# CFGpp-diffusion/CFGpp

Hardware: AMD Instinct MI355X
Metric: images/sec (higher is better)
Workload: dtype fp16; 1 GPU; SD1.5 512x512 ddim_cfg++ 50 NFE lambda=0.6 batch=8/GPU; per_gpu_batch=8, global_batch=8, nfe=50, unet_batch_rows=16, weights=seeded synthetic, exact diffusers shapes, build_id=cfgpp-build:b06ef47996861b66:nogit

## Files before the change

### cfgpp_amd/_lib.py

```python
from __future__ import annotations

import ctypes as C
import os

HERE = os.path.dirname(os.path.abspath(__file__))
LIB_PATH = os.environ.get("CFGPP_LIB") or os.path.join(HERE, "libcfgpp_hip.so")


class CfgppError(RuntimeError):
    pass


class UNetConfigC(C.Structure):
    _fields_ = [
        ("in_channels", C.c_int), ("out_channels", C.c_int),
        ("num_levels", C.c_int),
        ("block_out_channels", C.c_int * 4),
        ("layers_per_block", C.c_int),
        ("level_has_attn", C.c_int * 4),
        ("transformer_depth", C.c_int * 4),
        ("num_heads", C.c_int * 4),
        ("cross_attention_dim", C.c_int),
        ("addition_embed", C.c_int),
        ("addition_time_embed_dim", C.c_int),
        ("addition_pooled_dim", C.c_int),
        ("norm_groups", C.c_int),
        ("sample_h", C.c_int), ("sample_w", C.c_int),
        ("max_rows", C.c_int),
    ]


_P, _I, _F, _L = C.c_void_p, C.c_int, C.c_float, C.c_long

PROTOTYPES = {
    "cfgpp_last_error": (C.c_char_p, []),
    "cfgpp_build_id": (C.c_char_p, []),
    "cfgpp_step_ddim": (_I, [_P, _P, _P, _P, _I, _F, _F, _F, _F, _F, _I, _I, _L, _P]),
    "cfgpp_step_ddim_h": (_I, [_P, _P, _P, _P, _F, _F, _F, _F, _F, _I, _I, _L, _P]),
    "cfgpp_step_ddim_masked": (_I, [_P, _P, _P, _P, _F, _F, _F, _F, _F, _I, _I, _P, _P, _P, _F, _F, _I, _L, _P]),
    "cfgpp_kdiff_input": (_I, [_P, _P, _F, _I, _L, _P]),
    "cfgpp_step_kdiff": (_I, [_P, _P, _P, _P, _P, C.POINTER(C.c_float), _I, _I, _I, _I, _L, _P]),
    "cfgpp_kdiff_denoise": (_I, [_P, _P, _P, _F, _F, _P, _P, _L, _P]),
    "cfgpp_lincomb": (_I, [_P, _P, _P, _P, _F, _F, _I, _L, _P]),
    "cfgpp_unet_create": (_P, [C.POINTER(UNetConfigC), _I]),
    "cfgpp_unet_destroy": (None, [_P]),
    "cfgpp_unet_load_tensor": (_I, [_P, C.c_char_p, _P, _I, C.POINTER(C.c_long), _I]),
    "cfgpp_unet_missing": (_I, [_P]),
    "cfgpp_unet_finalize": (_I, [_P]),
    "cfgpp_unet_set_context": (_I, [_P, _P, _I, _I, _P, _P, _I, _P]),
    "cfgpp_unet_image_condition": (_I, [_P, _P, _I, _P]),
    "cfgpp_unet_forward": (_I, [_P, _P, _I, _I, _F, _P, _I, _P]),
    "cfgpp_sample_graph_ddim": (_I, [_P, _P, _P, _I, _I, _P, _P, _P, _I, C.POINTER(C.c_float), _I, _F, _I, _I, _P]),
    "cfgpp_unet_profile": (_I, [_P, _P, _I, _I, _F, _P, _I, _P, C.POINTER(C.c_double), C.POINTER(C.c_double), C.POINTER(C.c_int), C.c_char_p, _L]),
    "cfgpp_unet_tuning": (_I, [_P, _I, C.POINTER(C.c_int), _I, _I]),
    "cfgpp_unet_attach_control": (_I, [_P, _P, _F]),
    "cfgpp_unet_lora": (_I, [_P, C.c_char_p, _P, _P, _I, _P]),
    "cfgpp_unet_flops": (C.c_double, [_P, _I]),
    "cfgpp_unet_device_bytes": (C.c_double, [_P]),
    "cfgpp_vae_create": (_P, [_I, _I, _I, _F, _I]),
    "cfgpp_vae_destroy": (None, [_P]),
    "cfgpp_vae_load_tensor": (_I, [_P, C.c_char_p, _P, _I, C.POINTER(C.c_long), _I]),
    "cfgpp_vae_finalize": (_I, [_P]),
    "cfgpp_vae_decode": (_I, [_P, _P, _P, _I, _P]),
    "cfgpp_vae_decode_image": (_I, [_P, _P, _P, _I, _P]),
    "cfgpp_vae_encode": (_I, [_P, _P, _P, _P, _P, _I, _P]),
    "cfgpp_vae_flops": (C.c_double, [_P, _I]),
    "cfgpp_text_create": (_P, [_I, _I, _I, _I, _I, _I, _I, _I, _I]),
    "cfgpp_text_destroy": (None, [_P]),
    "cfgpp_text_load_tensor": (_I, [_P, C.c_char_p, _P, _I, C.POINTER(C.c_long), _I]),
    "cfgpp_text_finalize": (_I, [_P]),
    "cfgpp_text_encode": (_I, [_P, C.POINTER(C.c_int), C.POINTER(C.c_int), _I, _I, _P, _P, _P]),
    "cfgpp_text_device_bytes": (C.c_double, [_P]),
    "cfgpp_vae_encode_flops": (C.c_double, [_P, _I]),
    "cfgpp_vae_device_bytes": (C.c_double, [_P]),
}

IP_ADAPTER_PROTOTYPES = {
    "cfgpp_unet_ip_load": (_I, [_P, C.c_char_p, _P, _I, C.POINTER(C.c_long), _I]),
    "cfgpp_unet_image_context": (_I, [_P, _P, _I, _I, _F, _P]),
}

LONG_PROMPT_PROTOTYPES = {
    "cfgpp_unet_set_max_tokens": (_I, [_P, _I]),
}

DEBUG_PROTOTYPES = {
    "cfgpp_op_softmax_rows": (_I, [_P, _L, _I, _P]),
    "cfgpp_op_conv_in_ex": (_I, [_P, _I, _P, _P, _P, _I, _I, _I, _I, _I, _I, _P, _P, _F, _P]),
    "cfgpp_op_groupnorm": (_I, [_P, _P, _P, _P, _P, _P, _I, _I, _I, _I, _I, _I, _F, _I, _I, _P]),
    "cfgpp_op_groupnorm_pre": (_I, [_P, _P, _P, _P, _P, _P, _P, _P, _I, _I, _I, _I, _I, _I, _F, _I, _I, _P]),
    "cfgpp_op_igemm_set_gstat": (None, [_P]),
    "cfgpp_op_igemm_gstat_written": (_I, []),
    "cfgpp_groupnorm_set_prestats": (None, [_I]),
    "cfgpp_groupnorm_prestats_enabled": (_I, []),
    "cfgpp_unet_set_share_prefix": (None, [_I]),
    "cfgpp_unet_share_prefix_enabled": (_I, []),
    "cfgpp_unet_shared_prefix_ops": (_I, [_P, _I, _I]),
    "cfgpp_op_layernorm": (_I, [_P, _P, _P, _P, _L, _I, _F, _P]),
    "cfgpp_op_attention_prepare_vt": (_I, [_P, _I, _I, _I, _P]),
    "cfgpp_op_attention": (_I, [_P, _P, _P, _P, _I, _I, _I, _I, _I, _I, _I, _P]),
    "cfgpp_op_attention_cross": (_I, [_P, _P, _P, _P, _I, _I, _I, _I, _I, _I, _I, _P]),
    "cfgpp_attention_set_cross_long": (None, [_I]),
    "cfgpp_op_attention_clear_slots": (_I, [_P, _P, _I, _I, _I, _I, _I, _P]),
    "cfgpp_op_attention_ip": (_I, [_P, _P, _P, _P, _I, _I, _I, _I, _I, _I, _F, _I, _I, _P]),
    "cfgpp_op_conv_in": (_I, [_P, _I, _P, _P, _P, _I, _I, _I, _I, _I, _I, _P]),
    "cfgpp_op_conv_in_cond": (_I, [_P, _I, _P, _I, _I, _P, _P, _P, _I, _I, _I, _I, _I, _I, _P]),
    "cfgpp_op_conv_in_add": (_I, [_P, _I, _P, _I, _I, _P, _I, _P, _P, _P, _I, _I, _I, _I, _I, _I, _P]),
    "cfgpp_op_cn_conv3x3": (_I, [_P, _I, _P, _I, _P, _P, _I, _I, _I, _I, _I, _I, _I, _P]),
    "cfgpp_op_residual_add": (_I, [C.POINTER(C.c_void_p), C.POINTER(C.c_void_p), C.POINTER(C.c_int), _I, _I, _F, _P]),
    "cfgpp_op_residual_nchw": (_I, [_P, _P, _I, _I, _I, _I, _F, _P]),
    "cfgpp_controlnet_residual": (_I, [_P, _I, _F, _P, _I, C.POINTER(C.c_int), _P]),
    "cfgpp_vae_profile": (_I, [_P, _P, _P, _I, _P, C.c_char_p, C.c_long]),
    "cfgpp_unet_read_weight": (_I, [_P, C.c_char_p, _P]),
    "cfgpp_op_vae_posterior": (_I, [_P, _P, _P, _P, _P, _P, _I, _I, _F, _P]),
    "cfgpp_op_conv_out": (_I, [_P, _P, _I, _P, _P, _I, _I, _I, _I, _I, _P]),
    "cfgpp_op_conv_out_ex": (_I, [_P, _P, _I, _P, _P, _I, _I, _I, _I, _I, _F, _F, _I, _P]),
    "cfgpp_conv_out_set_tiled": (None, [_I]),
    "cfgpp_op_sinusoid": (_I, [_P, _F, _P, _I, _I, _I, _I, _P]),
    "cfgpp_op_skinny_gemm": (_I, [_P, _I, _P, _P, _P, _I, _P, _I, _I, _I, _I, _I, _I, _P]),
    "cfgpp_op_f16_to_f32_rows": (_I, [_P, _P, _I, _I, _I, _I, _P]),
    "cfgpp_op_igemm": (_I, [_P, _P, _I, _I, _I, _I, _I, _I, _P, _I, _I, _P, _P, _I, _P, _I, _I, _P, _I, _I, _I, _P]),
    "cfgpp_op_igemm_heads": (_I, [_P, _I, _P, _I, _I, _P, _I, _P, _P, _P, _I, _I, _I, _I, _I, _I, _P]),
    "cfgpp_op_fold_upsample": (_I, [_P, _P, _I, _I, _P]),
    "cfgpp_op_upsample_conv3x3": (_I, [_P, _I, _I, _I, _P, _P, _I, _I, _P, _P, _P]),
    "cfgpp_igemm_set_upsample_phase": (None, [_I]),
    "cfgpp_igemm_last_amode": (_I, []),
    "cfgpp_igemm_last_config_ran": (_I, []),
    "cfgpp_igemm_force_config": (None, [_I]),
    "cfgpp_igemm_set_staging": (None, [_I]),
    "cfgpp_igemm_set_staged_epilogue": (None, [_I]),
    "cfgpp_igemm_set_big_tiles": (None, [_I]),
    "cfgpp_igemm_set_tail_split": (None, [_I]),
    "cfgpp_igemm_set_autotune": (None, [_I]),
    "cfgpp_igemm_set_blocked_walk": (None, [_I]),
    "cfgpp_igemm_walk_plan_probe": (None, [_I, _I, _I, _I, _I, _I, _I, C.POINTER(C.c_int)]),
    "cfgpp_igemm_set_n_major": (None, [_I]),
    "cfgpp_igemm_force_split": (None, [_I]),
    "cfgpp_igemm_set_split_tile": (None, [_I]),
    "cfgpp_igemm_set_mf16": (None, [_I]),
    "cfgpp_igemm_set_mf16_rounds": (None, [_I]),
    "cfgpp_igemm_set_mf16_heads": (None, [_I]),
    "cfgpp_igemm_set_mf16_linear": (None, [_I]),
    "cfgpp_igemm_set_big_split": (None, [_I]),
    "cfgpp_igemm_set_tune_mask": (None, [C.c_uint]),
    "cfgpp_igemm_tuner_state": (C.c_uint, []),
    "cfgpp_igemm_timeline": (None, [_P, _L, _I]),
    "cfgpp_igemm_timeline_info": (None, [C.POINTER(C.c_int)]),
    "cfgpp_groupnorm_set_mode": (None, [_I]),
    "cfgpp_layernorm_set_rows_per_wave": (None, [_I]),
    "cfgpp_attention_set_dma": (None, [_I]),
    "cfgpp_attention_set_stagger": (None, [_I]),
    "cfgpp_attention_set_cross": (None, [_I]),
    "cfgpp_attention_last_launch": (None, [C.POINTER(C.c_int)]),
    "cfgpp_groupnorm_last_launch": (None, [C.POINTER(C.c_int)]),
    "cfgpp_layernorm_last_launch": (None, [C.POINTER(C.c_int)]),
    "cfgpp_softmax_last_launch": (None, [C.POINTER(C.c_int)]),
}

_lib = None


def load():
    global _lib
    if _lib is not None:
        return _lib
    if not os.path.exists(LIB_PATH):
        raise CfgppError(
            f"{LIB_PATH} not found: build it with `python -m cfgpp_amd.build` "
            "(__graft_entry__.build()).  The HIP path has no CPU fallback.")
    import torch
    try:
        lib = C.CDLL(LIB_PATH)
    except OSError as e:
        raise CfgppError(f"cannot load {LIB_PATH}: {e}") from e
    for name, (res, args) in list(PROTOTYPES.items()) + list(IP_ADAPTER_PROTOTYPES.items()) + list(LONG_PROMPT_PROTOTYPES.items()) + list(DEBUG_PROTOTYPES.items()):
        try:
            fn = getattr(lib, name)
        except AttributeError as e:
            raise CfgppError(f"{LIB_PATH} does not export {name}") from e
        fn.restype = res
        fn.argtypes = args
    if os.environ.get("CFGPP_AUTOTUNE", "1") == "0":
        lib.cfgpp_igemm_set_autotune(0)
    _lib = lib
    return lib


def build_id() -> str:
    return load().cfgpp_build_id().decode("utf-8", "replace")


def last_error() -> str:
    return load().cfgpp_last_error().decode("utf-8", "replace")


def check(rc: int, what: str):
    if rc != 0:
        raise CfgppError(f"{what} failed (rc={rc}): {last_error()}")
```

### cfgpp_amd/csrc/cfgpp_debug.h

```cpp
#ifndef CFGPP_DEBUG_H
#define CFGPP_DEBUG_H
#ifdef __cplusplus
extern "C" {
#endif

int cfgpp_op_softmax_rows(void* s, long rows, int ncols, void* stream);
int cfgpp_op_conv_in_ex(const void* z, int z_is_half, void* out, const float* w, const float* bias,
                        int R, int zB, int Cin, int H, int W, int Cout, const float* pre_w, const float* pre_b,
                        float in_scale, void* stream);
int cfgpp_op_groupnorm(const void* src0, const void* src1, void* dst, const float* gamma, const float* beta,
                       float* stats, int N, int H, int W, int C0, int C1, int G, float eps, int silu,
                       int dst_padded, void* stream);
int cfgpp_op_groupnorm_pre(const void* src0, const void* src1, void* dst, const float* gamma, const float* beta,
                           const float* gst0, const float* gst1, float* stats, int N, int H, int W, int C0, int C1, int G,
                           float eps, int silu, int dst_padded, void* stream);
void cfgpp_op_igemm_set_gstat(void* buf);
int cfgpp_op_igemm_gstat_written(void);
void cfgpp_groupnorm_set_prestats(int on);
int cfgpp_groupnorm_prestats_enabled(void);
void cfgpp_unet_set_share_prefix(int on);
int cfgpp_unet_share_prefix_enabled(void);
int cfgpp_unet_shared_prefix_ops(cfgpp_unet* u, int rows, int z_rows);
void cfgpp_groupnorm_set_mode(int mode);
int cfgpp_op_layernorm(const void* x, void* y, const float* gamma, const float* beta, long rows, int C,
                       float eps, void* stream);
void cfgpp_layernorm_set_rows_per_wave(int rpw);
void cfgpp_groupnorm_last_launch(int* out8);
void cfgpp_layernorm_last_launch(int* out2);
void cfgpp_softmax_last_launch(int* out1);
int cfgpp_op_attention_prepare_vt(void* vt, int BH, int d, int tok_pad, void* stream);
int cfgpp_op_attention(const void* q, const void* k, const void* vt, void* o, int B, int heads, int d,
                       int nq, int nk, int q_tok_pad, int k_tok_pad, void* stream);
void cfgpp_attention_set_dma(int mode);
void cfgpp_attention_set_stagger(int sleeps);
void cfgpp_attention_set_cross(int on);
int cfgpp_op_attention_cross(const void* q, const void* k, const void* vt, void* o, int B, int heads, int d,
                             int nq, int nk, int q_tok_pad, int k_tok_pad, void* stream);
void cfgpp_attention_set_cross_long(int mode);
void cfgpp_attention_last_launch(int* out4);
int cfgpp_op_attention_clear_slots(void* k, void* vt, int BH, int d, int tok_pad, int slot0, int n, void* stream);
int cfgpp_op_attention_ip(const void* q, const void* k, const void* vt, void* o, int B, int heads, int d, int nq, int nk_text,
                          int n_img, float ip_scale, int q_tok_pad, int k_tok_pad, void* stream);
int cfgpp_op_conv_in(const void* z, int z_is_half, void* out, const float* w, const float* bias,
                     int R, int zB, int Cin, int H, int W, int Cout, void* stream);
int cfgpp_op_conv_in_cond(const void* z, int z_is_half, const void* cond, int cond_rows, int Cc, void* out, const float* w,
                          const float* bias, int R, int zB, int Cz, int H, int W, int Cout, void* stream);
int cfgpp_op_conv_in_add(const void* z, int z_is_half, const void* cond, int cond_rows, int Cc, const void* addend, int add_rows,
                         void* out, const float* w, const float* bias, int R, int zB, int Cz, int H, int W, int Cout, void* stream);
int cfgpp_op_cn_conv3x3(const void* in, int in_kind, void* out, int out_pad, const float* w, const float* bias, int R, int Ci, int Co,
                        int Hi, int Wi, int stride, int silu, void* stream);
int cfgpp_op_residual_add(void* const* dst, const void* const* src, const int* hwc, int n, int rows, float scale, void* stream);
int cfgpp_op_residual_nchw(const void* src, float* out, int rows, int H, int W, int C, float scale, void* stream);
int cfgpp_controlnet_residual(cfgpp_unet* cn, int i, float scale, float* out, int rows, int* hwc_out, void* stream);

int cfgpp_unet_read_weight(cfgpp_unet* u, const char* key, void* host_fp16_out);

int cfgpp_vae_profile(cfgpp_vae* v, const void* z, void* img, int B, void* stream, char* detail, long detail_cap);

int cfgpp_op_vae_posterior(const float* conv_out, const float* qw, const float* qb, const float* noise, float* z,
                           float* moments, int B, int HW, float scale, void* stream);
int cfgpp_op_conv_out(const void* x, void* out, int out_is_half, const void* w, const float* bias,
                      int R, int H, int W, int C, int Cout, void* stream);
int cfgpp_op_conv_out_ex(const void* x, void* out, int out_is_half, const void* w, const float* bias,
                         int R, int H, int W, int C, int Cout, float post_scale, float post_shift, int clamp01, void* stream);
void cfgpp_conv_out_set_tiled(int on);
int cfgpp_op_sinusoid(const float* vals, float scalar, float* out, int count, int dim, int out_ld, int out_off,
                      void* stream);
int cfgpp_op_skinny_gemm(const float* x, int ldx, const void* w, const float* bias, const float* addend, int add_ld,
                         float* out, int ldo, int M, int N, int K, int silu_in, int silu_out, void* stream);
int cfgpp_op_f16_to_f32_rows(const void* in, float* out, int rows, int cols, int out_ld, int out_off, void* stream);

int cfgpp_op_igemm(const void* a0, const void* a1, int C0, int C1, int taps, int amode, int H, int W,
                   const void* w, int M, int N, const float* bias, const float* temb, int temb_ld,
                   const void* resid, int rmode, int rld, void* out, int omode, int old_, int epi,
                   void* stream);
int cfgpp_op_fold_upsample(const void* w9, void* w4, int O, int I, void* stream);
int cfgpp_op_upsample_conv3x3(const void* src, int C, int Hs, int Ws, const void* w9, const void* w4, int rows, int N,
                              const float* bias, void* out, void* stream);
void cfgpp_igemm_set_upsample_phase(int on);
int cfgpp_igemm_last_amode(void);
int cfgpp_igemm_last_config_ran(void);
int cfgpp_op_igemm_heads(const void* a, int K, const void* w, int M, int N, const float* bias, int rows_per_batch,
                         void* hq, void* hk, void* hvt, int part0, int part_width, int head_dim, int heads,
                         int q_tok_pad, int tok_pad, void* stream);
void cfgpp_igemm_force_config(int cfg);
void cfgpp_igemm_set_tail_split(int on);
void cfgpp_igemm_set_mf16(int mode);
void cfgpp_igemm_set_mf16_linear(int on);
void cfgpp_igemm_set_mf16_heads(int on);
void cfgpp_igemm_set_mf16_rounds(int n);
void cfgpp_igemm_set_split_tile(int cfg);
void cfgpp_igemm_force_split(int s);
void cfgpp_igemm_set_big_split(int min_kt);
void cfgpp_igemm_set_n_major(int mode);
void cfgpp_igemm_set_blocked_walk(int on);
void cfgpp_igemm_walk_plan_probe(int M, int N, int K, int BM, int BN, int smem, int n_major, int* out5);
void cfgpp_igemm_set_tune_mask(unsigned mask);
unsigned cfgpp_igemm_tuner_state(void);
void cfgpp_igemm_set_autotune(int on);
void cfgpp_igemm_set_big_tiles(int on);
void cfgpp_igemm_set_staged_epilogue(int on);
void cfgpp_igemm_set_staging(int glds);
void cfgpp_igemm_timeline(void* buf, long cap_blocks, int target);
void cfgpp_igemm_timeline_info(int* out12);

#ifdef __cplusplus
}
#endif
#endif
```

### cfgpp_amd/csrc/common.h

```cpp
#pragma once
#include <hip/hip_runtime.h>
#include <stdint.h>

typedef _Float16 half_t;
typedef _Float16 half2_t __attribute__((ext_vector_type(2)));
typedef _Float16 half4_t __attribute__((ext_vector_type(4)));
typedef _Float16 half8_t __attribute__((ext_vector_type(8)));
typedef float f32x4 __attribute__((ext_vector_type(4)));
typedef float f32x16 __attribute__((ext_vector_type(16)));

#define CFGPP_WAVE 64

void cfgpp_set_error(const char* fmt, ...);
int cfgpp_claim_device(int device_id);
#define CFGPP_HIP_CHECK(expr)                                                         \
    do {                                                                              \
        hipError_t _e = (expr);                                                       \
        if (_e != hipSuccess) {                                                       \
            cfgpp_set_error("%s:%d: %s -> %s", __FILE__, __LINE__, #expr,             \
                            hipGetErrorString(_e));                                   \
            return -1;                                                                \
        }                                                                             \
    } while (0)
#define CFGPP_REQUIRE(cond, ...)                                                      \
    do {                                                                              \
        if (!(cond)) {                                                                \
            cfgpp_set_error(__VA_ARGS__);                                             \
            return -2;                                                                \
        }                                                                             \
    } while (0)

int step_advance_launch(const float* tab, int* idx, float* cur, hipStream_t s);
int step_ddim_dev_launch(void* z, void* z0t_out, const void* eps_uc, const void* eps_c, int eps_is_half, int z_is_half, float lam,
                         const float* cdev, int tweedie_uc, int renoise_uc, long n, hipStream_t s);

struct CnAddEntry {
    half_t* dst;
    const half_t* src;
    int H, W, C, pad_;
};
int cn_residual_add_launch(const CnAddEntry* tab, int n, long max_n8, int rows, float scale, hipStream_t s);

int fanout_rows_launch(half_t* const* p, const long* row_elems, int nseg, int h, hipStream_t s);

int lora_merge_launch(const half_t* base, half_t* dst, const float* up, const float* down, int rank, int kind, long O, long I,
                      int taps, hipStream_t s);

static inline int cdiv(long a, long b) { return (int)((a + b - 1) / b); }

struct RowMap {
    int mode;
    int H, W;
    int ld;
};

__host__ __device__ __forceinline__ int cfgpp_vt_pos(int tok) {
    return (tok & ~12) | ((tok & 4) << 1) | ((tok & 8) >> 1);
}

__device__ __forceinline__ float silu_f(float x) { return x / (1.0f + __expf(-x)); }
__device__ __forceinline__ float gelu_erf_f(float x) {
    const float ax = fabsf(x) * 0.70710678118654752440f;
    const float t = __builtin_amdgcn_rcpf(1.0f + 0.3275911f * ax);
    const float poly = t * (0.254829592f + t * (-0.284496736f + t * (1.421413741f + t * (-1.453152027f + t * 1.061405429f))));
    const float erfc_ax = poly * __builtin_amdgcn_exp2f(-ax * ax * 1.4426950408889634f);
    const float cdf = x >= 0.f ? 1.0f - 0.5f * erfc_ax : 0.5f * erfc_ax;
    return x * cdf;
}

typedef float f32x2 __attribute__((ext_vector_type(2)));
#define CFGPP_GELU_C 4.75f
#define CFGPP_GELU_POLY {4.912262559e-01f, 5.645360425e-02f, -1.591939032e-01f, 2.464362979e-01f, -1.982378513e-01f, 1.363233291e-02f, \
                         1.386516690e-01f, -1.158297956e-01f, -9.092462249e-03f, 6.090912968e-02f, -1.936562732e-02f, -1.160200126e-02f, \
                         6.012340542e-03f}
__device__ __forceinline__ f32x2 gelu_erf_pk(f32x2 x) {
    constexpr float k[13] = CFGPP_GELU_POLY;
    f32x2 a;
    a.x = fminf(fabsf(x.x), CFGPP_GELU_C); a.y = fminf(fabsf(x.y), CFGPP_GELU_C);
    const f32x2 t = __builtin_elementwise_fma(a, (f32x2){2.0f / CFGPP_GELU_C, 2.0f / CFGPP_GELU_C}, (f32x2){-1.0f, -1.0f});
    f32x2 p = {k[12], k[12]};
#pragma unroll
    for (int i = 11; i >= 0; --i) p = __builtin_elementwise_fma(p, t, (f32x2){k[i], k[i]});
    f32x2 m;
    m.x = fabsf(x.x) * p.x; m.y = fabsf(x.y) * p.y;
    return __builtin_elementwise_fma(x, (f32x2){0.5f, 0.5f}, m);
}

template <int MAXV>
__device__ __forceinline__ void ln_row_stats(const half8_t (&raw)[MAXV], int chunks, int C, float eps, int lane,
                                             float (&v)[MAXV][8], float& mean, float& rstd) {
    float sum = 0.f;
#pragma unroll
    for (int j = 0; j < MAXV; ++j) {
        const bool live = lane + j * 64 < chunks;
#pragma unroll
        for (int k = 0; k < 8; ++k) { v[j][k] = live ? (float)raw[j][k] : 0.f; sum += v[j][k]; }
    }
#pragma unroll
    for (int o = 32; o > 0; o >>= 1) sum += __shfl_xor(sum, o);
    mean = sum / (float)C;
    float sq = 0.f;
#pragma unroll
    for (int j = 0; j < MAXV; ++j) {
        const bool live = lane + j * 64 < chunks;
#pragma unroll
        for (int k = 0; k < 8; ++k) { const float d = v[j][k] - mean; sq = live ? fmaf(d, d, sq) : sq; }
    }
#pragma unroll
    for (int o = 32; o > 0; o >>= 1) sq += __shfl_xor(sq, o);
    rstd = rsqrtf(sq / (float)C + eps);
}
__device__ __forceinline__ half8_t ln_row_affine(const float (&v)[8], float mean, float rstd, const float4 (&g)[2], const float4 (&be)[2]) {
    const float gg[8] = {g[0].x, g[0].y, g[0].z, g[0].w, g[1].x, g[1].y, g[1].z, g[1].w};
    const float bb[8] = {be[0].x, be[0].y, be[0].z, be[0].w, be[1].x, be[1].y, be[1].z, be[1].w};
    half8_t o;
#pragma unroll
    for (int k = 0; k < 8; ++k) {
        float f = fmaf((v[k] - mean) * rstd, gg[k], bb[k]);
        asm volatile("" : "+v"(f));
        o[k] = (half_t)f;
    }
    return o;
}
```

### cfgpp_amd/csrc/engine_base.h

```cpp
#pragma once
#include <algorithm>
#include <cmath>
#include <cstring>
#include <deque>
#include <functional>
#include <map>
#include <string>
#include <utility>
#include <vector>

#include "../../include/cfgpp.h"
#include "../../include/cfgpp_ip_adapter.h"
#include "../../include/cfgpp_long_prompt.h"
#include "cfgpp_debug.h"
#include "igemm.h"

namespace {


struct HostParam {
    std::vector<long> shape;
    std::vector<half_t> h;
    std::vector<float> f;
    bool is_matrix = false;
    bool loaded = false;
    long numel() const { long n = 1; for (long s : shape) n *= s; return n; }
};

struct Tensor {
    half_t* p = nullptr;
    int H = 0, W = 0, C = 0;
    float* gst = nullptr;
    int* gst_ok = nullptr;
};

using Op = std::function<int(hipStream_t, int )>;

enum { SLOT_PLAIN = 0, SLOT_CONV3 = 1, SLOT_GEGLU = 2, SLOT_MEMBER = 3 };
struct WeightSlot {
    half_t* ptr = nullptr;
    int kind = SLOT_PLAIN;
    long row_off = 0;
    long O = 0, I = 0; int taps = 1;
    half_t* base = nullptr;
    long K() const { return I * taps; }
    half_t* rows() const { return ptr + row_off * K(); }
};


struct EngineBase {
    int max_rows = 1;
    int norm_groups = 32;
    std::map<std::string, HostParam> params;
    std::map<std::string, WeightSlot> slots;
    std::vector<void*> allocs;
    double dev_bytes = 0;
    double macs_per_row = 0;
    double attn_macs_per_row = 0;

    std::vector<Op> plan;
    std::vector<int> plan_kind;
    std::vector<double> plan_macs;
    std::vector<std::string> plan_desc;
    std::vector<char> plan_share;
    int rows_for(size_t i, int rows, bool shared) const {
        const int m = i < plan_share.size() ? plan_share[i] : 0;
        if (m == 0) return rows;
        return shared ? rows / 2 : (m == 1 ? rows : 0);
    }
    void tag(int kind, double macs, const std::string& desc = "") {
        plan_kind.resize(plan.size(), 3); plan_macs.resize(plan.size(), 0.0); plan_desc.resize(plan.size());
        if (!plan.empty()) { plan_kind.back() = kind; plan_macs.back() = macs; plan_desc.back() = desc; }
    }
    std::deque<int> cfg_hints;
    std::vector<int*> plan_hint;
    int tuned_rows = 0;
    bool tuned_shared = false;
    std::map<std::pair<int, bool>, std::vector<int>> tuned_by_rows;
    int* new_hint(bool in_main_plan) {
        cfg_hints.push_back(0);
        int* h = &cfg_hints.back();
        if (in_main_plan) { plan_hint.resize(plan.size() + 1, nullptr); plan_hint[plan.size()] = h; }
        return h;
    }
    int tune_plan(hipStream_t s, int rows, bool shared = false) {
        const auto key = std::make_pair(rows, shared);
        auto cached = tuned_by_rows.find(key);
        if (cached != tuned_by_rows.end() && cached->second.size() == cfg_hints.size()) {
            size_t k = 0;
            for (int& h : cfg_hints) h = cached->second[k++];
            tuned_rows = rows; tuned_shared = shared;
            return 0;
        }
        static const int cands[] = {0, 1, 4, 5, 6, 7, 8, 9, 10, 11, 12, 13, 14, 15, 16, 17, 20, 24, 25, 26, 27, 28};
        const size_t n = plan.size();
        plan_hint.resize(n, nullptr);
        hipStreamCaptureStatus cap = hipStreamCaptureStatusNone;
        if (hipStreamIsCapturing(s, &cap) != hipSuccess || cap != hipStreamCaptureStatusNone) return 0;
// ... 333 lines not shown
```

### cfgpp_amd/csrc/norm_kernels.hip

```cpp
#include <algorithm>
#include "common.h"

namespace {

struct GNArgs {
    const half_t* src0;
    const half_t* src1;
    half_t* dst;
    const float* gamma;
    const float* beta;
    float* stats;
    int nblk;
    int spb;
    int N, H, W;
    int C0, C1;
    int G;
    float eps;
    int silu;
    int pix_per_block;
    int dst_padded;
    int gs;
    const float* gst0; const float* gst1;
    int pre;
};
// ... 225 lines not shown
    }
    s_acc[tid] = acc;
    __syncthreads();
    for (int o = 128; o > 0; o >>= 1) {
        if (tid < o) { GnAcc x = s_acc[tid]; gn_acc_merge(x, s_acc[tid + o]); s_acc[tid] = x; }
        __syncthreads();
    }
    if (tid == 0) {
        const GnAcc t = s_acc[0];
        float var = t.m2 / t.n;
        var = var < 0.f ? 0.f : var;
        float* dst = a.stats + ((long)n * a.G + g) * 2;
        dst[0] = t.mean; dst[1] = rsqrtf(var + a.eps);
    }
}

__global__ void __launch_bounds__(256)
gn_apply_kernel(GNArgs a) {
    __shared__ float s_mean[64], s_rstd[64];
    const int C = a.C0 + a.C1;
    const int cpg = C / a.G;
    const int chunks = C / 8;
    const int n = blockIdx.y;
    const int HW = a.H * a.W;
    const int p0 = blockIdx.x * a.pix_per_block;
    const int p1 = min(p0 + a.pix_per_block, HW);
    if (a.pre) {
        if ((int)threadIdx.x < a.G) {
            const float2 mr = *reinterpret_cast<const float2*>(a.stats + ((long)n * a.G + threadIdx.x) * 2);
            s_mean[threadIdx.x] = mr.x; s_rstd[threadIdx.x] = mr.y;
        }
    } else {
        __shared__ float s_ps[8][64];
        const int NSL = 256 / a.G < 8 ? 256 / a.G : 8;
        const int g = threadIdx.x % a.G, sl = threadIdx.x / a.G;
        const float* st = a.stats + (long)n * a.nblk * a.G * 2;
        const float n_full = (float)(cpg * a.spb), n_last = (float)(cpg * (HW - (a.nblk - 1) * a.spb));
        const float inv_cnt = 1.0f / ((float)cpg * (float)HW);
        const float ref = st[g * 2];
        if (sl < NSL) {
            float s = 0.f;
            for (int b = sl; b < a.nblk; b += NSL) s += (b == a.nblk - 1 ? n_last : n_full) * (st[((long)b * a.G + g) * 2] - ref);
            s_ps[sl][g] = s;
        }
        __syncthreads();
        float tot = 0.f;
        for (int k = 0; k < NSL; ++k) tot += s_ps[k][g];
        const float mean = ref + tot * inv_cnt;
        __syncthreads();
        if (sl < NSL) {
            float q = 0.f;
            for (int b = sl; b < a.nblk; b += NSL) {
                const float2 mm = *reinterpret_cast<const float2*>(st + ((long)b * a.G + g) * 2);
                const float d = mm.x - mean;
                q += mm.y + (b == a.nblk - 1 ? n_last : n_full) * d * d;
            }
            s_ps[sl][g] = q;
        }
        __syncthreads();
        if ((int)threadIdx.x < a.G) {
            float m2 = 0.f;
            for (int k = 0; k < NSL; ++k) m2 += s_ps[k][g];
            s_mean[g] = mean; s_rstd[g] = rsqrtf(m2 * inv_cnt + a.eps);
        }
    }
    __syncthreads();
    const int ppi = max(1, (int)blockDim.x / chunks);
    const float invW = 1.0f / (float)a.W;
    const long pbase = (long)n * (a.H + 2) * (a.W + 2) + (a.W + 2) + 1;
    auto poff = [&](int p) -> long { return pbase + p + 2 * (int)(((float)p + 0.5f) * invW); };
    for (int cbase = 0; cbase < chunks; cbase += blockDim.x) {
        int chunk, psub;
        if (chunks <= (int)blockDim.x) { chunk = threadIdx.x % chunks; psub = threadIdx.x / chunks; }
        else { chunk = cbase + threadIdx.x; psub = 0; }
        const bool active = (chunk < chunks) && (psub < ppi);
        if (active) {
            const int c = chunk * 8;
            const half_t* src; int cs, Cs;
            if (c < a.C0) { src = a.src0; cs = c; Cs = a.C0; } else { src = a.src1; cs = c - a.C0; Cs = a.C1; }
            float sc[8], sh[8];
#pragma unroll
            for (int k = 0; k < 8; ++k) {
                const int g = (c + k) / cpg;
                const float ga = a.gamma[c + k] * s_rstd[g];
                sc[k] = ga; sh[k] = a.beta[c + k] - s_mean[g] * ga;
            }
            auto one = [&](int p, const half8_t v, long po) {
                half8_t o;
#pragma unroll
                for (int k = 0; k < 8; ++k) {
                    float f = (float)v[k] * sc[k] + sh[k];
                    if (a.silu) f = silu_f(f);
                    o[k] = (half_t)f;
                }
                const long orow = a.dst_padded ? po : ((long)n * HW + p);
                *reinterpret_cast<half8_t*>(a.dst + orow * C + c) = o;
            };
            int p = p0 + psub;
            for (; p + 3 * ppi < p1; p += 4 * ppi) {
                half8_t v[4]; long po[4];
#pragma unroll
                for (int u = 0; u < 4; ++u) { po[u] = poff(p + u * ppi); v[u] = *reinterpret_cast<const half8_t*>(src + po[u] * Cs + cs); }
#pragma unroll
                for (int u = 0; u < 4; ++u) one(p + u * ppi, v[u], po[u]);
            }
            for (; p < p1; p += ppi) {
                const long po = poff(p);
                one(p, *reinterpret_cast<const half8_t*>(src + po * Cs + cs), po);
            }
        }
        if (chunks <= (int)blockDim.x) break;
    }
}

int g_gn_mode = 0;
int g_ln_rpw = 0;
int g_gn_last[8] = {0, 0, 0, 0, 0, 0, 0, 0};
int g_ln_last[2] = {0, 0};
int g_sm_last[1] = {0};

template <int MAXCH, int NT>
void launch_gn_slab(const GNArgs& a, int wgs, hipStream_t s) {
    hipLaunchKernelGGL((gn_slab_kernel<MAXCH, NT>), dim3(wgs), dim3(NT), 0, s, a);
}

template <int MAXV, int RPW>
__global__ void __launch_bounds__(256)
layernorm_kernel(const half_t* __restrict__ x, half_t* __restrict__ y, const float* __restrict__ gamma,
                 const float* __restrict__ beta, long rows, int C, float eps) {
    const int lane = threadIdx.x & 63;
    const long row0 = ((long)blockIdx.x * 4 + (threadIdx.x >> 6)) * RPW;
    if (row0 >= rows) return;
    const int chunks = C / 8;
    half8_t raw[RPW][MAXV];
#pragma unroll
    for (int r = 0; r < RPW; ++r) {
        const long row = row0 + r < rows ? row0 + r : rows - 1;
        const half_t* xr = x + row * C;
#pragma unroll
        for (int j = 0; j < MAXV; ++j) {
            const int ch = lane + j * 64;
            raw[r][j] = *reinterpret_cast<const half8_t*>(xr + (ch < chunks ? ch : chunks - 1) * 8);
        }
    }
    float v[RPW][MAXV][8];
    float mean[RPW], rstd[RPW];
#pragma unroll
    for (int r = 0; r < RPW; ++r) ln_row_stats<MAXV>(raw[r], chunks, C, eps, lane, v[r], mean[r], rstd[r]);
    float4 g[MAXV][2], be[MAXV][2];
#pragma unroll
    for (int j = 0; j < MAXV; ++j) {
        const int ch = lane + j * 64;
        const int cc = (ch < chunks ? ch : chunks - 1) * 8;
        g[j][0] = *reinterpret_cast<const float4*>(gamma + cc); g[j][1] = *reinterpret_cast<const float4*>(gamma + cc + 4);
        be[j][0] = *reinterpret_cast<const float4*>(beta + cc); be[j][1] = *reinterpret_cast<const float4*>(beta + cc + 4);
    }
#pragma unroll
    for (int j = 0; j < MAXV; ++j) {
        const int ch = lane + j * 64;
        if (ch < chunks) {
#pragma unroll
            for (int r = 0; r < RPW; ++r)
                if (row0 + r < rows) *reinterpret_cast<half8_t*>(y + (row0 + r) * C + ch * 8) = ln_row_affine(v[r][j], mean[r], rstd[r], g[j], be[j]);
        }
    }
}

template <int MAXC>
__global__ void __launch_bounds__(256)
softmax_rows_kernel(half_t* __restrict__ s, int ncols) {
    __shared__ float red[8];
    half_t* row = s + (long)blockIdx.x * ncols;
    const int nchunks = ncols / 8;
    const int tid = threadIdx.x, lane = tid & 63, wid = tid >> 6;
    float v[MAXC][8];
    float mx = -INFINITY;
#pragma unroll
// ... 76 lines not shown
    a.gamma = gamma; a.beta = beta;
    a.N = N; a.H = H; a.W = W; a.C0 = C0; a.C1 = C1; a.G = G; a.eps = eps; a.silu = silu;
    a.dst_padded = dst_padded; a.stats = stats; a.nblk = 0; a.spb = 0; a.gs = 1; a.pix_per_block = 0;
    a.gst0 = nullptr; a.gst1 = nullptr; a.pre = 0;
    const int HW = H * W;
    const int cpg = C / G;
    if (g_gn_mode != 1 && cpg >= 8) {
        int gs = 0;
        for (int t = 1; t <= 4; t <<= 1) if (G % t == 0 && (t * cpg) % 8 == 0) { gs = t; break; }
        const int cpp = gs ? gs * cpg / 8 : 0;
        int nt = 0;
        if (cpp && cpp <= 32) {
            for (int cand : {320, 640, 960}) {
                if (cand % cpp) continue;
                const int chunks_per_thread = cdiv(HW, cand / cpp);
                if (chunks_per_thread <= 16) { nt = cand; break; }
            }
        }
        if (nt) {
            const int R = nt / cpp, cpt = cdiv(HW, R);
            const int wgs = N * (G / gs);
            const bool worth = g_gn_mode == 2 || wgs >= 48;
            if (worth) {
                a.gs = gs;
#define GN_SLAB(NT_)                                                                        \
                if (nt == NT_) {                                                            \
                    if (cpt <= 2) launch_gn_slab<2, NT_>(a, wgs, s);                        \
                    else if (cpt <= 4) launch_gn_slab<4, NT_>(a, wgs, s);                   \
                    else if (cpt <= 8) launch_gn_slab<8, NT_>(a, wgs, s);                   \
                    else launch_gn_slab<16, NT_>(a, wgs, s);                                \
                }
                GN_SLAB(320) GN_SLAB(640) GN_SLAB(960)
#undef GN_SLAB
                g_gn_last[0] = 1; g_gn_last[1] = nt; g_gn_last[2] = cpt <= 2 ? 2 : cpt <= 4 ? 4 : cpt <= 8 ? 8 : 16;
                g_gn_last[3] = gs; g_gn_last[4] = cpp;
                CFGPP_HIP_CHECK(hipGetLastError());
                return 0;
            }
        }
    }
    const int nblk_max = std::max(64, std::min(256, cdiv(768, N)));
    int ppb = 16;
    while (cdiv(HW, ppb) > nblk_max) ppb <<= 1;
    a.pix_per_block = ppb; a.spb = ppb;
    a.nblk = cdiv(HW, ppb);
    hipLaunchKernelGGL(gn_stats_kernel, dim3(a.nblk, N), dim3(256), 0, s, a);
    GNArgs b = a;
    int apb = 64;
    while (apb > 16 && (long)N * cdiv(HW, apb) < 1024) apb >>= 1;
    b.pix_per_block = apb;
    hipLaunchKernelGGL(gn_apply_kernel, dim3(cdiv(HW, apb), N), dim3(256), 0, s, b);
    g_gn_last[0] = 2; g_gn_last[5] = ppb; g_gn_last[6] = a.nblk; g_gn_last[7] = apb;
    CFGPP_HIP_CHECK(hipGetLastError());
    return 0;
}

int cfgpp_op_groupnorm_pre(const void* src0, const void* src1, void* dst, const float* gamma, const float* beta,
                           const float* gst0, const float* gst1, float* stats, int N, int H, int W, int C0, int C1, int G,
                           float eps, int silu, int dst_padded, void* stream) {
    for (int i = 0; i < 8; ++i) g_gn_last[i] = 0;
    const int C = C0 + C1;
    CFGPP_REQUIRE(G > 0 && G <= 64 && C % G == 0, "groupnorm_pre: C=%d not divisible by G=%d (G<=64)", C, G);
    CFGPP_REQUIRE(C0 % 8 == 0 && C1 % 8 == 0, "groupnorm_pre: C0=%d C1=%d must be multiples of 8", C0, C1);
    CFGPP_REQUIRE((H * W) % 32 == 0, "groupnorm_pre: H*W=%d must be a multiple of 32 (the producers' statistics blocks)", H * W);
    CFGPP_REQUIRE(src0 && dst && gamma && beta && stats && gst0 && (C1 == 0 || (src1 && gst1)), "groupnorm_pre: null pointer");
    hipStream_t s = (hipStream_t)stream;
    GNArgs a;
    a.src0 = (const half_t*)src0; a.src1 = (const half_t*)src1; a.dst = (half_t*)dst;
    a.gamma = gamma; a.beta = beta;
    a.N = N; a.H = H; a.W = W; a.C0 = C0; a.C1 = C1; a.G = G; a.eps = eps; a.silu = silu;
    a.dst_padded = dst_padded; a.stats = stats; a.nblk = 0; a.spb = 0; a.gs = 1;
    a.gst0 = gst0; a.gst1 = gst1; a.pre = 1;
    const int HW = H * W;
    hipLaunchKernelGGL(gn_finalize_kernel, dim3(G, N), dim3(256), 0, s, a);
    int apb = 64;
    while (apb > 16 && (long)N * cdiv(HW, apb) < 1024) apb >>= 1;
    a.pix_per_block = apb;
    hipLaunchKernelGGL(gn_apply_kernel, dim3(cdiv(HW, apb), N), dim3(256), 0, s, a);
    g_gn_last[0] = 3; g_gn_last[7] = apb;
    CFGPP_HIP_CHECK(hipGetLastError());
    return 0;
}

int cfgpp_op_layernorm(const void* x, void* y, const float* gamma, const float* beta, long rows, int C,
                       float eps, void* stream) {
    g_ln_last[0] = 0; g_ln_last[1] = 0;
    CFGPP_REQUIRE(C % 8 == 0 && C <= 64 * 8 * 4, "layernorm: C=%d must be a multiple of 8 and <= 2048", C);
    CFGPP_REQUIRE(x && y && gamma && beta && rows > 0, "layernorm: bad args");
    hipStream_t s = (hipStream_t)stream;
    const int need = cdiv(C / 8, 64);
    const int rpw = g_ln_rpw > 0 ? g_ln_rpw : (C <= 320 && rows >= 2L * 4096 ? 2 : 1);
#define LN_LAUNCH(MV, RP) hipLaunchKernelGGL((layernorm_kernel<MV, RP>), dim3(cdiv(rows, 4 * RP)), dim3(256), 0, s, \
                                             (const half_t*)x, (half_t*)y, gamma, beta, rows, C, eps)
#define LN_BY_RPW(MV) do { if (rpw >= 4) LN_LAUNCH(MV, 4); else if (rpw == 2) LN_LAUNCH(MV, 2); else LN_LAUNCH(MV, 1); } while (0)
    if (need <= 1) LN_BY_RPW(1);
    else if (need <= 2) LN_BY_RPW(2);
    else if (need <= 3) LN_BY_RPW(3);
    else LN_LAUNCH(4, 1);
    g_ln_last[0] = need <= 3 ? need : 4; g_ln_last[1] = need <= 3 ? (rpw >= 4 ? 4 : rpw == 2 ? 2 : 1) : 1;
#undef LN_BY_RPW
#undef LN_LAUNCH
    CFGPP_HIP_CHECK(hipGetLastError());
    return 0;
}

}
```

### cfgpp_amd/csrc/small_kernels.hip

```cpp
#include <algorithm>

#include "common.h"

namespace {

template <typename TIN>
__global__ void __launch_bounds__(256)
conv_in_kernel(const TIN* __restrict__ z, const half_t* __restrict__ cond, int Cc, int cond_rows,
               half_t* __restrict__ out, const float* __restrict__ w,
               const float* __restrict__ bias, int R, int zB, int Cz, int H, int W, int Cout,
               const float* __restrict__ pre_w, const float* __restrict__ pre_b, float in_scale,
               const half_t* __restrict__ add, int add_rows) {
    constexpr int TP = 16;
    __shared__ float patch[TP][9 * 16];
    const int r = blockIdx.y;
    const int p0 = blockIdx.x * TP;
    const int HW = H * W;
    const int zb = r % zB;
    const int cb = cond ? zb % cond_rows : 0;
    const int Cin = Cz + Cc;
    const int K = 9 * Cin;
    for (int i = threadIdx.x; i < TP * K; i += blockDim.x) {
        const int tp = i / K, k = i - tp * K;
        const int tap = k / Cin, ci = k - tap * Cin;
        const int p = p0 + tp;
        float v = 0.f;
        if (p < HW) {
            const int y = p / W + tap / 3 - 1, x = p % W + tap % 3 - 1;
            if (y >= 0 && y < H && x >= 0 && x < W) {
                if (ci >= Cz) {
                    v = (float)cond[((long)(cb * Cc + ci - Cz) * H + y) * W + x];
                } else if (pre_w) {
                    float acc = pre_b ? pre_b[ci] : 0.f;
                    for (int j = 0; j < Cz; ++j)
                        acc += pre_w[ci * Cz + j] * (float)(half_t)((float)z[((long)(zb * Cz + j) * H + y) * W + x] * in_scale);
                    v = acc;
                } else {
                    v = (float)z[((long)(zb * Cz + ci) * H + y) * W + x] * in_scale;
                }
            }
        }
        patch[tp][k] = (float)(half_t)v;
    }
    __syncthreads();
    for (int co = threadIdx.x; co < Cout; co += blockDim.x) {
        float acc[TP];
        const float b = bias ? bias[co] : 0.f;
#pragma unroll
        for (int tp = 0; tp < TP; ++tp) acc[tp] = b;
        for (int k = 0; k < K; ++k) {
            const float wv = w[(long)k * Cout + co];
#pragma unroll
            for (int tp = 0; tp < TP; ++tp) acc[tp] += wv * patch[tp][k];
        }
#pragma unroll
        for (int tp = 0; tp < TP; ++tp) {
            const int p = p0 + tp;
            if (p < HW) {
                const int y = p / W, x = p - y * W;
                half_t v = (half_t)acc[tp];
                if (add) v = (half_t)((float)v + (float)add[((long)((zb % add_rows) * (H + 2) + y + 1) * (W + 2) + x + 1) * Cout + co]);
                out[((long)(r * (H + 2) + y + 1) * (W + 2) + x + 1) * Cout + co] = v;
            }
        }
    }
}

template <int CO, typename TOUT>
__global__ void __launch_bounds__(256)
conv_out_kernel(const half_t* __restrict__ x, TOUT* __restrict__ out, const half_t* __restrict__ w,
                const float* __restrict__ bias, int R, int H, int W, int C, int cout_real,
                float post_scale, float post_shift, int clamp01) {
    const int lane = threadIdx.x & 63;
    const long pix = (long)blockIdx.x * 4 + (threadIdx.x >> 6);
    const long total = (long)R * H * W;
    if (pix >= total) return;
    const int HW = H * W;
    const int r = (int)(pix / HW), p = (int)(pix - (long)r * HW);
    const int y = p / W, xq = p - y * W;
    const int cpt = C / 8;
    float acc[CO];
#pragma unroll
    for (int o = 0; o < CO; ++o) acc[o] = 0.f;
    for (int c = lane; c < 9 * cpt; c += 64) {
        const int tap = c / cpt, cc = (c - tap * cpt) * 8;
        const int dy = tap / 3 - 1, dx = tap % 3 - 1;
        const half8_t xv = *reinterpret_cast<const half8_t*>(
            x + ((long)(r * (H + 2) + y + 1 + dy) * (W + 2) + xq + 1 + dx) * C + cc);
#pragma unroll
        for (int o = 0; o < CO; ++o) {
            const half8_t wv = *reinterpret_cast<const half8_t*>(w + ((long)o * 9 + tap) * C + cc);
#pragma unroll
            for (int k = 0; k < 8; ++k) acc[o] += (float)xv[k] * (float)wv[k];
        }
    }
#pragma unroll
    for (int o = 0; o < CO; ++o)
#pragma unroll
        for (int s = 32; s > 0; s >>= 1) acc[o] += __shfl_xor(acc[o], s);
    if (lane < cout_real) {
        float v = 0.f;
#pragma unroll
        for (int o = 0; o < CO; ++o) if (lane == o) v = acc[o];
        v += bias ? bias[lane] : 0.f;
        v = v * post_scale + post_shift;
        if (clamp01) v = fminf(fmaxf(v, 0.f), 1.f);
        out[((long)(r * cout_real + lane) * H + y) * W + xq] = (TOUT)v;
    }
}

template <int CO, typename TOUT>
__global__ void __launch_bounds__(256)
conv_out_tile_kernel(const half_t* __restrict__ x, TOUT* __restrict__ out, const half_t* __restrict__ w,
                     const float* __restrict__ bias, int R, int H, int W, int C, int cout_real,
                     float post_scale, float post_shift, int clamp01) {
    constexpr int TH = 8, TW = 32, HH = TH + 2, HW_ = TW + 2, PITCH = 144;
    __shared__ __attribute__((aligned(16))) char tile[HH * HW_ * PITCH];
    const int tid = threadIdx.x;
    const int tiles_x = (W + TW - 1) / TW, tiles_y = (H + TH - 1) / TH;
    int b = blockIdx.x;
    const int txi = b % tiles_x; b /= tiles_x;
    const int tyi = b % tiles_y; const int r = b / tiles_y;
    const int y0 = tyi * TH, x0 = txi * TW;
    const int ty = tid >> 5, tx = tid & 31;
    typedef _Float16 h2 __attribute__((ext_vector_type(2)));
    float acc[CO];
#pragma unroll
    for (int o = 0; o < CO; ++o) acc[o] = 0.f;
    const half_t* xr = x + (long)r * (H + 2) * (W + 2) * C;
    for (int cb = 0; cb < C; cb += 64) {
        __syncthreads();
        for (int i = tid; i < HH * HW_ * 8; i += 256) {
            const int px = i >> 3, ch = i & 7;
            const int hy = px / HW_, hx = px - hy * HW_;
            const int gy = y0 + hy, gx = x0 + hx;
            half8_t v = {0, 0, 0, 0, 0, 0, 0, 0};
            if (gy < H + 2 && gx < W + 2) v = *reinterpret_cast<const half8_t*>(xr + ((long)gy * (W + 2) + gx) * C + cb + ch * 8);
            *reinterpret_cast<half8_t*>(tile + px * PITCH + ch * 16) = v;
        }
        __syncthreads();
#pragma unroll
        for (int tap = 0; tap < 9; ++tap) {
            const int dy = tap / 3, dx = tap - 3 * (tap / 3);
            const char* px = tile + ((ty + dy) * HW_ + tx + dx) * PITCH;
#pragma unroll
            for (int ch = 0; ch < 8; ++ch) {
                const half8_t xv = *reinterpret_cast<const half8_t*>(px + ch * 16);
#pragma unroll
                for (int o = 0; o < CO; ++o) {
                    const half8_t wv = *reinterpret_cast<const half8_t*>(w + ((long)o * 9 + tap) * C + cb + ch * 8);
#pragma unroll
                    for (int k = 0; k < 4; ++k)
                        acc[o] = __builtin_amdgcn_fdot2((h2){xv[2 * k], xv[2 * k + 1]}, (h2){wv[2 * k], wv[2 * k + 1]}, acc[o], false);
                }
            }
        }
    }
    const int y = y0 + ty, xq = x0 + tx;
    if (y < H && xq < W) {
#pragma unroll
        for (int o = 0; o < CO; ++o) {
            if (o < cout_real) {
                float v = acc[o] + (bias ? bias[o] : 0.f);
                v = v * post_scale + post_shift;
                if (clamp01) v = fminf(fmaxf(v, 0.f), 1.f);
                out[((long)(r * cout_real + o) * H + y) * W + xq] = (TOUT)v;
            }
        }
    }
}

__global__ void sinusoid_kernel(const float* __restrict__ vals, float scalar, float* __restrict__ out,
                                int count, int dim, int out_ld, int out_off) {
    const int i = blockIdx.x;
    const int half_dim = dim / 2;
    const float v = vals ? vals[i] : scalar;
    for (int j = threadIdx.x; j < half_dim; j += blockDim.x) {
        const float e = expf(-9.210340371976184f * (float)j / (float)half_dim);
        const float arg = v * e;
        out[(long)i * out_ld + out_off + j] = (float)(half_t)cosf(arg);
        out[(long)i * out_ld + out_off + half_dim + j] = (float)(half_t)sinf(arg);
    }
}

template <int MB, int NB>
__global__ void __launch_bounds__(256)
skinny_gemm_kernel(const float* __restrict__ x, int ldx, const half_t* __restrict__ w, const float* __restrict__ bias,
                   const float* __restrict__ addend, int add_ld, float* __restrict__ out, int ldo,
                   int M, int N, int K, int silu_in, int silu_out) {
    const int lane = threadIdx.x & 63, wid = threadIdx.x >> 6;
    const int n0 = (blockIdx.x * 4 + wid) * NB;
    const int m0 = blockIdx.y * MB;
    if (n0 >= N) return;
    float acc[MB][NB];
#pragma unroll
    for (int i = 0; i < MB; ++i)
#pragma unroll
        for (int j = 0; j < NB; ++j) acc[i][j] = 0.f;
    for (int kc = lane * 8; kc < K; kc += 64 * 8) {
        float xv[MB][8];
#pragma unroll
        for (int i = 0; i < MB; ++i) {
            const int m = min(m0 + i, M - 1);
            const float4 a = *reinterpret_cast<const float4*>(x + (long)m * ldx + kc);
            const float4 b = *reinterpret_cast<const float4*>(x + (long)m * ldx + kc + 4);
            xv[i][0] = a.x; xv[i][1] = a.y; xv[i][2] = a.z; xv[i][3] = a.w;
            xv[i][4] = b.x; xv[i][5] = b.y; xv[i][6] = b.z; xv[i][7] = b.w;
            if (silu_in) {
#pragma unroll
                for (int k = 0; k < 8; ++k) xv[i][k] = silu_f(xv[i][k]);
            }
        }
#pragma unroll
        for (int j = 0; j < NB; ++j) {
            const int n = min(n0 + j, N - 1);
            const half8_t wv = *reinterpret_cast<const half8_t*>(w + (long)n * K + kc);
#pragma unroll
            for (int i = 0; i < MB; ++i)
#pragma unroll
                for (int k = 0; k < 8; ++k) acc[i][j] += xv[i][k] * (float)wv[k];
        }
    }
#pragma unroll
    for (int i = 0; i < MB; ++i)
#pragma unroll
        for (int j = 0; j < NB; ++j)
#pragma unroll
            for (int s = 32; s > 0; s >>= 1) acc[i][j] += __shfl_xor(acc[i][j], s);
    if (lane == 0) {
#pragma unroll
        for (int i = 0; i < MB; ++i) {
            const int m = m0 + i;
            if (m >= M) continue;
#pragma unroll
            for (int j = 0; j < NB; ++j) {
                const int n = n0 + j;
                if (n >= N) continue;
                float v = acc[i][j] + (bias ? bias[n] : 0.f);
                if (addend) v += addend[(long)m * add_ld + n];
                if (silu_out) v = silu_f(v);
                out[(long)m * ldo + n] = v;
            }
        }
    }
}

__global__ void f16_to_f32_rows_kernel(const half_t* __restrict__ in, float* __restrict__ out, int rows, int cols,
                                       int out_ld, int out_off) {
    const long n = (long)rows * cols;
    for (long i = (long)blockIdx.x * blockDim.x + threadIdx.x; i < n; i += (long)gridDim.x * blockDim.x) {
        const int r = (int)(i / cols), c = (int)(i - (long)r * cols);
        out[(long)r * out_ld + out_off + c] = (float)in[i];
    }
}

struct FanoutArgs {
    uint4* p[3];
    long n16[3];
};

__global__ void __launch_bounds__(256)
fanout_rows_kernel(FanoutArgs a) {
    const long n = a.n16[blockIdx.y];
    const uint4* __restrict__ src = a.p[blockIdx.y];
    uint4* __restrict__ dst = a.p[blockIdx.y] + n;
    const long T = (long)gridDim.x * 256;
    long i = (long)blockIdx.x * 256 + threadIdx.x;
    for (; i + 3 * T < n; i += 4 * T) {
        const uint4 v0 = src[i], v1 = src[i + T], v2 = src[i + 2 * T], v3 = src[i + 3 * T];
        dst[i] = v0; dst[i + T] = v1; dst[i + 2 * T] = v2; dst[i + 3 * T] = v3;
    }
    for (; i < n; i += T) dst[i] = src[i];
}

}

int fanout_rows_launch(half_t* const* p, const long* row_elems, int nseg, int h, hipStream_t s) {
    CFGPP_REQUIRE(p && row_elems && nseg > 0 && nseg <= 3 && h > 0, "fanout_rows: bad args");
    FanoutArgs a{};
    long most = 0;
    for (int k = 0; k < nseg; ++k) {
        CFGPP_REQUIRE(p[k] && row_elems[k] > 0 && row_elems[k] % 8 == 0 && ((uintptr_t)p[k] & 15) == 0, "fanout_rows: segment %d is not made of 16-byte units", k);
        a.p[k] = reinterpret_cast<uint4*>(p[k]);
        a.n16[k] = (long)h * (row_elems[k] / 8);
        most = std::max(most, a.n16[k]);
    }
    dim3 grid((unsigned)std::min<long>(cdiv(most, 256 * 4), 2048), (unsigned)nseg);
    hipLaunchKernelGGL(fanout_rows_kernel, grid, dim3(256), 0, s, a);
    CFGPP_HIP_CHECK(hipGetLastError());
    return 0;
}


__global__ void __launch_bounds__(256)
vae_posterior_kernel(const float* __restrict__ co, const float* __restrict__ qw, const float* __restrict__ qb,
                     const float* __restrict__ noise, float* __restrict__ z, float* __restrict__ moments,
                     int B, int HW, float scale) {
    const long i = (long)blockIdx.x * blockDim.x + threadIdx.x;
    if (i >= (long)B * HW) return;
    const int b = (int)(i / HW), p = (int)(i - (long)b * HW);
    float x[8], m[8];
#pragma unroll
    for (int j = 0; j < 8; ++j) x[j] = (float)(half_t)co[((long)b * 8 + j) * HW + p];
#pragma unroll
    for (int o = 0; o < 8; ++o) {
        float acc = qb[o];
#pragma unroll
        for (int j = 0; j < 8; ++j) acc += qw[o * 8 + j] * x[j];
        m[o] = (float)(half_t)acc;
    }
#pragma unroll
    for (int c = 0; c < 4; ++c) {
        const float lv = fminf(fmaxf(m[4 + c], -30.f), 20.f);
        const float n = noise ? noise[((long)b * 4 + c) * HW + p] : 0.f;
        z[((long)b * 4 + c) * HW + p] = (m[c] + __expf(0.5f * lv) * n) * scale;
        if (moments) { moments[((long)b * 8 + c) * HW + p] = m[c]; moments[((long)b * 8 + 4 + c) * HW + p] = lv; }
    }
}

extern "C" {

int cfgpp_op_vae_posterior(const float* conv_out, const float* qw, const float* qb, const float* noise, float* z,
                           float* moments, int B, int HW, float scale, void* stream) {
    CFGPP_REQUIRE(conv_out && qw && qb && z && B > 0 && HW > 0, "vae_posterior: bad args");
    hipLaunchKernelGGL(vae_posterior_kernel, dim3(cdiv((long)B * HW, 256)), dim3(256), 0, (hipStream_t)stream, conv_out, qw, qb, noise, z, moments, B, HW, scale);
    CFGPP_HIP_CHECK(hipGetLastError());
    return 0;
}

int cfgpp_op_conv_in_add(const void* z, int z_is_half, const void* cond, int cond_rows, int Cc, const void* addend, int add_rows,
                         void* out, const float* w, const float* bias, int R, int zB, int Cz, int H, int W, int Cout, void* stream);

int cfgpp_op_conv_in_cond(const void* z, int z_is_half, const void* cond, int cond_rows, int Cc, void* out, const float* w,
                          const float* bias, int R, int zB, int Cz, int H, int W, int Cout, void* stream) {
    return cfgpp_op_conv_in_add(z, z_is_half, cond, cond_rows, Cc, nullptr, 1, out, w, bias, R, zB, Cz, H, W, Cout, stream);
}

int cfgpp_op_conv_in_add(const void* z, int z_is_half, const void* cond, int cond_rows, int Cc, const void* addend, int add_rows,
                         void* out, const float* w, const float* bias, int R, int zB, int Cz, int H, int W, int Cout, void* stream) {
    CFGPP_REQUIRE(Cz >= 1 && Cz <= 8, "conv_in: Cin=%d (<= 8)", Cz);
    CFGPP_REQUIRE(!addend || add_rows > 0, "conv_in: addend with add_rows=%d", add_rows);
    const half_t* add = (const half_t*)addend;
    if (!add) add_rows = 1;
    CFGPP_REQUIRE(!cond || (Cc >= 1 && Cz + Cc <= 16 && cond_rows > 0), "conv_in: condition of %d channels x %d rows on %d latent channels (Cin <= 16)",
                  Cc, cond_rows, Cz);
    CFGPP_REQUIRE(z && out && w && R > 0 && zB > 0, "conv_in: bad args");
    if (!cond) { Cc = 0; cond_rows = 1; }
    dim3 grid(cdiv((long)H * W, 16), R);
    hipStream_t s = (hipStream_t)stream;
    if (z_is_half)
        hipLaunchKernelGGL(conv_in_kernel<half_t>, grid, dim3(256), 0, s, (const half_t*)z, (const half_t*)cond, Cc, cond_rows, (half_t*)out, w, bias,
                           R, zB, Cz, H, W, Cout, (const float*)nullptr, (const float*)nullptr, 1.0f, add, add_rows);
    else
        hipLaunchKernelGGL(conv_in_kernel<float>, grid, dim3(256), 0, s, (const float*)z, (const half_t*)cond, Cc, cond_rows, (half_t*)out, w, bias,
                           R, zB, Cz, H, W, Cout, (const float*)nullptr, (const float*)nullptr, 1.0f, add, add_rows);
    CFGPP_HIP_CHECK(hipGetLastError());
    return 0;
}

int cfgpp_op_conv_in_ex(const void* z, int z_is_half, void* out, const float* w, const float* bias,
                        int R, int zB, int Cin, int H, int W, int Cout, const float* pre_w, const float* pre_b,
                        float in_scale, void* stream) {
    CFGPP_REQUIRE(Cin >= 1 && Cin <= 8, "conv_in: Cin=%d (<= 8)", Cin);
    CFGPP_REQUIRE(z && out && w && R > 0 && zB > 0, "conv_in: bad args");
    dim3 grid(cdiv((long)H * W, 16), R);
    hipStream_t s = (hipStream_t)stream;
    if (z_is_half)
        hipLaunchKernelGGL(conv_in_kernel<half_t>, grid, dim3(256), 0, s, (const half_t*)z, (const half_t*)nullptr, 0, 1, (half_t*)out, w, bias,
                           R, zB, Cin, H, W, Cout, pre_w, pre_b, in_scale, (const half_t*)nullptr, 1);
    else
        hipLaunchKernelGGL(conv_in_kernel<float>, grid, dim3(256), 0, s, (const float*)z, (const half_t*)nullptr, 0, 1, (half_t*)out, w, bias,
                           R, zB, Cin, H, W, Cout, pre_w, pre_b, in_scale, (const half_t*)nullptr, 1);
    CFGPP_HIP_CHECK(hipGetLastError());
    return 0;
}

int cfgpp_op_conv_in(const void* z, int z_is_half, void* out, const float* w, const float* bias,
                     int R, int zB, int Cin, int H, int W, int Cout, void* stream) {
    return cfgpp_op_conv_in_ex(z, z_is_half, out, w, bias, R, zB, Cin, H, W, Cout, nullptr, nullptr, 1.0f, stream);
}

int cfgpp_op_conv_out_ex(const void* x, void* out, int out_is_half, const void* w, const float* bias,
                         int R, int H, int W, int C, int Cout, float post_scale, float post_shift, int clamp01, void* stream);
static int g_conv_out_tiled = 1;
void cfgpp_conv_out_set_tiled(int on) { g_conv_out_tiled = on ? 1 : 0; }

int cfgpp_op_conv_out(const void* x, void* out, int out_is_half, const void* w, const float* bias,
                      int R, int H, int W, int C, int Cout, void* stream) {
    return cfgpp_op_conv_out_ex(x, out, out_is_half, w, bias, R, H, W, C, Cout, 1.0f, 0.0f, 0, stream);
}

int cfgpp_op_conv_out_ex(const void* x, void* out, int out_is_half, const void* w, const float* bias,
                         int R, int H, int W, int C, int Cout, float post_scale, float post_shift, int clamp01, void* stream) {
    CFGPP_REQUIRE(Cout >= 1 && Cout <= 8 && C % 8 == 0, "conv_out: Cout=%d C=%d", Cout, C);
    CFGPP_REQUIRE(x && out && w, "conv_out: null pointer");
    const long total = (long)R * H * W;
    dim3 grid(cdiv(total, 4));
    hipStream_t s = (hipStream_t)stream;
    if (Cout <= 4 && C % 64 == 0 && (long)H * W >= 128 * 128 && g_conv_out_tiled) {
        dim3 tg((unsigned)((long)R * cdiv(H, 8) * cdiv(W, 32)));
        if (out_is_half)
            hipLaunchKernelGGL((conv_out_tile_kernel<4, half_t>), tg, dim3(256), 0, s, (const half_t*)x, (half_t*)out, (const half_t*)w, bias, R, H, W, C, Cout, post_scale, post_shift, clamp01);
        else if (Cout <= 3)
            hipLaunchKernelGGL((conv_out_tile_kernel<3, float>), tg, dim3(256), 0, s, (const half_t*)x, (float*)out, (const half_t*)w, bias, R, H, W, C, Cout, post_scale, post_shift, clamp01);
        else
            hipLaunchKernelGGL((conv_out_tile_kernel<4, float>), tg, dim3(256), 0, s, (const half_t*)x, (float*)out, (const half_t*)w, bias, R, H, W, C, Cout, post_scale, post_shift, clamp01);
        CFGPP_HIP_CHECK(hipGetLastError());
        return 0;
    }
    if (Cout > 4) {
        CFGPP_REQUIRE(!out_is_half, "conv_out: 8-channel output is fp32 only");
        hipLaunchKernelGGL((conv_out_kernel<8, float>), grid, dim3(256), 0, s, (const half_t*)x, (float*)out, (const half_t*)w, bias, R, H, W, C, Cout, post_scale, post_shift, clamp01);
    } else if (out_is_half)
        hipLaunchKernelGGL((conv_out_kernel<4, half_t>), grid, dim3(256), 0, s, (const half_t*)x, (half_t*)out, (const half_t*)w, bias, R, H, W, C, Cout, post_scale, post_shift, clamp01);
    else
        hipLaunchKernelGGL((conv_out_kernel<4, float>), grid, dim3(256), 0, s, (const half_t*)x, (float*)out, (const half_t*)w, bias, R, H, W, C, Cout, post_scale, post_shift, clamp01);
    CFGPP_HIP_CHECK(hipGetLastError());
    return 0;
}

int cfgpp_op_sinusoid(const float* vals, float scalar, float* out, int count, int dim, int out_ld, int out_off,
                      void* stream) {
    CFGPP_REQUIRE(out && count > 0 && dim % 2 == 0, "sinusoid: bad args");
    hipLaunchKernelGGL(sinusoid_kernel, dim3(count), dim3(128), 0, (hipStream_t)stream, vals, scalar, out, count, dim, out_ld, out_off);
    CFGPP_HIP_CHECK(hipGetLastError());
    return 0;
}

int cfgpp_op_skinny_gemm(const float* x, int ldx, const void* w, const float* bias, const float* addend, int add_ld,
                         float* out, int ldo, int M, int N, int K, int silu_in, int silu_out, void* stream) {
    CFGPP_REQUIRE(x && w && out && M > 0 && N > 0 && K % 8 == 0, "skinny_gemm: bad args (K=%d)", K);
    hipStream_t s = (hipStream_t)stream;
    if (M == 1) {
        dim3 grid(cdiv(N, 4 * 2), 1);
        hipLaunchKernelGGL((skinny_gemm_kernel<1, 2>), grid, dim3(256), 0, s, x, ldx, (const half_t*)w, bias, addend, add_ld, out, ldo, M, N, K, silu_in, silu_out);
    } else {
        dim3 grid(cdiv(N, 4 * 2), cdiv(M, 4));
        hipLaunchKernelGGL((skinny_gemm_kernel<4, 2>), grid, dim3(256), 0, s, x, ldx, (const half_t*)w, bias, addend, add_ld, out, ldo, M, N, K, silu_in, silu_out);
    }
    CFGPP_HIP_CHECK(hipGetLastError());
    return 0;
}

int cfgpp_op_f16_to_f32_rows(const void* in, float* out, int rows, int cols, int out_ld, int out_off, void* stream) {
    hipLaunchKernelGGL(f16_to_f32_rows_kernel, dim3(cdiv((long)rows * cols, 256) > 1024 ? 1024 : cdiv((long)rows * cols, 256)),
                       dim3(256), 0, (hipStream_t)stream, (const half_t*)in, out, rows, cols, out_ld, out_off);
    CFGPP_HIP_CHECK(hipGetLastError());
    return 0;
}

}
```

### cfgpp_amd/csrc/unet.hip

```cpp
#include "engine_base.h"

struct cfgpp_unet : EngineBase {
    cfgpp_unet_config cfg;
    int device = 0;
    bool finalized = false;

    std::vector<Op> ctx_plan;
    const void* in_z = nullptr; int in_z_half = 0; int in_z_rows = 0; float in_t = 0.f; void* out_eps = nullptr;
    const float* in_t_dev = nullptr;
    half_t* d_cond = nullptr; int cond_rows = 0;
    float* d_step_tab = nullptr; int step_tab_cap = 0; float* d_step_cur = nullptr; int* d_step_idx = nullptr;
    hipStream_t cap_stream = nullptr;
    struct GraphKey { const void* z; void* z0t; void* eps; const void* euc; const void* ec; int z_half, z_rows, rows, tw, rn; float lam; long n; int tuned_serial; int cond_rows;
                      int ip_active = 0, ip_n_img = 0; unsigned ip_scale_bits = 0;
                      int ctx_tokens = 77; };
    struct Graph { GraphKey key; hipGraph_t graph; hipGraphExec_t exec; };
    std::vector<Graph> graphs;
    int tuned_serial = 0;
    int prefix_ops = 0;
    double prefix_macs_per_row = 0;
    int ran_shared = -1;
    bool shares(int rows, int z_rows) const;
    bool enter_call(int rows, int z_rows) {
        const bool sh = shares(rows, z_rows);
        if (ran_shared != (int)sh) { if (ran_shared >= 0) ++tuned_serial; ran_shared = (int)sh; }
        return sh;
    }
    static void destroy(Graph& g) { if (g.exec) hipGraphExecDestroy(g.exec); if (g.graph) hipGraphDestroy(g.graph); g.exec = nullptr; g.graph = nullptr; }
    void drop_graphs() { for (auto& g : graphs) destroy(g); graphs.clear(); }
    ~cfgpp_unet() { drop_graphs(); if (cap_stream) hipStreamDestroy(cap_stream); for (auto& a : ip_allocs) hipFree(a.first); }
    const half_t* ctx_ehs = nullptr; int ctx_rows = 0; int ctx_tokens = 77;
    int max_tokens = 77;
    const half_t* ctx_text = nullptr; const float* ctx_tids = nullptr; int ctx_cond_rows = 0;
    bool ctx_set = false;

    float* d_sin_t = nullptr; float* d_emb_h = nullptr; float* d_emb_t = nullptr; float* d_emb = nullptr;
    float* d_temb_all = nullptr; int temb_total = 0;
    float* d_add_in = nullptr; float* d_add_h = nullptr; float* d_aug = nullptr;

    half_t *tok_x = nullptr, *tok_ln = nullptr, *tok_attn = nullptr, *tok_ff = nullptr;
    half_t *hq[4] = {nullptr, nullptr, nullptr, nullptr}, *hk[4] = {nullptr, nullptr, nullptr, nullptr},
           *hvt[4] = {nullptr, nullptr, nullptr, nullptr};

    bool control = false;
    std::vector<int> embed_ch;
    std::vector<Op> img_plan;
    const void* img_in = nullptr; int img_in_half = 0;
    half_t* d_img_emb = nullptr; int img_rows = 0;
    std::vector<Tensor> ctrl_res;
    std::vector<Tensor> ctrl_dst;
    cfgpp_unet* ctrl = nullptr; float ctrl_scale = 0.f;
    CnAddEntry* d_ctrl_tab = nullptr; long ctrl_max_n8 = 0;

    static constexpr int IP_SLOT = 96, IP_MAX = 32;
    struct IpBlock {
        std::string name;
        int C, nheads, d, dp, tok; half_t* ck; half_t* cvt;
        size_t plan_idx;
        half_t* wkv = nullptr;
        bool has_k = false, has_v = false;
    };
    std::vector<IpBlock> ip_blocks;
    int ip_ck_pad = 0;
    half_t* ip_wproj = nullptr; float* ip_bproj = nullptr; float* ip_ng = nullptr; float* ip_nb = nullptr;
    long ip_proj_rows = 0, ip_bias_rows = 0; int ip_embed = 0;
    half_t* ip_proj_out = nullptr; half_t* ip_tok = nullptr; long ip_tok_cap = 0;
    std::vector<std::pair<void*, size_t>> ip_allocs;
    bool ip_active = false; int ip_n_img = 0; float ip_scale = 0.f;
    const void* ip_src = nullptr; int ip_rows = 0;
    void* ip_malloc(size_t bytes) {
        void* p = nullptr;
        if (hipMalloc(&p, bytes) != hipSuccess) return nullptr;
        ip_allocs.push_back(std::make_pair(p, bytes)); dev_bytes += (double)bytes;
        return p;
    }
    void ip_free(void* p) {
        for (size_t i = 0; i < ip_allocs.size(); ++i)
            if (ip_allocs[i].first == p) { hipFree(p); dev_bytes -= (double)ip_allocs[i].second; ip_allocs.erase(ip_allocs.begin() + i); return; }
    }
    double ip_macs_per_key = 0;
    void ip_set_active(bool on, int n_img, float scale) {
        ip_active = on; ip_n_img = on ? n_img : 0; ip_scale = on ? scale : 0.f;
        for (const IpBlock& b : ip_blocks) {
            const double per_key = 2.0 * (double)b.nheads * b.tok * b.d;
            const std::string desc = "cross_attn heads=" + std::to_string(b.nheads) + " N=" + std::to_string(b.tok) + " d=" + std::to_string(b.d);
            plan_macs[b.plan_idx] = per_key * (ctx_tokens + ip_n_img);
            plan_desc[b.plan_idx] = on ? desc + " ip=" + std::to_string(n_img) : ctx_tokens != 77 ? desc + " keys=" + std::to_string(ctx_tokens) : desc;
        }
    }
    void retag_cross() { if (plan_macs.size() == plan.size()) ip_set_active(ip_active, ip_n_img, ip_scale); }
    void ip_drop() {
        if (plan_macs.size() == plan.size()) ip_set_active(false, 0, 0.f);
        while (!ip_allocs.empty()) ip_free(ip_allocs.back().first);
        for (IpBlock& b : ip_blocks) { b.wkv = nullptr; b.has_k = b.has_v = false; }
        ip_wproj = nullptr; ip_bproj = nullptr; ip_ng = nullptr; ip_nb = nullptr; ip_proj_out = nullptr; ip_tok = nullptr;
        ip_proj_rows = ip_bias_rows = 0; ip_embed = 0; ip_tok_cap = 0; ip_src = nullptr; ip_rows = 0;
    }
};

static int g_share_prefix = 1;
bool cfgpp_unet::shares(int rows, int z_rows) const { return g_share_prefix && prefix_ops > 0 && rows == 2 * z_rows; }

namespace {

void build_param_table(cfgpp_unet* u) {
    const cfgpp_unet_config& c = u->cfg;
    const int L = c.num_levels;
    const long c0 = c.block_out_channels[0], temb = 4 * c0;
    expect_conv(u, "conv_in", c0, c.in_channels, 3);
    expect_linear(u, "time_embedding.linear_1", temb, c0);
    expect_linear(u, "time_embedding.linear_2", temb, temb);
    if (c.addition_embed) {
        const long in = (long)c.addition_time_embed_dim * 6 + c.addition_pooled_dim;
        expect_linear(u, "add_embedding.linear_1", temb, in);
        expect_linear(u, "add_embedding.linear_2", temb, temb);
    }
    long ch = c0;
    for (int i = 0; i < L; ++i) {
        const long co = c.block_out_channels[i];
        const std::string p = "down_blocks." + std::to_string(i);
        for (int j = 0; j < c.layers_per_block; ++j) {
// ... 222 lines not shown
    const cfgpp_unet_config& c = u->cfg;
    const int L = c.num_levels, R = c.max_rows;
    const int c0 = c.block_out_channels[0], temb_dim = 4 * c0;
    Builder B{u};
    Plan P{u, &B, &u->plan};
    Plan PC{u, &B, &u->ctx_plan};

    long max_tok_c = 0, max_ff = 0;
    {
        int H = c.sample_h, W = c.sample_w;
        for (int i = 0; i < L; ++i) {
            const long C = c.block_out_channels[i];
            if (c.level_has_attn[i] || i == L - 1) {
                const long tok = (long)H * W;
                const int d = (int)(C / c.num_heads[i]), dp = round_up(d, 32);
                max_tok_c = std::max(max_tok_c, tok * C);
                max_ff = std::max(max_ff, tok * 4 * C);
                u->hq[i] = (half_t*)u->dmalloc((size_t)R * c.num_heads[i] * round_up((int)tok, 128) * dp * 2);
                u->hk[i] = (half_t*)u->dmalloc((size_t)R * c.num_heads[i] * round_up((int)tok, 128) * dp * 2);
                u->hvt[i] = (half_t*)u->dmalloc((size_t)R * c.num_heads[i] * dp * round_up((int)tok, 64) * 2);
                CFGPP_REQUIRE(u->hq[i] && u->hk[i] && u->hvt[i], "finalize: hipMalloc failed");
                if (cfgpp_op_attention_prepare_vt(u->hvt[i], R * c.num_heads[i], d, round_up((int)tok, 64), nullptr)) return -1;
            }
            if (i != L - 1) { H /= 2; W /= 2; }
        }
    }
    u->tok_x = (half_t*)u->dmalloc((size_t)R * max_tok_c * 2);
    u->tok_ln = (half_t*)u->dmalloc((size_t)R * max_tok_c * 2);
    u->tok_attn = (half_t*)u->dmalloc((size_t)R * max_tok_c * 2);
    u->tok_ff = (half_t*)u->dmalloc((size_t)R * max_ff * 2);
    u->d_gn_stats = (float*)u->dmalloc((size_t)R * (1024 * 64 * 2 + 64 * 2) * sizeof(float));
    u->d_sin_t = (float*)u->dmalloc((size_t)c0 * sizeof(float));
    u->d_emb_h = (float*)u->dmalloc((size_t)temb_dim * sizeof(float));
    u->d_emb_t = (float*)u->dmalloc((size_t)temb_dim * sizeof(float));
    u->d_emb = (float*)u->dmalloc((size_t)R * temb_dim * sizeof(float));
    CFGPP_REQUIRE(u->tok_x && u->tok_ln && u->tok_attn && u->tok_ff, "finalize: hipMalloc failed");

    std::vector<std::string> res_names;
    {
        for (int i = 0; i < L; ++i)
            for (int j = 0; j < c.layers_per_block; ++j) res_names.push_back("down_blocks." + std::to_string(i) + ".resnets." + std::to_string(j));
        res_names.push_back("mid_block.resnets.0"); res_names.push_back("mid_block.resnets.1");
        for (int i = 0; i < L && !u->control; ++i)
            for (int j = 0; j < c.layers_per_block + 1; ++j) res_names.push_back("up_blocks." + std::to_string(i) + ".resnets." + std::to_string(j));
    }
    std::map<std::string, int> temb_off;
    half_t* w_temb_all = nullptr; float* b_temb_all = nullptr;
    {
        std::vector<half_t> wa; std::vector<float> ba; int off = 0;
        for (auto& rn : res_names) {
            HostParam* pw = B.get(rn + ".time_emb_proj.weight"); HostParam* pb = B.get(rn + ".time_emb_proj.bias");
            CFGPP_REQUIRE(pw && pb, "finalize: %s", B.err.c_str());
            temb_off[rn] = off; off += (int)pw->shape[0];
            wa.insert(wa.end(), pw->h.begin(), pw->h.end()); ba.insert(ba.end(), pb->f.begin(), pb->f.end());
            B.drop(rn + ".time_emb_proj.weight"); B.drop(rn + ".time_emb_proj.bias");
        }
        u->temb_total = off;
        w_temb_all = B.upload(wa); b_temb_all = B.upload(ba);
        for (auto& rn : res_names) B.slot(rn + ".time_emb_proj.weight", w_temb_all, SLOT_MEMBER, temb_off[rn]);
        u->d_temb_all = (float*)u->dmalloc((size_t)R * off * sizeof(float));
    }
    const bool per_row_temb = c.addition_embed != 0;
    const int temb_ld = per_row_temb ? u->temb_total : 0;

    {
        half_t* w1 = B.linear("time_embedding.linear_1.weight"); float* b1 = B.f32("time_embedding.linear_1.bias");
        half_t* w2 = B.linear("time_embedding.linear_2.weight"); float* b2 = B.f32("time_embedding.linear_2.bias");
        cfgpp_unet* uu = u;
        u->plan.push_back([=](hipStream_t s, int) { return cfgpp_op_sinusoid(uu->in_t_dev, uu->in_t, uu->d_sin_t, 1, c0, c0, 0, s); });
        u->plan.push_back([=](hipStream_t s, int) { return cfgpp_op_skinny_gemm(uu->d_sin_t, c0, w1, b1, nullptr, 0, uu->d_emb_h, temb_dim, 1, temb_dim, c0, 0, 1, s); });
        if (per_row_temb) {
            u->plan.push_back([=](hipStream_t s, int rows) {
                const int add_ld = uu->ctx_cond_rows == 1 ? 0 : temb_dim;
                return cfgpp_op_skinny_gemm(uu->d_emb_h, 0, w2, b2, uu->d_aug, add_ld, uu->d_emb, temb_dim, rows, temb_dim, temb_dim, 0, 0, s);
            });
            u->plan.push_back([=](hipStream_t s, int rows) {
                return cfgpp_op_skinny_gemm(uu->d_emb, temb_dim, w_temb_all, b_temb_all, nullptr, 0, uu->d_temb_all, uu->temb_total, rows, uu->temb_total, temb_dim, 1, 0, s);
            });
        } else {
            u->plan.push_back([=](hipStream_t s, int) { return cfgpp_op_skinny_gemm(uu->d_emb_h, temb_dim, w2, b2, nullptr, 0, uu->d_emb_t, temb_dim, 1, temb_dim, temb_dim, 0, 0, s); });
            u->plan.push_back([=](hipStream_t s, int) {
                return cfgpp_op_skinny_gemm(uu->d_emb_t, temb_dim, w_temb_all, b_temb_all, nullptr, 0, uu->d_temb_all, uu->temb_total, 1, uu->temb_total, temb_dim, 1, 0, s);
            });
        }
        if (c.addition_embed) {
            const int tdim = c.addition_time_embed_dim, pooled = c.addition_pooled_dim, in = 6 * tdim + pooled;
            half_t* aw1 = B.linear("add_embedding.linear_1.weight"); float* ab1 = B.f32("add_embedding.linear_1.bias");
            half_t* aw2 = B.linear("add_embedding.linear_2.weight"); float* ab2 = B.f32("add_embedding.linear_2.bias");
            u->d_add_in = (float*)u->dmalloc((size_t)R * in * sizeof(float));
            u->d_add_h = (float*)u->dmalloc((size_t)R * temb_dim * sizeof(float));
            u->d_aug = (float*)u->dmalloc((size_t)R * temb_dim * sizeof(float));
            u->ctx_plan.push_back([=](hipStream_t s, int) { return cfgpp_op_f16_to_f32_rows(uu->ctx_text, uu->d_add_in, uu->ctx_cond_rows, pooled, in, 0, s); });
            u->ctx_plan.push_back([=](hipStream_t s, int) {
                for (int r = 0; r < uu->ctx_cond_rows; ++r) {
                    int e = cfgpp_op_sinusoid(uu->ctx_tids + (long)r * 6, 0.f, uu->d_add_in + (long)r * in + pooled, 6, tdim, tdim, 0, s);
                    if (e) return e;
                }
                return 0;
            });
            u->ctx_plan.push_back([=](hipStream_t s, int) { return cfgpp_op_skinny_gemm(uu->d_add_in, in, aw1, ab1, nullptr, 0, uu->d_add_h, temb_dim, uu->ctx_cond_rows, temb_dim, in, 0, 1, s); });
            u->ctx_plan.push_back([=](hipStream_t s, int) { return cfgpp_op_skinny_gemm(uu->d_add_h, temb_dim, aw2, ab2, nullptr, 0, uu->d_aug, temb_dim, uu->ctx_cond_rows, temb_dim, temb_dim, 0, 0, s); });
        }
    }

    auto load_res = [&](const std::string& p, int cin, int cout) {
        ResW w{}; w.cin = cin; w.cout = cout;
        w.n1g = B.f32(p + ".norm1.weight"); w.n1b = B.f32(p + ".norm1.bias");
        w.w1 = B.conv3(p + ".conv1.weight"); w.b1 = B.f32(p + ".conv1.bias");
        w.n2g = B.f32(p + ".norm2.weight"); w.n2b = B.f32(p + ".norm2.bias");
        w.w2 = B.conv3(p + ".conv2.weight"); w.b2 = B.f32(p + ".conv2.bias");
        if (cin != cout) { w.wsc = B.linear(p + ".conv_shortcut.weight"); w.bsc = B.f32(p + ".conv_shortcut.bias"); }
        w.temb_off = temb_off[p];
        return w;
    };
    auto resblock = [&](const std::string& p, const Tensor& x0, const Tensor* x1, int cout) {
        const int cin = x0.C + (x1 ? x1->C : 0);
        ResW w = load_res(p, cin, cout);
        Tensor g1 = u->acq(x0.H, x0.W, cin);
        P.groupnorm(x0, x1, g1.p, true, w.n1g, w.n1b, 1e-5f, true);
        Tensor h1 = u->acq(x0.H, x0.W, cout);
        P.conv3x3(g1, h1, w.w1, w.b1, 1, u->d_temb_all + w.temb_off, temb_ld, nullptr);
        u->rel(g1);
        Tensor g2 = u->acq(x0.H, x0.W, cout);
        P.groupnorm(h1, nullptr, g2.p, true, w.n2g, w.n2b, 1e-5f, true);
        u->rel(h1);
        Tensor out = u->acq(x0.H, x0.W, cout);
        if (cin != cout) {
            Tensor sc = u->acq(x0.H, x0.W, cout);
            P.conv1x1(x0, x1, sc, w.wsc, w.bsc);
            P.conv3x3(g2, out, w.w2, w.b2, 1, nullptr, 0, &sc);
            u->rel(sc);
        } else {
            P.conv3x3(g2, out, w.w2, w.b2, 1, nullptr, 0, &x0);
        }
        u->rel(g2);
        return out;
    };
    int cross_block_counter = 0;
    long prefix_from = -1;
    auto transformer = [&](const std::string& p, const Tensor& x, int depth, int nheads, int lvl) {
        half_t* const HQ = u->hq[lvl]; half_t* const HK = u->hk[lvl]; half_t* const HVT = u->hvt[lvl];
        const int C = x.C, tok = x.H * x.W, d = C / nheads, dp = round_up(d, 32);
        const int q_pad = round_up(tok, 128), k_pad = round_up(tok, 64);
        const int ck_pad = std::max(128, round_up(u->max_tokens, 64));
        float* ng = B.f32(p + ".norm.weight"); float* nb = B.f32(p + ".norm.bias");
        half_t* wpi = B.linear(p + ".proj_in.weight"); float* bpi = B.f32(p + ".proj_in.bias");
        half_t* wpo = B.linear(p + ".proj_out.weight"); float* bpo = B.f32(p + ".proj_out.bias");
        P.groupnorm(x, nullptr, u->tok_ln, false, ng, nb, 1e-6f, false);
        P.linear(u->tok_ln, C, u->tok_x, C, wpi, bpi, nullptr, tok);
        for (int k = 0; k < depth; ++k) {
            const std::string b = p + ".transformer_blocks." + std::to_string(k);
            float* l1g = B.f32(b + ".norm1.weight"); float* l1b = B.f32(b + ".norm1.bias");
            float* l2g = B.f32(b + ".norm2.weight"); float* l2b = B.f32(b + ".norm2.bias");
            float* l3g = B.f32(b + ".norm3.weight"); float* l3b = B.f32(b + ".norm3.bias");
            half_t* wqkv = B.concat({b + ".attn1.to_q.weight", b + ".attn1.to_k.weight", b + ".attn1.to_v.weight"});
            half_t* wq2 = B.linear(b + ".attn2.to_q.weight");
            half_t* wff1 = nullptr; float* bff1 = nullptr;
            B.geglu(b + ".ff.net.0.proj", C, &wff1, &bff1);
            half_t* wo1 = B.linear(b + ".attn1.to_out.0.weight"); float* bo1 = B.f32(b + ".attn1.to_out.0.bias");
            half_t* wkv2 = B.concat({b + ".attn2.to_k.weight", b + ".attn2.to_v.weight"});
            half_t* wo2 = B.linear(b + ".attn2.to_out.0.weight"); float* bo2 = B.f32(b + ".attn2.to_out.0.bias");
            half_t* wff2 = B.linear(b + ".ff.net.2.weight"); float* bff2 = B.f32(b + ".ff.net.2.bias");
            half_t* ck = (half_t*)u->dmalloc((size_t)R * nheads * ck_pad * dp * 2);
            half_t* cvt = (half_t*)u->dmalloc((size_t)R * nheads * dp * ck_pad * 2);
            if (!ck || !cvt || cfgpp_op_attention_prepare_vt(cvt, R * nheads, d, ck_pad, nullptr)) { B.ok = false; B.err = "cross-attention K/V^T allocation failed"; }
            {
// ... 89 lines not shown
            });
        }
    }
    std::vector<Tensor> skips; skips.push_back(x);
    for (int i = 0; i < L; ++i) {
        const int co = c.block_out_channels[i];
        const std::string p = "down_blocks." + std::to_string(i);
        for (int j = 0; j < c.layers_per_block; ++j) {
            if (i == 0 && j == 0 && !per_row_temb && c.level_has_attn[0]) prefix_from = (long)u->plan.size();
            Tensor y = resblock(p + ".resnets." + std::to_string(j), x, nullptr, co);
            if (c.level_has_attn[i]) {
                Tensor z = transformer(p + ".attentions." + std::to_string(j), y, c.transformer_depth[i], c.num_heads[i], i);
                u->rel(y); y = z;
            }
            x = y; skips.push_back(x);
        }
        if (i != L - 1) {
            half_t* wd = B.conv3(p + ".downsamplers.0.conv.weight"); float* bd = B.f32(p + ".downsamplers.0.conv.bias");
            H /= 2; W /= 2;
            Tensor y = u->acq(H, W, co);
            P.conv3x3(x, y, wd, bd, 2, nullptr, 0, nullptr);
            x = y; skips.push_back(x);
        }
    }
    {
        const int cm = c.block_out_channels[L - 1];
        Tensor y = resblock("mid_block.resnets.0", x, nullptr, cm);
        Tensor z = transformer("mid_block.attentions.0", y, c.transformer_depth[L - 1], c.num_heads[L - 1], L - 1);
        u->rel(y);
        Tensor w = resblock("mid_block.resnets.1", z, nullptr, cm);
        u->rel(z);
        x = w;
    }
    if (u->control) {
        int e = controlnet_tail(u, B, P, skips, x);
        if (e) return e;
        skips.clear();
        CFGPP_REQUIRE(B.ok, "finalize: %s", B.err.c_str());
        CFGPP_HIP_CHECK(hipDeviceSynchronize());
        u->plan_kind.resize(u->plan.size(), 3); u->plan_macs.resize(u->plan.size(), 0.0); u->plan_desc.resize(u->plan.size());
        u->plan_share.resize(u->plan.size(), 0);
        u->finalized = true;
        return 0;
    }
    {
        u->ctrl_dst = skips; u->ctrl_dst.push_back(x);
        u->d_ctrl_tab = (CnAddEntry*)u->dmalloc(u->ctrl_dst.size() * sizeof(CnAddEntry));
        CFGPP_REQUIRE(u->d_ctrl_tab, "finalize: hipMalloc failed");
        for (const Tensor& t : u->ctrl_dst) u->ctrl_max_n8 = std::max(u->ctrl_max_n8, (long)R * t.H * t.W * (t.C / 8));
        cfgpp_unet* uu = u;
        const int n = (int)u->ctrl_dst.size();
        u->plan.push_back([uu, n](hipStream_t s, int rows) {
            if (!uu->ctrl || uu->ctrl_scale == 0.f) return 0;
            for (const Tensor& t : uu->ctrl_dst) if (t.gst_ok) *t.gst_ok = 0;
            return cn_residual_add_launch(uu->d_ctrl_tab, n, uu->ctrl_max_n8, rows, uu->ctrl_scale, s);
        });
        u->tag(3, 0.0, "controlnet residual add");
    }
    for (int i = 0; i < L; ++i) {
        const int lvl = L - 1 - i;
        const int co = c.block_out_channels[lvl];
        const std::string p = "up_blocks." + std::to_string(i);
        for (int j = 0; j < c.layers_per_block + 1; ++j) {
            Tensor skip = skips.back(); skips.pop_back();
            Tensor y = resblock(p + ".resnets." + std::to_string(j), x, &skip, co);
            u->rel(x); u->rel(skip);
            if (c.level_has_attn[lvl]) {
                Tensor z = transformer(p + ".attentions." + std::to_string(j), y, c.transformer_depth[lvl], c.num_heads[lvl], lvl);
                u->rel(y); y = z;
            }
            x = y;
        }
        if (i != L - 1) {
            half_t* wu = B.conv3(p + ".upsamplers.0.conv.weight"); float* bu = B.f32(p + ".upsamplers.0.conv.bias");
            H *= 2; W *= 2;
            Tensor y = u->acq(H, W, co);
            P.conv3x3(x, y, wu, bu, 3, nullptr, 0, nullptr);
            u->rel(x); x = y;
        }
    }
    {
        float* g = B.f32("conv_norm_out.weight"); float* b = B.f32("conv_norm_out.bias");
        Tensor gn = u->acq(H, W, c0);
        P.groupnorm(x, nullptr, gn.p, true, g, b, 1e-5f, true);
        HostParam* pw = B.get("conv_out.weight"); float* bo = B.f32("conv_out.bias");
        CFGPP_REQUIRE(pw, "finalize: %s", B.err.c_str());
        const int Co = c.out_channels;
        CFGPP_REQUIRE(Co <= 4, "finalize: out_channels %d > 4 unsupported", Co);
        std::vector<half_t> r((size_t)Co * 9 * c0);
        for (int o = 0; o < Co; ++o) for (int i = 0; i < c0; ++i) for (int t = 0; t < 9; ++t)
            r[((size_t)o * 9 + t) * c0 + i] = pw->h[((size_t)o * c0 + i) * 9 + t];
        half_t* dw = B.upload(r);
        cfgpp_unet* uu = u; half_t* gp = gn.p; const int HH = H, WW = W;
        u->macs_per_row += (double)H * W * Co * 9.0 * c0 + (double)c.sample_h * c.sample_w * c0 * 9.0 * c.in_channels;
        u->plan.push_back([=](hipStream_t s, int rows) { return cfgpp_op_conv_out(gp, uu->out_eps, 1, dw, bo, rows, HH, WW, c0, Co, s); });
    }
    CFGPP_REQUIRE(B.ok, "finalize: %s", B.err.c_str());
    CFGPP_REQUIRE(skips.empty(), "finalize: internal error, %d skips left", (int)skips.size());
    CFGPP_HIP_CHECK(hipDeviceSynchronize());
    u->plan_kind.resize(u->plan.size(), 3); u->plan_macs.resize(u->plan.size(), 0.0); u->plan_desc.resize(u->plan.size());
    u->plan_share.resize(u->plan.size(), 0);
    u->finalized = true;
    return 0;
}

int cfgpp_unet_set_context(cfgpp_unet* u, const void* ehs, int rows, int tokens, const void* text_embeds,
                           const void* time_ids, int cond_rows, void* stream) {
    CFGPP_REQUIRE(u && u->finalized, "set_context: context not finalized");
    CFGPP_REQUIRE(ehs && rows > 0 && rows <= u->cfg.max_rows, "set_context: rows=%d (max %d)", rows, u->cfg.max_rows);
    CFGPP_REQUIRE(tokens >= 77 && tokens % 77 == 0 && tokens <= u->max_tokens,
                  "set_context: tokens=%d (a multiple of 77 up to max_tokens=%d, which cfgpp_unet_set_max_tokens raises before finalize)", tokens,
                  u->max_tokens);
    if (u->cfg.addition_embed) {
        CFGPP_REQUIRE(text_embeds && time_ids, "set_context: SDXL needs text_embeds and time_ids");
        CFGPP_REQUIRE(cond_rows == rows || cond_rows == 1, "set_context: cond_rows=%d must be rows (%d) or 1", cond_rows, rows);
    }
    u->ctx_ehs = (const half_t*)ehs; u->ctx_rows = rows; u->ctx_tokens = tokens;
    u->ctx_text = (const half_t*)text_embeds; u->ctx_tids = (const float*)time_ids; u->ctx_cond_rows = cond_rows;
    for (auto& op : u->ctx_plan) { int e = op((hipStream_t)stream, rows); if (e) return e; }
    u->ctx_set = true;
    u->retag_cross();
    return 0;
}

int cfgpp_unet_set_max_tokens(cfgpp_unet* u, int max_tokens) {
    CFGPP_REQUIRE(u, "set_max_tokens: null engine");
    CFGPP_REQUIRE(!u->finalized, "set_max_tokens: max_tokens=%d after cfgpp_unet_finalize (the cross-attention buffers are sized there)", max_tokens);
    CFGPP_REQUIRE(max_tokens == 77 || max_tokens == 154 || max_tokens == 231 || max_tokens == 308,
                  "set_max_tokens: max_tokens=%d (77, 154, 231 or 308)", max_tokens);
    u->max_tokens = max_tokens;
    return 0;
}

int cfgpp_unet_image_condition(cfgpp_unet* u, const void* cond, int cond_rows, void* stream) {
    CFGPP_REQUIRE(u && u->finalized, "image_condition: engine not finalized");
    if (u->control) {
        CFGPP_REQUIRE(cond && cond_rows > 0 && cond_rows <= u->cfg.max_rows, "image_condition: ControlNet image_rows=%d (1 .. %d)", cond_rows,
                      u->cfg.max_rows);
        u->img_in = cond; u->img_in_half = 1;
        for (auto& op : u->img_plan) { int e = op((hipStream_t)stream, cond_rows); if (e) return e; }
        u->img_in = nullptr;
        u->img_rows = cond_rows;
        return 0;
    }
    CFGPP_REQUIRE(u->cfg.in_channels > u->cfg.out_channels && u->d_cond,
                  "image_condition: this UNet takes %d input channels for %d latent channels - no image condition (not an inpaint UNet)",
                  u->cfg.in_channels, u->cfg.out_channels);
    CFGPP_REQUIRE(cond && cond_rows > 0 && cond_rows <= u->cfg.max_rows, "image_condition: cond_rows=%d (1 .. %d)", cond_rows, u->cfg.max_rows);
    const size_t bytes = (size_t)cond_rows * (u->cfg.in_channels - u->cfg.out_channels) * u->cfg.sample_h * u->cfg.sample_w * sizeof(half_t);
    CFGPP_HIP_CHECK(hipMemcpyAsync(u->d_cond, cond, bytes, hipMemcpyDeviceToDevice, (hipStream_t)stream));
    u->cond_rows = cond_rows;
    return 0;
}

static int ip_fail(const char* key, const char* why) { cfgpp_set_error("ip_load: %s: %s", key, why); return -2; }

int cfgpp_unet_ip_load(cfgpp_unet* u, const char* key, const void* host, int dtype, const long* shape, int ndim) {
    CFGPP_REQUIRE(u && u->finalized, "ip_load: the engine is not finalized (the adapter attaches to the uploaded UNet)");
    CFGPP_REQUIRE(!u->control, "ip_load: a ControlNet takes no image tokens (diffusers passes it the text context only)");
    CFGPP_REQUIRE(!key || u->max_tokens == 77, "ip_load: IP-Adapter on an engine with max_tokens=%d (the image slots sit at key 96 of a 128-slot "
                  "buffer: max_tokens must be 77)", u->max_tokens);
    CFGPP_HIP_CHECK(hipSetDevice(u->device));
    if (!key) {
        CFGPP_HIP_CHECK(hipDeviceSynchronize());
        u->ip_drop();
        for (const auto& b : u->ip_blocks)
            if (cfgpp_op_attention_clear_slots(b.ck, b.cvt, u->max_rows * b.nheads, b.d, u->ip_ck_pad, cfgpp_unet::IP_SLOT, cfgpp_unet::IP_MAX, nullptr)) return -1;
        return 0;
    }
    CFGPP_REQUIRE(host && shape && (dtype == 0 || dtype == 1), "ip_load: %s: null tensor or dtype %d (0 fp32, 1 fp16)", key, dtype);
    const std::string k = key;
    const long cross = u->cfg.cross_attention_dim;
    long n = 1; for (int i = 0; i < ndim; ++i) n *= shape[i];
    auto to_half = [&](std::vector<half_t>& h) {
        h.resize(n);
        if (dtype == 0) { const float* s = (const float*)host; for (long i = 0; i < n; ++i) h[i] = (half_t)s[i]; }
        else std::memcpy(h.data(), host, n * sizeof(half_t));
    };
// ... 117 lines not shown
            a.a0 = u->ip_tok; a.C0 = cross; a.amode = 0; a.w = b.wkv; a.N = 2 * b.C; a.K = cross; a.epi = EPI_HEADS;
            a.hq = nullptr; a.hk = b.ck + (size_t)cfgpp_unet::IP_SLOT * b.dp; a.hvt = b.cvt + cfgpp_unet::IP_SLOT;
            a.part0 = 1; a.part_width = b.C; a.head_dim = b.d; a.head_dim_pad = b.dp; a.heads = b.nheads;
            a.tok_pad = u->ip_ck_pad; a.q_tok_pad = u->ip_ck_pad; a.rows_per_batch = n_img; a.M = rows * n_img;
            if (int e = igemm_launch(a, s)) return e;
        }
        u->ip_src = image_embeds; u->ip_rows = rows;
    }
    u->ip_set_active(true, n_img, scale);
    return 0;
}

int cfgpp_unet_attach_control(cfgpp_unet* u, cfgpp_unet* cn, float scale) {
    CFGPP_REQUIRE(u && u->finalized, "attach_control: UNet not finalized");
    CFGPP_REQUIRE(!u->control, "attach_control: the target is itself a ControlNet");
    if (!cn) { u->ctrl = nullptr; u->ctrl_scale = 0.f; return 0; }
    CFGPP_REQUIRE(cn->finalized && cn->control, "attach_control: not a finalized ControlNet (cfgpp_unet_create with out_channels = 0, then finalize)");
    const cfgpp_unet_config &a = u->cfg, &b = cn->cfg;
    CFGPP_REQUIRE(a.num_levels == b.num_levels && a.layers_per_block == b.layers_per_block, "attach_control: levels %d x %d vs the UNet's %d x %d",
                  b.num_levels, b.layers_per_block, a.num_levels, a.layers_per_block);
    for (int i = 0; i < a.num_levels; ++i)
        CFGPP_REQUIRE(a.block_out_channels[i] == b.block_out_channels[i], "attach_control: channels of level %d: %d vs the UNet's %d", i,
                      b.block_out_channels[i], a.block_out_channels[i]);
    CFGPP_REQUIRE(a.sample_h == b.sample_h && a.sample_w == b.sample_w, "attach_control: latent %d x %d vs the UNet's %d x %d", b.sample_h,
                  b.sample_w, a.sample_h, a.sample_w);
    CFGPP_REQUIRE(a.max_rows == b.max_rows, "attach_control: max_rows %d vs the UNet's %d", b.max_rows, a.max_rows);
    CFGPP_REQUIRE(b.in_channels == a.out_channels, "attach_control: the ControlNet takes %d latent channels, the UNet %d", b.in_channels,
                  a.out_channels);
    CFGPP_REQUIRE(cn->ctrl_res.size() == u->ctrl_dst.size(), "attach_control: %d residuals for %d skip connections + mid block",
                  (int)cn->ctrl_res.size(), (int)u->ctrl_dst.size());
    std::vector<CnAddEntry> tab(u->ctrl_dst.size());
    for (size_t i = 0; i < tab.size(); ++i) {
        const Tensor &d = u->ctrl_dst[i], &r = cn->ctrl_res[i];
        CFGPP_REQUIRE(d.H == r.H && d.W == r.W && d.C == r.C, "attach_control: residual %d is %d x %d x %d, the UNet tensor %d x %d x %d", (int)i,
                      r.H, r.W, r.C, d.H, d.W, d.C);
        tab[i] = CnAddEntry{d.p, r.p, d.H, d.W, d.C, 0};
    }
    CFGPP_HIP_CHECK(hipSetDevice(u->device));
    CFGPP_HIP_CHECK(hipDeviceSynchronize());
    CFGPP_HIP_CHECK(hipMemcpy(u->d_ctrl_tab, tab.data(), tab.size() * sizeof(CnAddEntry), hipMemcpyHostToDevice));
    u->ctrl = cn; u->ctrl_scale = scale;
    return 0;
}

int cfgpp_controlnet_residual(cfgpp_unet* cn, int i, float scale, float* out, int rows, int* hwc_out, void* stream) {
    CFGPP_REQUIRE(cn && cn->finalized && cn->control, "controlnet_residual: not a finalized ControlNet");
    const int n = (int)cn->ctrl_res.size();
    if (!out && !hwc_out) return n;
    CFGPP_REQUIRE(i >= 0 && i < n, "controlnet_residual: index %d (0 .. %d)", i, n - 1);
    const Tensor& r = cn->ctrl_res[i];
    if (hwc_out) { hwc_out[0] = r.H; hwc_out[1] = r.W; hwc_out[2] = r.C; }
    if (!out) return n;
    CFGPP_REQUIRE(rows > 0 && rows <= cn->cfg.max_rows, "controlnet_residual: rows=%d", rows);
    int e = cfgpp_op_residual_nchw(r.p, out, rows, r.H, r.W, r.C, scale, stream);
    return e ? e : n;
}

int cfgpp_unet_forward(cfgpp_unet* u, const void* z, int z_is_half, int z_rows, float t, void* eps_out, int rows,
                       void* stream) {
    CFGPP_REQUIRE(u && u->finalized, "forward: context not finalized");
    CFGPP_REQUIRE(u->ctx_set, "forward: set_context has not been called");
    CFGPP_REQUIRE(z && eps_out && z_rows > 0 && rows > 0 && rows <= u->cfg.max_rows, "forward: bad args (rows=%d max=%d)", rows, u->cfg.max_rows);
    CFGPP_REQUIRE(rows == u->ctx_rows, "forward: rows=%d but context was set for %d rows", rows, u->ctx_rows);
    CFGPP_REQUIRE(u->control || u->cfg.in_channels == u->cfg.out_channels || (u->cond_rows > 0 && (u->cond_rows == 1 || u->cond_rows == z_rows)),
                  "forward: inpaint UNet (%d input channels) needs cfgpp_unet_image_condition with 1 or z_rows=%d rows first (has %d)",
                  u->cfg.in_channels, z_rows, u->cond_rows);
    CFGPP_REQUIRE(!u->control || u->img_rows > 0, "forward: ControlNet without a control image (call cfgpp_unet_image_condition first)");
    CFGPP_REQUIRE(!u->ip_active || u->ip_rows == rows, "forward: the image context (IP-Adapter) was set for %d rows, the forward runs %d: call "
                  "cfgpp_unet_image_context after cfgpp_unet_set_context", u->ip_rows, rows);
    if (u->ctrl && u->ctrl_scale != 0.f) {
        cfgpp_unet* cn = u->ctrl;
        CFGPP_REQUIRE(cn->img_rows > 0, "forward: a ControlNet is attached but has no control image (cfgpp_unet_image_condition)");
        CFGPP_REQUIRE(cn->ctx_set && cn->ctx_rows == rows, "forward: the attached ControlNet's context is set for %d rows, the forward runs %d",
                      cn->ctx_set ? cn->ctx_rows : 0, rows);
        int e = cfgpp_unet_forward(cn, z, z_is_half, z_rows, t, eps_out, rows, stream);
        if (e) return e;
    }
    u->in_z = z; u->in_z_half = z_is_half; u->in_z_rows = z_rows; u->in_t = t; u->in_t_dev = nullptr; u->out_eps = eps_out;
    const bool shared = u->enter_call(rows, z_rows);
    if ((u->tuned_rows != rows || u->tuned_shared != shared) && igemm_autotune_enabled()) {
        int e = u->tune_plan((hipStream_t)stream, rows, shared); if (e) return e;
        ++u->tuned_serial;
    }
    for (size_t i = 0; i < u->plan.size(); ++i) { int e = u->plan[i]((hipStream_t)stream, u->rows_for(i, rows, shared)); if (e) return e; }
    return 0;
}

int cfgpp_sample_graph_ddim(cfgpp_unet* u, void* z, void* z0t, int z_is_half, int z_rows, void* eps, const void* eps_uc,
                            const void* eps_c, int rows, const float* host_steps, int n_steps, float lam, int tweedie_uc,
                            int renoise_uc, void* stream) {
    CFGPP_REQUIRE(u && u->finalized && u->ctx_set, "sample_graph: context not ready");
    CFGPP_REQUIRE(z && z0t && eps && eps_uc && eps_c && host_steps && n_steps > 0 && z_rows > 0, "sample_graph: bad args");
    CFGPP_REQUIRE(rows == u->ctx_rows && rows <= u->cfg.max_rows, "sample_graph: rows=%d but context was set for %d rows", rows, u->ctx_rows);
    CFGPP_REQUIRE(!u->ctrl && !u->control, "sample_graph: a ControlNet is attached (a controlled step is not captured): detach it "
                                            "(cfgpp_unet_attach_control(u, NULL, 0)) or run the eager loop");
    hipStream_t s = (hipStream_t)stream;
    CFGPP_REQUIRE(u->cfg.in_channels == u->cfg.out_channels || (u->cond_rows > 0 && (u->cond_rows == 1 || u->cond_rows == z_rows)),
                  "sample_graph: inpaint UNet (%d input channels) needs cfgpp_unet_image_condition with 1 or z_rows=%d rows first (has %d)",
                  u->cfg.in_channels, z_rows, u->cond_rows);
    const long n = (long)z_rows * u->cfg.out_channels * u->cfg.sample_h * u->cfg.sample_w;
    if (!u->d_step_cur) {
        u->d_step_cur = (float*)u->dmalloc(8 * sizeof(float));
        u->d_step_idx = (int*)u->dmalloc(sizeof(int));
        CFGPP_REQUIRE(u->d_step_cur && u->d_step_idx, "sample_graph: out of device memory");
        CFGPP_HIP_CHECK(hipStreamCreateWithFlags(&u->cap_stream, hipStreamNonBlocking));
    }
    if (n_steps > u->step_tab_cap) {
        u->drop_graphs();
        const int cap = n_steps < 64 ? 64 : n_steps;
        u->d_step_tab = (float*)u->dmalloc((size_t)cap * 8 * sizeof(float));
        CFGPP_REQUIRE(u->d_step_tab, "sample_graph: out of device memory");
        u->step_tab_cap = cap;
    }
    u->enter_call(rows, z_rows);
    CFGPP_REQUIRE(!u->ip_active || u->ip_rows == rows, "sample_graph: the image context (IP-Adapter) was set for %d rows, the loop runs %d", u->ip_rows, rows);
    cfgpp_unet::GraphKey want{z, z0t, eps, eps_uc, eps_c, z_is_half, z_rows, rows, tweedie_uc, renoise_uc, lam, n, 0, u->cond_rows};
    want.ip_active = u->ip_active ? 1 : 0; want.ip_n_img = u->ip_n_img; std::memcpy(&want.ip_scale_bits, &u->ip_scale, sizeof(float));
    want.ctx_tokens = u->ctx_tokens;
    auto same = [&](const cfgpp_unet::GraphKey& k) {
        return k.z == want.z && k.z0t == want.z0t && k.eps == want.eps && k.euc == want.euc && k.ec == want.ec && k.z_half == want.z_half &&
               k.z_rows == want.z_rows && k.rows == want.rows && k.tw == want.tw && k.rn == want.rn && k.lam == want.lam && k.n == want.n &&
               k.tuned_serial == u->tuned_serial && k.cond_rows == want.cond_rows && k.ip_active == want.ip_active &&
               k.ip_n_img == want.ip_n_img && k.ip_scale_bits == want.ip_scale_bits && k.ctx_tokens == want.ctx_tokens;
    };
    int hit = -1;
    for (size_t i = 0; i < u->graphs.size(); ++i) if (same(u->graphs[i].key)) hit = (int)i;
    if (hit < 0) {
        int e = cfgpp_unet_forward(u, z, z_is_half, z_rows, host_steps[0], eps, rows, stream);
        if (e) return e;
        CFGPP_HIP_CHECK(hipStreamSynchronize(s));
        for (size_t i = 0; i < u->graphs.size();)
            if (u->graphs[i].key.tuned_serial != u->tuned_serial) { cfgpp_unet::destroy(u->graphs[i]); u->graphs.erase(u->graphs.begin() + i); } else ++i;
        cfgpp_unet::Graph g{want, nullptr, nullptr};
        g.key.tuned_serial = u->tuned_serial;
        u->in_t_dev = u->d_step_cur;
        hipError_t he = hipStreamBeginCapture(u->cap_stream, hipStreamCaptureModeRelaxed);
        int rc = 0;
        if (he == hipSuccess) {
            rc = step_advance_launch(u->d_step_tab, u->d_step_idx, u->d_step_cur, u->cap_stream);
            const bool shared = u->shares(rows, z_rows);
            for (size_t i = 0; i < u->plan.size() && rc == 0; ++i) rc = u->plan[i](u->cap_stream, u->rows_for(i, rows, shared));
            if (rc == 0) rc = step_ddim_dev_launch(z, z0t, eps_uc, eps_c, 1, z_is_half, lam, u->d_step_cur + 1, tweedie_uc, renoise_uc, n, u->cap_stream);
            he = hipStreamEndCapture(u->cap_stream, &g.graph);
        }
        u->in_t_dev = nullptr;
        if (he != hipSuccess || rc != 0 || !g.graph) {
            cfgpp_unet::destroy(g);
            if (rc == 0) cfgpp_set_error("sample_graph: stream capture failed: %s", hipGetErrorString(he));
            return rc ? rc : -1;
        }
        he = hipGraphInstantiate(&g.exec, g.graph, nullptr, nullptr, 0);
        if (he != hipSuccess) { cfgpp_unet::destroy(g); cfgpp_set_error("sample_graph: hipGraphInstantiate: %s", hipGetErrorString(he)); return -1; }
        if (u->graphs.size() >= 4) { cfgpp_unet::destroy(u->graphs.front()); u->graphs.erase(u->graphs.begin()); }
        u->graphs.push_back(g);
        hit = (int)u->graphs.size() - 1;
    }
    if (hit != (int)u->graphs.size() - 1) std::swap(u->graphs[hit], u->graphs.back());
    hipGraphExec_t exec = u->graphs.back().exec;
    std::vector<float> tab((size_t)n_steps * 8, 0.f);
    for (int i = 0; i < n_steps; ++i) for (int k = 0; k < 5; ++k) tab[(size_t)i * 8 + k] = host_steps[(size_t)i * 5 + k];
    CFGPP_HIP_CHECK(hipMemcpyAsync(u->d_step_tab, tab.data(), tab.size() * sizeof(float), hipMemcpyHostToDevice, s));
    CFGPP_HIP_CHECK(hipStreamSynchronize(s));
    CFGPP_HIP_CHECK(hipMemsetAsync(u->d_step_idx, 0, sizeof(int), s));
    for (int i = 0; i < n_steps; ++i) CFGPP_HIP_CHECK(hipGraphLaunch(exec, s));
    return 0;
}

// ... 11 lines not shown
    std::vector<hipEvent_t> ev(n + 1);
    for (auto& e : ev) CFGPP_HIP_CHECK(hipEventCreate(&e));
    CFGPP_HIP_CHECK(hipEventRecord(ev[0], s));
    int rc = 0;
    for (size_t i = 0; i < n && rc == 0; ++i) { rc = u->plan[i](s, op_rows[i]); if (rc == 0 && hipEventRecord(ev[i + 1], s) != hipSuccess) rc = -1; }
    if (rc == 0 && hipStreamSynchronize(s) != hipSuccess) rc = -1;
    for (int k = 0; k < 4; ++k) { out_ms[k] = 0; out_flops[k] = 0; out_launches[k] = 0; }
    if (rc == 0) {
        for (size_t i = 0; i < n; ++i) {
            if (op_rows[i] == 0) continue;
            float ms = 0.f; hipEventElapsedTime(&ms, ev[i], ev[i + 1]);
            const int k = u->plan_kind[i];
            out_ms[k] += ms; out_flops[k] += 2.0 * u->plan_macs[i] * op_rows[i]; out_launches[k] += 1;
        }
        if (detail && detail_cap > 0) {
            std::string txt;
            for (size_t i = 0; i < n; ++i) {
                if (op_rows[i] == 0) continue;
                float ms = 0.f; hipEventElapsedTime(&ms, ev[i], ev[i + 1]);
                char line[256];
                const std::string desc = u->plan_desc[i] + (op_rows[i] != rows ? " rows=" + std::to_string(op_rows[i]) : std::string());
                snprintf(line, sizeof(line), "%zu\t%d\t%s\t%.1f\t%.3f\n", i, u->plan_kind[i], desc.c_str(), ms * 1e3,
                         2.0 * u->plan_macs[i] * op_rows[i] * 1e-9);
                txt += line;
            }
            const long ncopy = std::min<long>((long)txt.size(), detail_cap - 1);
            std::memcpy(detail, txt.data(), ncopy); detail[ncopy] = 0;
        }
    }
    for (auto& e : ev) hipEventDestroy(e);
    return rc;
}

int cfgpp_unet_tuning(cfgpp_unet* u, int rows, int* hints, int cap, int set) {
    CFGPP_REQUIRE(u && u->finalized && hints && rows > 0, "unet_tuning: bad args");
    const int n = (int)u->cfg_hints.size();
    CFGPP_REQUIRE(cap >= n, "unet_tuning: buffer of %d for %d launches", cap, n);
    if (set) {
        for (int sh = 0; sh < 2; ++sh) u->tuned_by_rows[std::make_pair(rows, sh != 0)] = std::vector<int>(hints, hints + n);
        if (u->tuned_rows == rows) u->tuned_rows = 0;
        ++u->tuned_serial;
        return n;
    }
    auto it = u->tuned_by_rows.find(std::make_pair(rows, u->ran_shared == 1));
    if (it == u->tuned_by_rows.end()) { cfgpp_set_error("unet_tuning: batch %d has not been tuned", rows); return -3; }
    std::copy(it->second.begin(), it->second.end(), hints);
    return n;
}

double cfgpp_unet_flops(cfgpp_unet* u, int rows) {
    if (!u || !u->finalized) return 0.0;
    const double once = u->ran_shared == 1 ? u->prefix_macs_per_row * (rows / 2) : 0.0;
    const double ip = u->ip_active ? u->ip_macs_per_key * u->ip_n_img : 0.0;
    const double text = u->ip_macs_per_key * (u->ctx_tokens - 77);
    return 2.0 * ((u->macs_per_row + u->attn_macs_per_row + text + ip) * rows - once);
}

void cfgpp_unet_set_share_prefix(int on) { g_share_prefix = on ? 1 : 0; }
int cfgpp_unet_share_prefix_enabled(void) { return g_share_prefix; }
int cfgpp_unet_shared_prefix_ops(cfgpp_unet* u, int rows, int z_rows) {
    if (!u || !u->finalized) return 0;
    return u->shares(rows, z_rows) ? u->prefix_ops : 0;
}
double cfgpp_unet_device_bytes(cfgpp_unet* u) { return u ? u->dev_bytes : 0.0; }

static WeightSlot* lora_slot(cfgpp_unet* u, const char* key, const char* who) {
    if (!u || !key) { cfgpp_set_error("%s: null argument", who); return nullptr; }
    if (!u->finalized) { cfgpp_set_error("%s: %s: the engine is not finalized (weights are merged into the uploaded, repacked matrices)", who, key); return nullptr; }
    const std::string k = key;
    if (k == "conv_in.weight" || k == "conv_out.weight") {
        cfgpp_set_error("%s: %s runs on the fp32 small-kernel path and takes no adapter", who, key); return nullptr;
    }
    auto it = u->params.find(k);
    if (it == u->params.end()) { cfgpp_set_error("%s: unknown key %s", who, key); return nullptr; }
    if (!it->second.is_matrix) { cfgpp_set_error("%s: %s is a 1-D parameter (bias / norm): adapters apply to matrices", who, key); return nullptr; }
    auto sl = u->slots.find(k);
    if (sl == u->slots.end()) { cfgpp_set_error("%s: %s is not held as an fp16 matrix (fp32 direct-convolution path)", who, key); return nullptr; }
    return &sl->second;
}

int cfgpp_unet_lora(cfgpp_unet* u, const char* key, const float* up, const float* down, int rank, void* stream) {
    WeightSlot* w = lora_slot(u, key, "lora");
    if (!w) return -2;
    CFGPP_REQUIRE(rank >= 0, "lora: %s: rank %d", key, rank);
    CFGPP_REQUIRE(rank == 0 || (up && down), "lora: %s: rank %d with a null up / down matrix", key, rank);
    CFGPP_HIP_CHECK(hipSetDevice(u->device));
    hipStream_t s = (hipStream_t)stream;
    const size_t bytes = (size_t)w->O * w->K() * sizeof(half_t);
    if (rank == 0) {
        if (w->base) {
            CFGPP_HIP_CHECK(hipMemcpyAsync(w->rows(), w->base, bytes, hipMemcpyDeviceToDevice, s));
            return u->refold(w->rows(), s);
        }
        return 0;
    }
    if (!w->base) {
        half_t* b = (half_t*)u->dmalloc(bytes, false);
        CFGPP_REQUIRE(b, "lora: %s: out of device memory for the saved base (%zu bytes)", key, bytes);
        CFGPP_HIP_CHECK(hipMemcpyAsync(b, w->rows(), bytes, hipMemcpyDeviceToDevice, s));
        w->base = b;
    }
    const int kind = w->kind == SLOT_MEMBER ? SLOT_PLAIN : w->kind;
    int e = lora_merge_launch(w->base, w->rows(), up, down, rank, kind, w->O, w->I, w->taps, s);
    if (e) { const std::string m = cfgpp_last_error(); cfgpp_set_error("lora: %s: %s", key, m.c_str()); return e; }
    return u->refold(w->rows(), s);
}

int cfgpp_unet_read_weight(cfgpp_unet* u, const char* key, void* host_fp16_out) {
    WeightSlot* w = lora_slot(u, key, "read_weight");
    if (!w) return -2;
    CFGPP_REQUIRE(host_fp16_out, "read_weight: %s: null output", key);
    const long O = w->O, Kc = w->K(), I = w->I; const int taps = w->taps;
    std::vector<half_t> r((size_t)O * Kc);
    CFGPP_HIP_CHECK(hipSetDevice(u->device));
    CFGPP_HIP_CHECK(hipDeviceSynchronize());
    CFGPP_HIP_CHECK(hipMemcpy(r.data(), w->rows(), r.size() * sizeof(half_t), hipMemcpyDeviceToHost));
    half_t* out = (half_t*)host_fp16_out;
    for (long p = 0; p < O; ++p) {
        long o = p;
        if (w->kind == SLOT_GEGLU) { const long q = p & 63; o = (p >> 6) * 32 + (q & 31) + (q >= 32 ? O / 2 : 0); }
        const half_t* src = &r[(size_t)p * Kc];
        half_t* dst = out + (size_t)o * Kc;
        if (w->kind == SLOT_CONV3) {
            for (long i = 0; i < I; ++i) for (int t = 0; t < taps; ++t) dst[i * taps + t] = src[((i >> 6) * taps + t) * 64 + (i & 63)];
        } else {
            std::memcpy(dst, src, Kc * sizeof(half_t));
        }
    }
    return 0;
}

static float* g_op_gstat = nullptr;
static int g_op_gstat_flag = 0;
void cfgpp_op_igemm_set_gstat(void* buf) { g_op_gstat = (float*)buf; }
int cfgpp_op_igemm_gstat_written() { return g_op_gstat_flag; }

int cfgpp_op_igemm(const void* a0, const void* a1, int C0, int C1, int taps, int amode, int H, int W,
                   const void* w, int M, int N, const float* bias, const float* temb, int temb_ld,
                   const void* resid, int rmode, int rld, void* out, int omode, int old_, int epi, void* stream) {
    IGemmArgs a = base_args();
    a.a0 = (const half_t*)a0; a.a1 = (const half_t*)a1; a.C0 = C0; a.C1 = C1; a.taps = taps; a.amode = amode; a.H = H; a.W = W;
    a.w = (const half_t*)w; a.M = M; a.N = N; a.K = taps * (C0 + C1); a.bias = bias; a.temb = temb; a.temb_ld = temb_ld;
    a.rows_per_batch = H * W; a.resid = (const half_t*)resid; a.rmode = rmode; a.rld = rld;
    a.out = (half_t*)out; a.omode = omode; a.old = old_; a.epi = epi;
    a.gstat = g_op_gstat; a.stat_flag = &g_op_gstat_flag; g_op_gstat_flag = 0;
    return igemm_launch(a, (hipStream_t)stream);
}

int cfgpp_op_fold_upsample(const void* w9, void* w4, int O, int I, void* stream) {
    return igemm_fold_upsample_launch((const half_t*)w9, (half_t*)w4, O, I, (hipStream_t)stream);
}

int cfgpp_op_upsample_conv3x3(const void* src, int C, int Hs, int Ws, const void* w9, const void* w4, int rows, int N,
                              const float* bias, void* out, void* stream) {
    IGemmArgs a = base_args();
    const bool ph = w4 != nullptr && upsample_phase_form(Hs, Ws, N);
    a.a0 = (const half_t*)src; a.C0 = C; a.taps = ph ? 4 : 9; a.amode = ph ? 4 : 3; a.H = 2 * Hs; a.W = 2 * Ws;
    a.w = (const half_t*)(ph ? w4 : w9); a.M = rows * a.H * a.W; a.N = N; a.K = a.taps * C; a.bias = bias;
    a.rows_per_batch = a.H * a.W; a.out = (half_t*)out; a.omode = 1; a.old = N; a.epi = EPI_STORE;
    a.gstat = g_op_gstat; a.stat_flag = &g_op_gstat_flag; g_op_gstat_flag = 0;
    return igemm_launch(a, (hipStream_t)stream);
}

int cfgpp_op_igemm_heads(const void* a_, int K, const void* w, int M, int N, const float* bias, int rows_per_batch,
                         void* hq, void* hk, void* hvt, int part0, int part_width, int head_dim, int heads,
                         int q_tok_pad, int tok_pad, void* stream) {
// ... 10 lines not shown
```

### cfgpp_amd/csrc/vae.hip

```cpp
#include "engine_base.h"

extern "C" int cfgpp_op_softmax_rows(void* s, long rows, int ncols, void* stream);
extern "C" int cfgpp_op_vae_posterior(const float* conv_out, const float* qw, const float* qb, const float* noise, float* z,
                                      float* moments, int B, int HW, float scale, void* stream);
extern "C" int cfgpp_op_conv_in_ex(const void* z, int z_is_half, void* out, const float* w, const float* bias,
                                   int R, int zB, int Cin, int H, int W, int Cout, const float* pre_w, const float* pre_b,
                                   float in_scale, void* stream);

struct cfgpp_vae : EngineBase {
    int h = 0, w = 0, device = 0;
    float scaling = 1.f;
    bool finalized = false, has_encoder = false;
    int ch[4] = {128, 256, 512, 512};
    const void* in_z = nullptr; void* out_img = nullptr;
    std::vector<Op> enc_plan;
    const void* in_img = nullptr; const float* in_noise = nullptr; float* out_z = nullptr; float* out_moments = nullptr;
    float* enc_co = nullptr;
    float post_scale = 1.0f, post_shift = 0.0f; int post_clamp = 0;
    double dec_macs = 0, enc_macs = 0;
    half_t *tok_a = nullptr, *tok_o = nullptr, *hq = nullptr, *hk = nullptr, *hvt = nullptr, *smat = nullptr;
};

namespace {

// ... 153 lines not shown
        float* bqkv = B.upload(bb);
        half_t* wo = B.linear(ap + ".to_out.0.weight"); float* bo = B.f32(ap + ".to_out.0.bias");
        P.groupnorm(y, nullptr, v->tok_a, false, ng, nb, 1e-6f, false);
        {
            IGemmArgs a = base_args(v);
            a.a0 = v->tok_a; a.C0 = C; a.amode = 0; a.w = wqkv; a.N = 3 * C; a.K = C; a.bias = bqkv; a.epi = EPI_HEADS;
            a.rows_per_batch = T; a.hq = v->hq; a.hk = v->hk; a.hvt = v->hvt; a.part0 = 0; a.part_width = C;
            a.head_dim = C; a.head_dim_pad = C; a.heads = 1; a.tok_pad = T; a.q_tok_pad = T;
            a.vt_linear = 1;
            v->macs_per_row += (double)T * 3 * C * C;
            P.ops->push_back([a, T](hipStream_t s, int rows) mutable { IGemmArgs b = a; b.M = rows * T; return igemm_launch(b, s); });
            if (tagged) v->tag(0, (double)T * 3 * C * C, "vae qkv");
        }
        {
            cfgpp_vae* vv = v; const float scale = 1.0f / sqrtf((float)C);
            P.ops->push_back([=](hipStream_t s, int rows) {
                for (int b = 0; b < rows; ++b) {
                    IGemmArgs a = base_args(vv);
                    a.a0 = vv->hq + (size_t)b * T * C; a.C0 = C; a.amode = 0; a.w = vv->hk + (size_t)b * T * C; a.M = T; a.N = T; a.K = C;
                    a.out = vv->smat + (size_t)b * T * T; a.omode = 0; a.old = T; a.epi = EPI_STORE; a.out_scale = scale; a.rows_per_batch = T;
                    int e = igemm_launch(a, s); if (e) return e;
                }
                return 0;
            });
            if (tagged) v->tag(1, (double)T * T * C, "vae attn QK^T");
            P.ops->push_back([=](hipStream_t s, int rows) { return cfgpp_op_softmax_rows(vv->smat, (long)rows * T, T, s); });
            if (tagged) v->tag(2, 0.0, "vae softmax");
            P.ops->push_back([=](hipStream_t s, int rows) {
                for (int b = 0; b < rows; ++b) {
                    IGemmArgs a = base_args(vv);
                    a.a0 = vv->smat + (size_t)b * T * T; a.C0 = T; a.amode = 0; a.w = vv->hvt + (size_t)b * C * T; a.M = T; a.N = C; a.K = T;
                    a.out = vv->tok_o + (size_t)b * T * C; a.omode = 0; a.old = C; a.epi = EPI_STORE; a.rows_per_batch = T;
                    int e = igemm_launch(a, s); if (e) return e;
                }
                return 0;
            });
            if (tagged) v->tag(1, (double)T * T * C, "vae attn PV");
            v->attn_macs_per_row += 2.0 * T * (double)T * C;
        }
        Tensor z2 = v->acq(y.H, y.W, C);
        P.linear_to_padded(v->tok_o, C, z2, wo, bo, y);
        v->rel(y);
        Tensor out = resblock(P, pfx + ".resnets.1", z2, C);
        v->rel(z2);
        return out;
    };

    Tensor x = v->acq(H, W, C);
    {
        HostParam* pw = B.get("decoder.conv_in.weight"); HostParam* pb = B.get("decoder.conv_in.bias");
        HostParam* qw = B.get("post_quant_conv.weight"); HostParam* qb = B.get("post_quant_conv.bias");
        CFGPP_REQUIRE(pw && pb && qw && qb, "vae_finalize: %s", B.err.c_str());
        std::vector<float> r((size_t)36 * C);
        for (int o = 0; o < C; ++o) for (int i = 0; i < 4; ++i) for (int t = 0; t < 9; ++t)
            r[(size_t)(t * 4 + i) * C + o] = pw->f[((size_t)o * 4 + i) * 9 + t];
        float* dw = B.upload(r); float* db = B.upload(pb->f);
        float* dqw = B.upload(qw->f); float* dqb = B.upload(qb->f);
        cfgpp_vae* vv = v; half_t* xp = x.p; const int HH = H, WW = W; const float inv = 1.0f / v->scaling;
        v->plan.push_back([=](hipStream_t s, int rows) {
            return cfgpp_op_conv_in_ex(vv->in_z, 0, xp, dw, db, rows, rows, 4, HH, WW, C, dqw, dqb, inv, s);
        });
        v->tag(3, 0.0, "vae conv_in");
        v->macs_per_row += (double)H * W * C * 36.0;
    }
    x = mid_block(PD, "decoder.mid_block", x);
    for (int i = 0; i < 4; ++i) {
        const int co = v->ch[3 - i];
        const std::string p = "decoder.up_blocks." + std::to_string(i);
        for (int j = 0; j < 3; ++j) {
            Tensor y = resblock(PD, p + ".resnets." + std::to_string(j), x, co);
            v->rel(x); x = y;
        }
        if (i != 3) {
            half_t* wu = B.conv3(p + ".upsamplers.0.conv.weight"); float* bu = B.f32(p + ".upsamplers.0.conv.bias");
            H *= 2; W *= 2;
            Tensor y = v->acq(H, W, co);
            PD.conv3x3(x, y, wu, bu, 3, nullptr, 0, nullptr);
            v->rel(x); x = y;
        }
    }
    {
        float* g = B.f32("decoder.conv_norm_out.weight"); float* b = B.f32("decoder.conv_norm_out.bias");
        Tensor gn = v->acq(H, W, x.C);
        PD.groupnorm(x, nullptr, gn.p, true, g, b, 1e-6f, true);
        HostParam* pw = B.get("decoder.conv_out.weight"); float* bo = B.f32("decoder.conv_out.bias");
        CFGPP_REQUIRE(pw, "vae_finalize: %s", B.err.c_str());
        const int Cc = x.C;
        std::vector<half_t> r((size_t)4 * 9 * Cc, (half_t)0.f);
        for (int o = 0; o < 3; ++o) for (int i = 0; i < Cc; ++i) for (int t = 0; t < 9; ++t)
            r[((size_t)o * 9 + t) * Cc + i] = pw->h[((size_t)o * Cc + i) * 9 + t];
        half_t* dw = B.upload(r);
        cfgpp_vae* vv = v; half_t* gp = gn.p; const int HH = H, WW = W;
        v->macs_per_row += (double)H * W * 3 * 9.0 * Cc;
        v->plan.push_back([=](hipStream_t s, int rows) {
            return cfgpp_op_conv_out_ex(gp, vv->out_img, 0, dw, bo, rows, HH, WW, Cc, 3, vv->post_scale, vv->post_shift, vv->post_clamp, s);
        });
        v->tag(3, 0.0, "vae conv_out");
        v->rel(gn); v->rel(x);
    }
    v->dec_macs = v->macs_per_row + v->attn_macs_per_row;

    if (v->has_encoder) {
        int EH = 8 * v->h, EW = 8 * v->w;
        const int c0 = v->ch[0];
        Tensor e = v->acq(EH, EW, c0);
        {
            HostParam* pw = B.get("encoder.conv_in.weight"); HostParam* pb = B.get("encoder.conv_in.bias");
            CFGPP_REQUIRE(pw && pb, "vae_finalize: %s", B.err.c_str());
            std::vector<float> r((size_t)27 * c0);
            for (int o = 0; o < c0; ++o) for (int i = 0; i < 3; ++i) for (int t = 0; t < 9; ++t)
                r[(size_t)(t * 3 + i) * c0 + o] = pw->f[((size_t)o * 3 + i) * 9 + t];
            float* dw = B.upload(r); float* db = B.upload(pb->f);
            cfgpp_vae* vv = v; half_t* ep = e.p; const int HH = EH, WW = EW;
            v->enc_plan.push_back([=](hipStream_t s, int rows) {
                return cfgpp_op_conv_in_ex(vv->in_img, 0, ep, dw, db, rows, rows, 3, HH, WW, c0, nullptr, nullptr, 1.0f, s);
            });
            v->macs_per_row += (double)EH * EW * c0 * 27.0;
        }
        for (int i = 0; i < 4; ++i) {
            const int co = v->ch[i];
            const std::string p = "encoder.down_blocks." + std::to_string(i);
            for (int j = 0; j < 2; ++j) {
                Tensor y = resblock(PE, p + ".resnets." + std::to_string(j), e, co);
                v->rel(e); e = y;
            }
            if (i != 3) {
                half_t* wd = B.conv3(p + ".downsamplers.0.conv.weight"); float* bd = B.f32(p + ".downsamplers.0.conv.bias");
                EH /= 2; EW /= 2;
                Tensor y = v->acq(EH, EW, co);
                PE.conv3x3(e, y, wd, bd, 2, nullptr, 0, nullptr, 1);
                v->rel(e); e = y;
            }
        }
        e = mid_block(PE, "encoder.mid_block", e);
        {
            float* g = B.f32("encoder.conv_norm_out.weight"); float* b = B.f32("encoder.conv_norm_out.bias");
            Tensor gn = v->acq(EH, EW, C);
            PE.groupnorm(e, nullptr, gn.p, true, g, b, 1e-6f, true);
            HostParam* pw = B.get("encoder.conv_out.weight"); float* bo = B.f32("encoder.conv_out.bias");
            HostParam* qw = B.get("quant_conv.weight"); HostParam* qb = B.get("quant_conv.bias");
            CFGPP_REQUIRE(pw && qw && qb, "vae_finalize: %s", B.err.c_str());
            std::vector<half_t> r((size_t)8 * 9 * C);
            for (int o = 0; o < 8; ++o) for (int i = 0; i < C; ++i) for (int t = 0; t < 9; ++t)
                r[((size_t)o * 9 + t) * C + i] = pw->h[((size_t)o * C + i) * 9 + t];
            half_t* dw = B.upload(r);
            std::vector<float> qwr(qw->f);
            for (auto& f : qwr) f = (float)(half_t)f;
            float* dqw = B.upload(qwr); float* dqb = B.upload(qb->f);
            v->enc_co = (float*)v->dmalloc((size_t)R * 8 * T * sizeof(float));
            CFGPP_REQUIRE(v->enc_co, "vae_finalize: hipMalloc failed");
            cfgpp_vae* vv = v; half_t* gp = gn.p; const int HH = EH, WW = EW; const float sc = v->scaling;
            v->macs_per_row += (double)T * 8 * 9.0 * C;
            v->enc_plan.push_back([=](hipStream_t s, int rows) { return cfgpp_op_conv_out(gp, vv->enc_co, 0, dw, bo, rows, HH, WW, C, 8, s); });
            v->enc_plan.push_back([=](hipStream_t s, int rows) {
                return cfgpp_op_vae_posterior(vv->enc_co, dqw, dqb, vv->in_noise, vv->out_z, vv->out_moments, rows, T, sc, s);
            });
            v->rel(gn); v->rel(e);
        }
        v->enc_macs = v->macs_per_row + v->attn_macs_per_row - v->dec_macs;
    }
    CFGPP_REQUIRE(B.ok, "vae_finalize: %s", B.err.c_str());
    CFGPP_HIP_CHECK(hipDeviceSynchronize());
    v->plan_kind.resize(v->plan.size(), 3); v->plan_macs.resize(v->plan.size(), 0.0); v->plan_desc.resize(v->plan.size());
    v->finalized = true;
    return 0;
}

static int vae_decode_impl(cfgpp_vae* v, const void* z, void* img, int B, void* stream);

int cfgpp_vae_decode(cfgpp_vae* v, const void* z, void* img, int B, void* stream) {
    if (v) { v->post_scale = 1.0f; v->post_shift = 0.0f; v->post_clamp = 0; }
    return vae_decode_impl(v, z, img, B, stream);
}

int cfgpp_vae_decode_image(cfgpp_vae* v, const void* z, void* img, int B, void* stream) {
    if (v) { v->post_scale = 0.5f; v->post_shift = 0.5f; v->post_clamp = 1; }
    return vae_decode_impl(v, z, img, B, stream);
}

static int vae_decode_impl(cfgpp_vae* v, const void* z, void* img, int B, void* stream) {
// ... 49 lines not shown
```

### cfgpp_amd/engine.py

```python
from __future__ import annotations

import ctypes as C
from typing import Dict, Iterable, Optional, Tuple

import torch

from . import _lib
from ._lib import CfgppError, UNetConfigC, check
from .unet_config import UNetConfig


def _require_cuda(t: torch.Tensor, name: str):
    if not t.is_cuda:
        raise CfgppError(f"{name} must live on the GPU (got {t.device}); the HIP path has no CPU fallback")
    if not t.is_contiguous():
        raise CfgppError(f"{name} must be contiguous")


def _stream_ptr(t: Optional[torch.Tensor] = None) -> int:
    if t is not None and t.is_cuda:
        return torch.cuda.current_stream(t.device).cuda_stream
    return torch.cuda.current_stream().cuda_stream


# ... 149 lines not shown
        if h:
            try:
                torch.cuda.synchronize()
            except Exception:
                pass
            self.lib.cfgpp_unet_destroy(h)
            self._h = None

    def load_tensor(self, key: str, t: torch.Tensor):
        t = t.detach().cpu().contiguous()
        if t.dtype == torch.float16:
            dt = 1
        else:
            t = t.to(torch.float32)
            dt = 0
        shape = (C.c_long * t.dim())(*t.shape)
        check(self.lib.cfgpp_unet_load_tensor(self._h, key.encode(), t.data_ptr(), dt, shape, t.dim()),
              f"cfgpp_unet_load_tensor({key})")

    def load_state_dict(self, items: Iterable[Tuple[str, torch.Tensor]]):
        if isinstance(items, dict):
            items = items.items()
        for k, v in items:
            self.load_tensor(k, v)
        return self

    def set_max_tokens(self, max_tokens: int):
        check(self.lib.cfgpp_unet_set_max_tokens(self._h, int(max_tokens)), "cfgpp_unet_set_max_tokens")
        self.max_tokens = int(max_tokens)
        return self

    def finalize(self):
        check(self.lib.cfgpp_unet_finalize(self._h), "cfgpp_unet_finalize")
        self.finalized = True
        return self

    def set_context(self, ehs: torch.Tensor, text_embeds: Optional[torch.Tensor] = None,
                    time_ids: Optional[torch.Tensor] = None):
        dev = torch.device("cuda", self.device)
        ehs = ehs.to(device=dev, dtype=torch.float16).contiguous()
        rows, tokens = int(ehs.shape[0]), int(ehs.shape[1])
        te = ti = None
        cond_rows = 0
        if self.cfg.addition_embed:
            if text_embeds is None or time_ids is None:
                raise CfgppError("set_context: SDXL needs text_embeds and time_ids")
            te = text_embeds.to(device=dev, dtype=torch.float16).contiguous()
            ti = time_ids.to(device=dev, dtype=torch.float32).contiguous()
            cond_rows = int(te.shape[0])
            if int(ti.shape[0]) != cond_rows:
                raise CfgppError("set_context: text_embeds / time_ids row mismatch")
        self._keep["ctx"] = (ehs, te, ti)
        self.rows = rows
        check(self.lib.cfgpp_unet_set_context(self._h, ehs.data_ptr(), rows, tokens, _ptr(te), _ptr(ti), cond_rows,
                                              _stream_ptr(ehs)), "cfgpp_unet_set_context")

    def image_condition(self, cond: torch.Tensor):
        if self.cond_channels <= 0:
            raise CfgppError(f"image_condition: {self.cfg.name} takes no image condition (in_channels == out_channels)")
        dev = torch.device("cuda", self.device)
        cond = cond.to(device=dev, dtype=torch.float16).contiguous()
        if cond.dim() != 4 or tuple(cond.shape[1:]) != (self.cond_channels, self.H, self.W):
            raise CfgppError(f"image_condition: cond shape {tuple(cond.shape)} != [*, {self.cond_channels}, {self.H}, {self.W}]")
        check(self.lib.cfgpp_unet_image_condition(self._h, cond.data_ptr(), int(cond.shape[0]), _stream_ptr(cond)),
              "cfgpp_unet_image_condition")
        self._keep["cond"] = cond

    def forward(self, z: torch.Tensor, t: float, eps_out: Optional[torch.Tensor] = None) -> torch.Tensor:
        _require_cuda(z, "z")
        if z.dtype not in (torch.float16, torch.float32):
            raise CfgppError("forward: z must be fp16 or fp32")
        zr = int(z.shape[0])
        if tuple(z.shape[1:]) != (self.latent_channels, self.H, self.W):
            raise CfgppError(f"forward: z shape {tuple(z.shape)} != [*, {self.latent_channels}, {self.H}, {self.W}]")
        rows = self.rows
        if rows % zr != 0:
            raise CfgppError(f"forward: rows={rows} is not a multiple of z rows={zr}")
        if eps_out is None:
            eps_out = torch.empty((rows, self.cfg.out_channels, self.H, self.W), dtype=torch.float16, device=z.device)
        check(self.lib.cfgpp_unet_forward(self._h, z.data_ptr(), 1 if z.dtype == torch.float16 else 0, zr, float(t),
                                          eps_out.data_ptr(), rows, _stream_ptr(z)), "cfgpp_unet_forward")
        return eps_out

    def _matrix_shape(self, key: str):
        from .unet_config import param_shapes
        shapes = getattr(self, "_shapes", None)
        if shapes is None:
            shapes = self._shapes = dict(param_shapes(self.cfg))
        return shapes.get(key)

    def lora(self, key: str, up: Optional[torch.Tensor], down: Optional[torch.Tensor]):
        dev = torch.device("cuda", self.device)
        stream = torch.cuda.current_stream(dev).cuda_stream
        if up is None or int(up.shape[1]) == 0:
            check(self.lib.cfgpp_unet_lora(self._h, key.encode(), None, None, 0, stream), f"cfgpp_unet_lora({key})")
            return
        shape = self._matrix_shape(key)
        if shape is not None and len(shape) in (2, 4):
            O, K = int(shape[0]), 1
            for d in shape[1:]:
                K *= int(d)
            if up.dim() != 2 or down.dim() != 2 or int(up.shape[0]) != O or int(down.shape[1]) != K or int(up.shape[1]) != int(down.shape[0]):
                raise CfgppError(f"lora({key}): up {tuple(up.shape)} / down {tuple(down.shape)} do not fit the weight {tuple(shape)} "
                                 f"(up [{O}, rank], down [rank, {K}])")
        up = up.to(device=dev, dtype=torch.float32).contiguous()
        down = down.to(device=dev, dtype=torch.float32).contiguous()
        check(self.lib.cfgpp_unet_lora(self._h, key.encode(), up.data_ptr(), down.data_ptr(), int(up.shape[1]), stream),
              f"cfgpp_unet_lora({key})")

    def read_weight(self, key: str) -> torch.Tensor:
        shape = self._matrix_shape(key)
        if shape is None:
            raise CfgppError(f"read_weight: unknown key {key}")
        out = torch.empty(tuple(shape), dtype=torch.float16)
        check(self.lib.cfgpp_unet_read_weight(self._h, key.encode(), out.data_ptr()), f"cfgpp_unet_read_weight({key})")
        return out

    def ip_load(self, key: Optional[str], t: Optional[torch.Tensor] = None):
        if key is None:
            check(self.lib.cfgpp_unet_ip_load(self._h, None, None, 0, None, 0), "cfgpp_unet_ip_load(NULL)")
            self._keep.pop("ip_embeds", None)
            return
        t = t.detach().cpu().contiguous()
        if t.dtype == torch.float16:
            dt = 1
        else:
            t = t.to(torch.float32)
            dt = 0
        shape = (C.c_long * t.dim())(*t.shape)
        check(self.lib.cfgpp_unet_ip_load(self._h, key.encode(), t.data_ptr(), dt, shape, t.dim()), f"cfgpp_unet_ip_load({key})")

    def set_image_context(self, image_embeds: Optional[torch.Tensor], scale: float = 1.0):
        dev = torch.device("cuda", self.device)
        stream = torch.cuda.current_stream(dev).cuda_stream
        if image_embeds is None or float(scale) == 0.0:
            check(self.lib.cfgpp_unet_image_context(self._h, None, 0, 0, 0.0, stream), "cfgpp_unet_image_context")
            return
        e = image_embeds.to(device=dev, dtype=torch.float16).contiguous()
        if e.dim() != 2:
            raise CfgppError(f"set_image_context: image_embeds shape {tuple(e.shape)}, expected [rows, embed_dim]")
        old = self._keep.get("ip_embeds")
        if old is not None and old.shape == e.shape and bool(torch.equal(old, e)):
            e = old
        else:
            e = e.clone()
        check(self.lib.cfgpp_unet_image_context(self._h, e.data_ptr(), int(e.shape[0]), int(e.shape[1]), float(scale), stream),
              "cfgpp_unet_image_context")
        self._keep["ip_embeds"] = e

    def attach_control(self, cn, scale: float):
        check(self.lib.cfgpp_unet_attach_control(self._h, None if cn is None else cn._h, float(scale)), "cfgpp_unet_attach_control")
        self._keep["control"] = cn

    def sample_graph_ddim(self, z: torch.Tensor, z0t: torch.Tensor, eps: torch.Tensor, eps_uc: torch.Tensor, eps_c: torch.Tensor,
                          steps, lam: float, tweedie_uc: bool, renoise_uc: bool):
        for n, t in (("z", z), ("z0t", z0t), ("eps", eps)):
            _require_cuda(t, n)
        if z.dtype != z0t.dtype or z.dtype not in (torch.float16, torch.float32) or eps.dtype != torch.float16:
            raise CfgppError("sample_graph_ddim: z / z0t must both be fp32 or both fp16, eps fp16")
        if tuple(z.shape[1:]) != (self.latent_channels, self.H, self.W) or z.shape != z0t.shape:
            raise CfgppError(f"sample_graph_ddim: z shape {tuple(z.shape)}")
        if int(eps.shape[0]) != self.rows or self.rows % int(z.shape[0]) != 0:
            raise CfgppError(f"sample_graph_ddim: eps rows {int(eps.shape[0])} / z rows {int(z.shape[0])} vs context rows {self.rows}")
        flat = [float(v) for st in steps for v in st]
        if len(flat) != 5 * len(steps) or not steps:
            raise CfgppError("sample_graph_ddim: steps must be a non-empty list of (t, c1, c2, c3, c4)")
# ... 51 lines not shown
```

### cfgpp_amd/hip_engine.py

```python
from __future__ import annotations

import os
from typing import Optional, Tuple

import torch

from . import engine as E
from . import _lib
from ._lib import CfgppError
from .tune_cache import PinCache, build_id
from .unet_config import CONFIGS, UNetConfig
from .weights import load_safetensors_iter, synth_state_dict_iter


class HipEngine:

    def __init__(self, cfg: UNetConfig, max_batch: int = 1, latent_hw: Optional[Tuple[int, int]] = None,
                 device=None, weights="synthetic", weight_seed: int = 0, max_tokens: int = 77):
        if isinstance(cfg, str):
            cfg = CONFIGS[cfg]
        if not torch.cuda.is_available():
            raise CfgppError("HipEngine needs a ROCm GPU; the HIP path has no CPU fallback")
        dev = torch.device(device if device is not None else "cuda")
        if dev.type != "cuda":
# ... 37 lines not shown
            raise CfgppError(f"batch {B} exceeds engine max_batch {self.max_batch}")
        if uc.shape[0] != B:
            uc = uc.expand(B, -1, -1)
        if c.shape[0] != B:
            c = c.expand(B, -1, -1)
        if int(uc.shape[1]) != int(c.shape[1]):
            raise CfgppError(f"set_context: uc has {int(uc.shape[1])} tokens, c {int(c.shape[1])}: pad the shorter prompt with chunks of the "
                             "empty prompt (cfgpp_amd.prompt)")
        ehs = torch.cat([uc, c], dim=0)
        self.unet.set_context(ehs, text_embeds, time_ids)
        self._ctx = (ehs, text_embeds, time_ids)
        if self._control is not None:
            self._control[0].set_context(ehs, text_embeds, time_ids)
        self._pins.load(2 * B)
        self.B = B
        if self._eps is None or int(self._eps.shape[0]) != 2 * B:
            self._eps = torch.empty((2 * B, self.cfg.out_channels, self.H, self.W), dtype=torch.float16, device=self.device)

    def image_condition(self, cond: torch.Tensor):
        self.unet.image_condition(cond)

    def set_control(self, cn, image: torch.Tensor, scale: float = 1.0):
        cn.set_image(image)
        if self._ctx is not None:
            cn.set_context(*self._ctx)
        self.unet.attach_control(cn, float(scale))
        self._control = (cn, float(scale))

    def clear_control(self):
        if self._control is not None:
            self.unet.attach_control(None, 0.0)
        self._control = None

    def build_controlnet(self, spec, seed: int = 0):
        from .controlnet import build_controlnet
        return build_controlnet(spec, self.cfg, 2 * self.max_batch, (self.H, self.W), self.device.index, seed, max_tokens=self.max_tokens)

    @property
    def control(self):
        return self._control

    def set_ip_adapter(self, spec):
        from .ip_adapter import resolve
        if spec is not None and self.max_tokens != 77:
            raise CfgppError(f"ip_adapter=...: IP-Adapter on an engine with max_tokens={self.max_tokens} (max_prompt_chunks > 1) is not "
                             "supported: the image tokens' key slots sit at key 96 of a 128-slot buffer")
        parsed = resolve(spec, self.cfg)
        if self._ip is not None:
            self.unet.ip_load(None)
        self._ip = None
        if parsed is not None:
            for k, v in parsed.items():
                self.unet.ip_load(k, v)
            self._ip = parsed
        return self

    @property
    def ip_adapter(self):
        return self._ip

    def set_image_embeds(self, embeds: Optional[torch.Tensor], negative: Optional[torch.Tensor] = None, scale: float = 1.0):
        if embeds is None or float(scale) == 0.0:
            self.unet.set_image_context(None)
            return
        if self.ip_adapter is None:
            raise CfgppError("ip_adapter_image_embeds given but no IP-Adapter is loaded (get_solver(..., ip_adapter=...) / set_ip_adapter)")
        from .ip_adapter import assemble_embeds
        if int(embeds.shape[-1]) != self.ip_adapter.embed_dim:
            raise CfgppError(f"ip_adapter_image_embeds: embed_dim {int(embeds.shape[-1])}, the adapter takes {self.ip_adapter.embed_dim}")
        self.unet.set_image_context(assemble_embeds(embeds, negative, self.B), float(scale))

    def set_lora(self, adapters, ignore_text_encoder: bool = False):
        self._lora.set(adapters, ignore_text_encoder=ignore_text_encoder)
        return self

    @property
    def lora_epoch(self) -> int:
        return self._lora.epoch

    @property
    def lora_adapters(self):
        return list(self._lora.adapters)

    def predict(self, z: torch.Tensor, t: float):
        eps = self.unet.forward(z, float(t), self._eps)
        self._pins.save(self.unet.rows)
        if self.check_finite:
            self._finite_or_raise(t)
        return eps[: self.B], eps[self.B:]

    @property
    def graph_enabled(self) -> bool:
        return os.environ.get("CFGPP_GRAPH", "0") not in ("", "0") and self._control is None

    def ddim_loop_graph(self, zt: torch.Tensor, steps, lam: float, tweedie_uc: bool, renoise_uc: bool, single: str = ""):
        key = (int(zt.shape[0]), zt.dtype)
        if self._g_buf is None or self._g_buf[0] != key:
            self._g_buf = (key, torch.empty_like(zt), torch.empty_like(zt))
        _, gz, gz0 = self._g_buf
        gz.copy_(zt)
        eps = self._eps
        euc, ec = eps[: self.B], eps[self.B:]
        if single == "uc":
            ec = euc
        elif single == "c":
            euc = ec
        self.unet.sample_graph_ddim(gz, gz0, eps, euc, ec, steps, lam, tweedie_uc, renoise_uc)
        self._pins.save(self.unet.rows)
        if self.check_finite:
            self._finite_or_raise(steps[-1][0])
        return gz0.clone(), gz.clone()

    def export_tuning(self):
        return self.unet.export_tuning(self.unet.rows)

    def import_tuning(self, hints, batch: int):
        self.unet.import_tuning(hints, 2 * int(batch))
        self._pins.mark_imported(2 * int(batch))

    def device_bytes(self) -> float:
        return self.unet.device_bytes()

    step_ddim = staticmethod(E.step_ddim)
    step_ddim_masked = staticmethod(E.step_ddim_masked)
    kdiff_input = staticmethod(E.kdiff_input)
    step_kdiff = staticmethod(E.step_kdiff)
    kdiff_denoise = staticmethod(E.kdiff_denoise)
    lincomb = staticmethod(E.lincomb)

    def randn_like(self, x):
        return torch.randn_like(x)

    def flops_per_forward(self, rows: int) -> float:
        return self.unet.flops(rows)
```

### cfgpp_amd/latent_diffusion.py

```python
from __future__ import annotations

import contextlib
import functools
import os
import sys
from typing import Any, Callable, Dict, List, Optional

import torch

from . import coeffs as K
from ._lib import CfgppError
from .conditioning import SyntheticTextEncoder, as_list
from .registry import Registry
from .schedule import SchedulerTables, get_ancestral_step, get_sigmas_karras
from .unet_config import SD15, UNetConfig

__SOLVER__ = Registry("Solver")
register_solver = __SOLVER__.register
get_solver = __SOLVER__.create


class _SchedulerView:

    def __init__(self, tables: SchedulerTables):
# ... 160 lines not shown
    def _ensure_image_context(self, ctx_changed: bool, uc, c):
        job, eng = self._ip_job, self.engine
        if not hasattr(eng, "set_image_embeds"):
            return
        key = None if job is None else (job[3], uc is None, c is None)
        if not ctx_changed and self._ip_key == key:
            return
        if job is None:
            eng.set_image_embeds(None)
        else:
            emb, neg, scale = job[:3]
            if uc is None:
                neg = emb
            elif c is None:
                emb = torch.zeros_like(emb) if neg is None else neg
                neg = emb
            eng.set_image_embeds(emb, neg, scale)
        self._ip_key = key

    def _lora_epoch(self) -> int:
        return int(getattr(self.engine, "lora_epoch", 0))

    @contextlib.contextmanager
    def _control(self, image, scale):
        eng = self.engine
        if image is None:
            if getattr(eng, "control", None) is not None:
                eng.clear_control()
            yield
            return
        if self.controlnet is None:
            raise ValueError("control_image given, but the solver has no ControlNet: get_solver(..., controlnet=\"synthetic\" | path | state_dict)")
        if not torch.is_tensor(image) or image.dim() != 4 or int(image.shape[1]) != 3:
            raise ValueError(f"control_image must be a [1 or B, 3, 8h, 8w] tensor in [0, 1], got {getattr(image, 'shape', type(image))}")
        eng.set_control(self.controlnet, image, float(scale))
        try:
            yield
        finally:
            eng.clear_control()

    @torch.no_grad()
    def get_text_embed(self, null_prompt, prompt):
        if self.max_prompt_chunks > 1:
            uc, c = self._long_text_embed(self.text_encoder, [as_list(null_prompt), as_list(prompt)])[0]
            return uc.to(self.work_device), c.to(self.work_device)
        uc, _ = self.text_encoder(as_list(null_prompt))
        c, _ = self.text_encoder(as_list(prompt))
        return uc.to(self.work_device), c.to(self.work_device)

    @staticmethod
    def _refuse_long_context_when_sharded(tokens: int):
        if int(tokens) > 77:
            import torch.distributed as dist
            if dist.is_available() and dist.is_initialized() and dist.get_world_size() > 1:
                raise ValueError(f"a text context of {int(tokens)} tokens ({int(tokens) // 77} prompt chunks) in a sharded run (world size > 1) is "
                                 "not supported: the packed broadcast of the conditioning has the shapes of one 77-token chunk")

    def _long_text_embed(self, encoder, groups, n_chunks=None, clip_skip=None):
        from . import prompt as P
        K = self.max_prompt_chunks
        j = max([P.chunks_needed(encoder, g, K) for g in groups] + [int(n_chunks or 1)])
        self._refuse_long_context_when_sharded(77 * j)
        enc = [P.encode_prompts(encoder, g, K, n_chunks=j, clip_skip=clip_skip) for g in groups]
        return [e[0] for e in enc], [e[1] for e in enc], j

    def _get_vae(self):
        if self.vae is None:
            if self.work_device.type != "cuda":
                raise CfgppError("decode/encode need the HIP VAE (ROCm GPU); on CPU pass vae=<object with decode/encode>")
            from .vae import HipVAE
            self.vae = HipVAE(self.cfg.vae_scale, self.latent_hw, max_batch=self.max_batch, device=self.work_device,
                              **self._vae_kwargs)
        return self.vae

    def encode(self, x):
        return self._get_vae().encode(x.to(self.work_device)).to(self.dtype)

    def decode(self, zt):
        return self._get_vae().decode(zt.to(self.work_device))

    def predict_noise(self, zt: torch.Tensor, t, uc: Optional[torch.Tensor], c: Optional[torch.Tensor]):
        return self._predict(zt, t, uc, c)

    def _predict(self, zt, t, uc, c, added=None):
        self._ensure_context(uc, c, added)
        noise_uc, noise_c = self.engine.predict(zt, float(t))
        if uc is None:
            return noise_c, noise_c
        if c is None:
            return noise_uc, noise_uc
        return noise_uc, noise_c

    def _ensure_context(self, uc, c, added=None):
        if uc is None and c is None:
            raise ValueError("predict_noise needs at least one of uc / c")
        a = c if uc is None else uc
        b = uc if c is None else c
        extra, extra_key = self._added_context(added)
        key = (a.data_ptr(), b.data_ptr(), tuple(a.shape), tuple(b.shape), a._version, b._version, self._lora_epoch(), *extra_key)
        changed = getattr(self, "_ctx_key", None) != key
        if changed:
            self._refuse_long_context_when_sharded(max(int(a.shape[1]), int(b.shape[1])))
            self._set_context(a, b, *extra)
            self._ctx_key = key
            self._ctx_keep = (a, b, *extra)
        self._ensure_image_context(changed, uc, c)

    def _added_context(self, added):
        return (), ()

    def _ddim_step_coeffs(self, t, inversion: bool, wrap: bool):
        sqrt4 = self.tables.ddim_sqrt_coeffs(t, wrap=wrap, inversion=inversion)
        final = not wrap and int(t) - self.tables.skip < 0
        return sqrt4, (("tw" if inversion else "rn") if final else None)

    def _graph_loop(self, zt, ts, uc, c, lam, tweedie_uc, renoise_uc, inversion, wrap):
        if not getattr(self.engine, "graph_enabled", False):
            return None
        z_half = zt.dtype == torch.float16
        steps = []
        for t in ts:
            sqrt4, dev_a = self._ddim_step_coeffs(t, inversion, wrap)
            co = K.ddim_coeffs_pinned(sqrt4, eps_half=True, semantics=self.scalar_semantics, z_half=z_half, device_alpha=dev_a)
            steps.append((float(t), *[float(v) for v in co]))
        single = "c" if uc is None else ("uc" if c is None else "")
        return self.engine.ddim_loop_graph(zt, steps, lam, tweedie_uc, renoise_uc, single)

    def _set_context(self, uc, c):
        self.engine.set_context(uc, c)

    def initialize_latent(self, method: str = "random", src_img: Optional[torch.Tensor] = None, **kwargs):
        if method == "ddim":
            z = self.inversion(self.encode(src_img.to(self.dtype)), kwargs.get("uc"), kwargs.get("c"),
                               cfg_guidance=kwargs.get("cfg_guidance", 0.0))
        elif method == "npi":
            z = self.inversion(self.encode(src_img.to(self.dtype)), kwargs.get("c"), kwargs.get("c"), cfg_guidance=1.0)
        elif method in ("random", "random_kdiffusion"):
            size = tuple(kwargs.get("latent_dim", (1, self.cfg.out_channels) + self.latent_hw))
            z = self._randn(size, kwargs.get("seeds"))
            if method == "random_kdiffusion":
                sigmas = kwargs.get("sigmas", [14.6146])
                z = z * (sigmas[0] ** 2 + 1) ** 0.5
            z = z.to(self.work_device)
        else:
            raise NotImplementedError
        return z

    @staticmethod
    def _randn(size, seeds=None) -> torch.Tensor:
        if seeds is None:
            return torch.randn(size)
        if len(seeds) != size[0]:
            raise ValueError(f"{len(seeds)} seeds for a batch of {size[0]}")
        out = []
        for s in seeds:
            g = torch.Generator().manual_seed(int(s))
            out.append(torch.randn((1,) + tuple(size[1:]), generator=g))
        return torch.cat(out, dim=0)

    def timestep(self, sigma):
        return self.tables.timestep(sigma)

    def to_d(self, x, sigma, denoised):
        return (x - denoised) / sigma.item()

    get_ancestral_step = staticmethod(get_ancestral_step)

    def calculate_input(self, x, sigma):
        return x / (sigma ** 2 + 1) ** 0.5

    def calculate_denoised(self, x, model_pred, sigma):
        return x - model_pred * sigma

    def _ddim_update(self, zt, z0t, noise_uc, noise_c, lam, sqrt4, tweedie_uc, renoise_uc, device_alpha=None, last=False):
        co = K.ddim_coeffs_pinned(sqrt4, eps_half=(noise_uc.dtype == torch.float16), semantics=self.scalar_semantics,
                                  z_half=(zt.dtype == torch.float16), device_alpha=device_alpha)
        self.engine.step_ddim(zt, z0t, noise_uc, noise_c, lam, co, tweedie_uc, renoise_uc)

    def _own_latent(self, z):
        dt = torch.float16 if z.dtype == torch.float16 else torch.float32
        return z.detach().to(device=self.work_device, dtype=dt, copy=True).contiguous()

    def _run_callback(self, callback_fn, step, t, z0t, zt):
        kw = callback_fn(step, t, {"z0t": z0t.detach(), "zt": zt.detach(), "decode": self.decode})
        if kw["z0t"] is not z0t:
            z0t.copy_(kw["z0t"])
        if kw["zt"] is not zt:
            zt.copy_(kw["zt"])

    def _ddim_loop(self, zt, uc, c, lam, tweedie_uc: bool, renoise_uc: bool, *, inversion=False, wrap=False, added=None, ts=None,
                   callback_fn=None, desc="SD", update=None):
        zt = self._own_latent(zt)
        if ts is None:
            ts = self.scheduler.timesteps.flip(0) if inversion else self.scheduler.timesteps
        ts = ts.int() if wrap else ts
        self._ensure_context(uc, c, added)
        if callback_fn is None:
            done = self._graph_loop(zt, ts, uc, c, lam, tweedie_uc, renoise_uc, inversion, wrap)
            if done is not None:
                return done
        update = update or self._ddim_update
        z0t = torch.empty_like(zt)
        n = len(ts)
        for step, t in enumerate(_progress(ts, desc)):
            sqrt4, dev_a = self._ddim_step_coeffs(t, inversion, wrap)
            noise_uc, noise_c = self._predict(zt, t, uc, c, added)
            update(zt, z0t, noise_uc, noise_c, lam, sqrt4, tweedie_uc, renoise_uc, dev_a, last=(step == n - 1))
            if callback_fn is not None:
                self._run_callback(callback_fn, step, t, z0t, zt)
        return z0t, zt

    inversion_cfgpp = False

    @torch.no_grad()
    def inversion(self, z0, uc, c, cfg_guidance: float = 1.0):
        return self._ddim_loop(z0, uc, c, cfg_guidance, self.inversion_cfgpp, False, inversion=True, desc="DDIM Inversion")[1]

    def _result(self, return_latents, latents, z):
        return latents if return_latents else self._finish(z)

    def _finish(self, z):
        if os.environ.get("CFGPP_TRACE"):
            torch.cuda.synchronize() if z.is_cuda else None
            print("[cfgpp] sampling loop done, decoding", file=sys.stderr, flush=True)
        vae = self._get_vae()
        if hasattr(vae, "decode_image"):
            img = vae.decode_image(z.to(self.work_device))
        else:
            img = (self.decode(z) / 2 + 0.5).clamp(0, 1)
        return img.detach().cpu()

    def _embeds(self, prompt, kwargs, n_cond=1):
        pe = kwargs.get("prompt_embeds")
        if pe is not None:
            return tuple(e.to(self.work_device, torch.float16) for e in pe)
        if self.max_prompt_chunks > 1:
            hs = self._long_text_embed(self.text_encoder, [as_list(prompt[k]) for k in range(1 + n_cond)])[0]
            return tuple(h.to(self.work_device) for h in hs)
        out = []
        uc = None
        for k in range(n_cond):
            uc, c = self.get_text_embed(null_prompt=prompt[0], prompt=prompt[1 + k])
            out.append(c)
        return (uc, *out)

    def _batch_of(self, c, kwargs):
        return int(c.shape[0])

    def _kdiff_start(self, size, sigmas, seeds):
        return self.initialize_latent(method="random_kdiffusion", latent_dim=size, sigmas=sigmas, seeds=seeds).to(torch.float16).contiguous()

    def _kdiff_loop(self, x, sigmas, uc, c, cfg_guidance, variant: int, solver: str, callback_fn=None, *, added=None, n_steps=None,
                    alphas=None, xl_form=False, t_of_sigma=None, desc="SD"):
        xc, den, old = torch.empty_like(x), torch.empty_like(x), torch.empty_like(x)
        t_of_sigma = t_of_sigma or self.timestep
        have_old = False
        for i in _progress(range(len(self.scheduler.timesteps) if n_steps is None else n_steps), desc):
            sigma = sigmas[i]
            new_t = t_of_sigma(sigma)
            if alphas is None:
                self.engine.kdiff_input(x, xc, K.kdiff_input_scale_sd(sigma, self.scalar_semantics), 0)
            else:
                self.engine.kdiff_input(x, xc, float(alphas[i].clone().sqrt()), 1)
            noise_uc, noise_c = self._predict(xc, new_t, uc, c, added)
            first = (solver == "euler") or (not have_old)
            coef, euler = K.kdiff_coeffs(cfg_guidance, sigmas, i, first, xl_form=xl_form, semantics=self.scalar_semantics)
            self.engine.step_kdiff(x, den, old, noise_uc, noise_c, coef, variant, xl_form, euler, solver != "euler")
            have_old = True
            if callback_fn is not None:
                self._run_callback(callback_fn, i, new_t, den, x)
        return den, x

    def _ancestral_loop(self, uc, c, cfg_guidance, cfgpp: bool, two_stage: bool, callback_fn=None, seeds=None):
        B = self._batch_of(c, None)
        lam = cfg_guidance
        sigmas = self.tables.karras_sigmas()
        x = self._kdiff_start((B, self.cfg.out_channels) + self.latent_hw, sigmas, seeds)
        xc, den, uden = torch.empty_like(x), torch.empty_like(x), torch.empty_like(x)
        x2, den2, uden2 = torch.empty_like(x), torch.empty_like(x), torch.empty_like(x)
        variant = 1 if cfgpp else 0
        sem = self.scalar_semantics
        t_fn = lambda sg: sg.log().neg()
        sigma_fn = lambda tt: tt.neg().exp()
        first = lambda sc: K._first(K._s(sc), True, sem)
        n = len(self.scheduler.timesteps)
        for i in _progress(range(n), "SD"):
            sigma = sigmas[i]
            new_t = self.timestep(sigma)
            sigma_down, sigma_up = get_ancestral_step(sigmas[i], sigmas[i + 1])
            self.engine.kdiff_input(x, xc, K.kdiff_input_scale_sd(sigma, self.scalar_semantics), 0)
            noise_uc, noise_c = self.predict_noise(xc, new_t, uc, c)
            if (not two_stage) or float(sigma_down) == 0.0:
                coef = [float(lam), float(sigma), 0.0, K.divisor(sigma.item(), sem), float(sigma_down), 0.0, 0.0, 1.0, 0.0]
                self.engine.step_kdiff(x, den, None, noise_uc, noise_c, coef, variant, False, True, False)
            else:
                self.engine.kdiff_denoise(x, noise_uc, noise_c, lam, float(sigma), den, uden)
                t, t_next = t_fn(sigmas[i]), t_fn(K._s(sigma_down))
                r = 1 / 2
                h = t_next - t
                s_mid = t + r * h
                self.engine.lincomb(x2, x, uden if cfgpp else den, None, first(sigma_fn(s_mid) / sigma_fn(t)),
                                    first((-h * r).expm1()), 0)
                sigma_s = sigma_fn(s_mid)
                t_2 = self.timestep(sigma_s)
                self.engine.kdiff_input(x2, xc, K.kdiff_input_scale_sd(sigma_s, self.scalar_semantics), 0)
                nuc2, nc2 = self.predict_noise(xc, t_2, uc, c)
                self.engine.kdiff_denoise(x2, nuc2, nc2, lam, float(sigma_s), den2, uden2)
                ratio_n = first(sigma_fn(t_next) / sigma_fn(t))
                if cfgpp:
                    self.engine.lincomb(x, x, den2, uden2, ratio_n, first(torch.exp(-h)), 1)
                else:
                    self.engine.lincomb(x, x, den2, None, ratio_n, first((-h).expm1()), 0)
            if sigmas[i + 1] > 0:
                self.engine.lincomb(x, x, self.engine.randn_like(x), None, float(sigma_up), 0.0, 2)
            if callback_fn is not None:
                self._run_callback(callback_fn, i, new_t, den, x)
        return den, x


def _sd_prompts(prompt):
    return prompt


@register_solver("ddim")
class BaseDDIM(StableDiffusion):
    cfgpp = False

    @torch.no_grad()
    @controlled
    def sample(self, cfg_guidance=7.5, prompt=["", ""], callback_fn=None, **kwargs):
        uc, c = self._embeds(prompt, kwargs)
        B = int(c.shape[0])
        zt = kwargs.get("latents")
        if zt is None:
            zt = self.initialize_latent(latent_dim=(B, self.cfg.out_channels) + self.latent_hw, seeds=kwargs.get("seeds"))
        z0t, zt = self._ddim_loop(zt.to(self.work_device), uc, c, cfg_guidance, False, self.cfgpp, callback_fn=callback_fn)
        return self._result(kwargs.get("return_latents"), (z0t, zt), z0t)


@register_solver("euler")
# ... 104 lines not shown
```

Baseline: 9.146 images/sec.

## Precompute time embeddings per schedule and fuse final groupnorm into conv_out

```diff
diff --git a/cfgpp_amd/_lib.py b/cfgpp_amd/_lib.py
--- a/cfgpp_amd/_lib.py
+++ b/cfgpp_amd/_lib.py
@@ -84,6 +84,10 @@
     "cfgpp_unet_set_max_tokens": (_I, [_P, _I]),
 }
 
+TIMESTEP_PROTOTYPES = {
+    "cfgpp_unet_set_timesteps": (_I, [_P, C.POINTER(C.c_float), _I, _P]),
+}
+
 DEBUG_PROTOTYPES = {
     "cfgpp_op_softmax_rows": (_I, [_P, _L, _I, _P]),
     "cfgpp_op_conv_in_ex": (_I, [_P, _I, _P, _P, _P, _I, _I, _I, _I, _I, _I, _P, _P, _F, _P]),
@@ -116,8 +120,16 @@
     "cfgpp_op_conv_out": (_I, [_P, _P, _I, _P, _P, _I, _I, _I, _I, _I, _P]),
     "cfgpp_op_conv_out_ex": (_I, [_P, _P, _I, _P, _P, _I, _I, _I, _I, _I, _F, _F, _I, _P]),
     "cfgpp_conv_out_set_tiled": (None, [_I]),
+    "cfgpp_conv_in_set_tiled": (None, [_I]),
+    "cfgpp_op_gn_conv_out_stats": (_I, [_P, _P, _P, _I, _P, _P, _I, _I, _P, _P, _I, _I, _I, _I, _I, _F, _F, _I, _P]),
+    "cfgpp_op_gn_conv_out": (_I, [_P, _P, _I, _P, _P, _I, _P, _P, _P, _I, _F, _I, _P, _P, _I, _I, _I, _I, _I, _F, _F, _I, _P]),
+    "cfgpp_tail_set_fused": (None, [_I]),
+    "cfgpp_tail_last_fused": (_I, []),
+    "cfgpp_op_groupnorm_finalize": (_I, [_P, _P, _I, _I, _I, _I, _I, _F, _P]),
+    "cfgpp_op_groupnorm_apply": (_I, [_P, _P, _P, _P, _P, _I, _I, _I, _I, _I, _I, _P]),
     "cfgpp_op_sinusoid": (_I, [_P, _F, _P, _I, _I, _I, _I, _P]),
     "cfgpp_op_skinny_gemm": (_I, [_P, _I, _P, _P, _P, _I, _P, _I, _I, _I, _I, _I, _I, _P]),
+    "cfgpp_op_skinny_gemm_m1": (_I, [_P, _I, _P, _P, _P, _I, _P, _I, _I, _I, _I, _I, _I, _P]),
     "cfgpp_op_f16_to_f32_rows": (_I, [_P, _P, _I, _I, _I, _I, _P]),
     "cfgpp_op_igemm": (_I, [_P, _P, _I, _I, _I, _I, _I, _I, _P, _I, _I, _P, _P, _I, _P, _I, _I, _P, _I, _I, _I, _P]),
     "cfgpp_op_igemm_heads": (_I, [_P, _I, _P, _I, _I, _P, _I, _P, _P, _P, _I, _I, _I, _I, _I, _I, _P]),
@@ -173,7 +185,7 @@
         lib = C.CDLL(LIB_PATH)
     except OSError as e:
         raise CfgppError(f"cannot load {LIB_PATH}: {e}") from e
-    for name, (res, args) in list(PROTOTYPES.items()) + list(IP_ADAPTER_PROTOTYPES.items()) + list(LONG_PROMPT_PROTOTYPES.items()) + list(DEBUG_PROTOTYPES.items()):
+    for name, (res, args) in list(PROTOTYPES.items()) + list(IP_ADAPTER_PROTOTYPES.items()) + list(LONG_PROMPT_PROTOTYPES.items()) + list(TIMESTEP_PROTOTYPES.items()) + list(DEBUG_PROTOTYPES.items()):
         try:
             fn = getattr(lib, name)
         except AttributeError as e:
diff --git a/cfgpp_amd/csrc/cfgpp_debug.h b/cfgpp_amd/csrc/cfgpp_debug.h
--- a/cfgpp_amd/csrc/cfgpp_debug.h
+++ b/cfgpp_amd/csrc/cfgpp_debug.h
@@ -64,10 +64,25 @@
 int cfgpp_op_conv_out_ex(const void* x, void* out, int out_is_half, const void* w, const float* bias,
                          int R, int H, int W, int C, int Cout, float post_scale, float post_shift, int clamp01, void* stream);
 void cfgpp_conv_out_set_tiled(int on);
+void cfgpp_conv_in_set_tiled(int on);
+int cfgpp_op_gn_conv_out_stats(const void* x, const float* stats, void* out, int out_is_half, const float* gamma, const float* beta,
+                               int G, int silu, const void* w, const float* bias, int R, int H, int W, int C, int Cout,
+                               float post_scale, float post_shift, int clamp01, void* stream);
+int cfgpp_op_gn_conv_out(const void* x, const float* gst, int gst_valid, void* scratch, void* out, int out_is_half,
+                         const float* gamma, const float* beta, float* stats, int G, float eps, int silu, const void* w,
+                         const float* bias, int R, int H, int W, int C, int Cout, float post_scale, float post_shift, int clamp01,
+                         void* stream);
+void cfgpp_tail_set_fused(int on);
+int cfgpp_tail_last_fused(void);
+int cfgpp_op_groupnorm_finalize(const float* gst, float* stats, int N, int H, int W, int C, int G, float eps, void* stream);
+int cfgpp_op_groupnorm_apply(const void* src, void* dst, const float* gamma, const float* beta, const float* stats, int N, int H, int W,
+                             int C, int G, int silu, void* stream);
 int cfgpp_op_sinusoid(const float* vals, float scalar, float* out, int count, int dim, int out_ld, int out_off,
                       void* stream);
 int cfgpp_op_skinny_gemm(const float* x, int ldx, const void* w, const float* bias, const float* addend, int add_ld,
                          float* out, int ldo, int M, int N, int K, int silu_in, int silu_out, void* stream);
+int cfgpp_op_skinny_gemm_m1(const float* x, int ldx, const void* w, const float* bias, const float* addend, int add_ld,
+                            float* out, int ldo, int M, int N, int K, int silu_in, int silu_out, void* stream);
 int cfgpp_op_f16_to_f32_rows(const void* in, float* out, int rows, int cols, int out_ld, int out_off, void* stream);
 
 int cfgpp_op_igemm(const void* a0, const void* a1, int C0, int C1, int taps, int amode, int H, int W,
diff --git a/cfgpp_amd/csrc/common.h b/cfgpp_amd/csrc/common.h
--- a/cfgpp_amd/csrc/common.h
+++ b/cfgpp_amd/csrc/common.h
@@ -59,6 +59,15 @@
 }
 
 __device__ __forceinline__ float silu_f(float x) { return x / (1.0f + __expf(-x)); }
+__device__ __forceinline__ void gn_scale_shift(float gamma, float beta, float mean, float rstd, float& sc, float& sh) {
+    const float ga = gamma * rstd;
+    sc = ga; sh = beta - mean * ga;
+}
+__device__ __forceinline__ half_t gn_value(half_t x, float sc, float sh, int silu) {
+    float f = (float)x * sc + sh;
+    if (silu) f = silu_f(f);
+    return (half_t)f;
+}
 __device__ __forceinline__ float gelu_erf_f(float x) {
     const float ax = fabsf(x) * 0.70710678118654752440f;
     const float t = __builtin_amdgcn_rcpf(1.0f + 0.3275911f * ax);
diff --git a/cfgpp_amd/csrc/engine_base.h b/cfgpp_amd/csrc/engine_base.h
--- a/cfgpp_amd/csrc/engine_base.h
+++ b/cfgpp_amd/csrc/engine_base.h
@@ -12,8 +12,10 @@
 #include "../../include/cfgpp.h"
 #include "../../include/cfgpp_ip_adapter.h"
 #include "../../include/cfgpp_long_prompt.h"
+#include "../../include/cfgpp_timesteps.h"
 #include "cfgpp_debug.h"
 #include "igemm.h"
+#include "head_tail_host.h"
 
 namespace {
 
diff --git a/cfgpp_amd/csrc/head_tail_host.h b/cfgpp_amd/csrc/head_tail_host.h
--- /dev/null
+++ b/cfgpp_amd/csrc/head_tail_host.h
@@ -0,0 +1,32 @@
+#pragma once
+#include <cstring>
+#include <vector>
+
+inline bool cfgpp_tail_fused(bool have_stats, int H, int W, int C, int Cout, int G) {
+    if (!have_stats) return false;
+    if (H <= 0 || W <= 0 || C <= 0 || G <= 0) return false;
+    if ((long)H * W < 1024 || ((long)H * W) % 32 != 0) return false;
+    if (C % 64 != 0 || Cout < 1 || Cout > 4) return false;
+    return G <= 64 && C % G == 0;
+}
+
+struct CfgppTimestepTable {
+    static constexpr int MAX_N = 1024;
+    std::vector<float> ts;
+    bool set(const float* v, int n) {
+        clear();
+        if (!v || n <= 0 || n > MAX_N) return false;
+        ts.assign(v, v + n);
+        return true;
+    }
+    void clear() { ts.clear(); }
+    int size() const { return (int)ts.size(); }
+    int find(float t) const {
+        for (size_t i = 0; i < ts.size(); ++i) if (ts[i] == t) return (int)i;
+        return -1;
+    }
+};
+inline bool cfgpp_key_feeds_time_embedding(const char* key) {
+    if (!key) return true;
+    return std::strstr(key, "time_embedding.") != nullptr || std::strstr(key, ".time_emb_proj.") != nullptr;
+}
diff --git a/cfgpp_amd/csrc/norm_kernels.hip b/cfgpp_amd/csrc/norm_kernels.hip
--- a/cfgpp_amd/csrc/norm_kernels.hip
+++ b/cfgpp_amd/csrc/norm_kernels.hip
@@ -331,17 +331,12 @@
 #pragma unroll
             for (int k = 0; k < 8; ++k) {
                 const int g = (c + k) / cpg;
-                const float ga = a.gamma[c + k] * s_rstd[g];
-                sc[k] = ga; sh[k] = a.beta[c + k] - s_mean[g] * ga;
+                gn_scale_shift(a.gamma[c + k], a.beta[c + k], s_mean[g], s_rstd[g], sc[k], sh[k]);
             }
             auto one = [&](int p, const half8_t v, long po) {
                 half8_t o;
 #pragma unroll
-                for (int k = 0; k < 8; ++k) {
-                    float f = (float)v[k] * sc[k] + sh[k];
-                    if (a.silu) f = silu_f(f);
-                    o[k] = (half_t)f;
-                }
+                for (int k = 0; k < 8; ++k) o[k] = gn_value(v[k], sc[k], sh[k], a.silu);
                 const long orow = a.dst_padded ? po : ((long)n * HW + p);
                 *reinterpret_cast<half8_t*>(a.dst + orow * C + c) = o;
             };
@@ -584,6 +579,32 @@
     return 0;
 }
 
+int cfgpp_op_groupnorm_finalize(const float* gst, float* stats, int N, int H, int W, int C, int G, float eps, void* stream) {
+    CFGPP_REQUIRE(G > 0 && G <= 64 && C % G == 0 && C % 8 == 0, "groupnorm_finalize: C=%d G=%d", C, G);
+    CFGPP_REQUIRE((H * W) % 32 == 0, "groupnorm_finalize: H*W=%d must be a multiple of 32 (the producers' statistics blocks)", H * W);
+    CFGPP_REQUIRE(gst && stats && N > 0, "groupnorm_finalize: bad args");
+    GNArgs a{};
+    a.N = N; a.H = H; a.W = W; a.C0 = C; a.C1 = 0; a.G = G; a.eps = eps; a.stats = stats; a.gst0 = gst; a.pre = 1;
+    hipLaunchKernelGGL(gn_finalize_kernel, dim3(G, N), dim3(256), 0, (hipStream_t)stream, a);
+    CFGPP_HIP_CHECK(hipGetLastError());
+    return 0;
+}
+
+int cfgpp_op_groupnorm_apply(const void* src, void* dst, const float* gamma, const float* beta, const float* stats, int N, int H, int W,
+                             int C, int G, int silu, void* stream) {
+    CFGPP_REQUIRE(G > 0 && G <= 64 && C % G == 0 && C % 8 == 0, "groupnorm_apply: C=%d G=%d", C, G);
+    CFGPP_REQUIRE(src && dst && gamma && beta && stats && N > 0, "groupnorm_apply: bad args");
+    GNArgs a{};
+    a.src0 = (const half_t*)src; a.dst = (half_t*)dst; a.gamma = gamma; a.beta = beta; a.stats = const_cast<float*>(stats);
+    a.N = N; a.H = H; a.W = W; a.C0 = C; a.G = G; a.silu = silu; a.dst_padded = 1; a.gs = 1; a.pre = 1;
+    int apb = 64;
+    while (apb > 16 && (long)N * cdiv(H * W, apb) < 1024) apb >>= 1;
+    a.pix_per_block = apb;
+    hipLaunchKernelGGL(gn_apply_kernel, dim3(cdiv(H * W, apb), N), dim3(256), 0, (hipStream_t)stream, a);
+    CFGPP_HIP_CHECK(hipGetLastError());
+    return 0;
+}
+
 int cfgpp_op_layernorm(const void* x, void* y, const float* gamma, const float* beta, long rows, int C,
                        float eps, void* stream) {
     g_ln_last[0] = 0; g_ln_last[1] = 0;
diff --git a/cfgpp_amd/csrc/small_kernels.hip b/cfgpp_amd/csrc/small_kernels.hip
--- a/cfgpp_amd/csrc/small_kernels.hip
+++ b/cfgpp_amd/csrc/small_kernels.hip
@@ -1,6 +1,18 @@
 #include <algorithm>
 
 #include "common.h"
+#include "head_tail_host.h"
+
+extern "C" {
+int cfgpp_groupnorm_prestats_enabled(void);
+int cfgpp_op_groupnorm(const void* src0, const void* src1, void* dst, const float* gamma, const float* beta,
+                       float* stats, int N, int H, int W, int C0, int C1, int G, float eps, int silu,
+                       int dst_padded, void* stream);
+int cfgpp_op_groupnorm_pre(const void* src0, const void* src1, void* dst, const float* gamma, const float* beta,
+                           const float* gst0, const float* gst1, float* stats, int N, int H, int W, int C0, int C1, int G,
+                           float eps, int silu, int dst_padded, void* stream);
+int cfgpp_op_groupnorm_finalize(const float* gst, float* stats, int N, int H, int W, int C, int G, float eps, void* stream);
+}
 
 namespace {
 
@@ -66,6 +78,97 @@
     }
 }
 
+template <typename TIN>
+__global__ void __launch_bounds__(256)
+conv_in_tile_kernel(const TIN* __restrict__ z, const half_t* __restrict__ cond, int Cc, int cond_rows,
+                    half_t* __restrict__ out, const float* __restrict__ w,
+                    const float* __restrict__ bias, int R, int zB, int Cz, int H, int W, int Cout,
+                    const float* __restrict__ pre_w, const float* __restrict__ pre_b, float in_scale,
+                    const half_t* __restrict__ add, int add_rows, int TP, int KC) {
+    extern __shared__ __attribute__((aligned(16))) float cin_lds[];
+    const int tid = threadIdx.x;
+    const int zb = blockIdx.y;
+    const int p0 = blockIdx.x * TP;
+    const int HW = H * W;
+    const int cb = cond ? zb % cond_rows : 0;
+    const int Cin = Cz + Cc;
+    const int K = 9 * Cin;
+    float* sP = cin_lds;
+    float* sW = cin_lds + K * TP;
+    for (int i = tid; i < TP * K; i += 256) {
+        const int k = i / TP, tp = i - k * TP;
+        const int tap = k / Cin, ci = k - tap * Cin;
+        const int p = p0 + tp;
+        float v = 0.f;
+        if (p < HW) {
+            const int y = p / W + tap / 3 - 1, x = p % W + tap % 3 - 1;
+            if (y >= 0 && y < H && x >= 0 && x < W) {
+                if (ci >= Cz) {
+                    v = (float)cond[((long)(cb * Cc + ci - Cz) * H + y) * W + x];
+                } else if (pre_w) {
+                    float acc = pre_b ? pre_b[ci] : 0.f;
+                    for (int j = 0; j < Cz; ++j)
+                        acc += pre_w[ci * Cz + j] * (float)(half_t)((float)z[((long)(zb * Cz + j) * H + y) * W + x] * in_scale);
+                    v = acc;
+                } else {
+                    v = (float)z[((long)(zb * Cz + ci) * H + y) * W + x] * in_scale;
+                }
+            }
+        }
+        sP[i] = (float)(half_t)v;
+    }
+    const int CG = Cout >> 3;
+    const int pg = tid / CG, cg = tid - pg * CG;
+    const bool active = pg * 8 < TP;
+    f32x2 acc[8][4];
+    if (active) {
+#pragma unroll
+        for (int c2 = 0; c2 < 4; ++c2) {
+            const f32x2 b = {bias ? bias[cg * 8 + 2 * c2] : 0.f, bias ? bias[cg * 8 + 2 * c2 + 1] : 0.f};
+#pragma unroll
+            for (int j = 0; j < 8; ++j) acc[j][c2] = b;
+        }
+    }
+    for (int k0 = 0; k0 < K; k0 += KC) {
+        const int kn = min(KC, K - k0);
+        __syncthreads();
+        const float4* wsrc = reinterpret_cast<const float4*>(w + (long)k0 * Cout);
+        for (int i = tid; i < kn * (Cout >> 2); i += 256) reinterpret_cast<float4*>(sW)[i] = wsrc[i];
+        __syncthreads();
+        if (active) {
+            for (int kk = 0; kk < kn; ++kk) {
+                const float4 wa = *reinterpret_cast<const float4*>(sW + kk * Cout + cg * 8);
+                const float4 wb = *reinterpret_cast<const float4*>(sW + kk * Cout + cg * 8 + 4);
+                const float4 pa = *reinterpret_cast<const float4*>(sP + (k0 + kk) * TP + pg * 8);
+                const float4 pb = *reinterpret_cast<const float4*>(sP + (k0 + kk) * TP + pg * 8 + 4);
+                const f32x2 w2[4] = {{wa.x, wa.y}, {wa.z, wa.w}, {wb.x, wb.y}, {wb.z, wb.w}};
+                const float pv[8] = {pa.x, pa.y, pa.z, pa.w, pb.x, pb.y, pb.z, pb.w};
+#pragma unroll
+                for (int j = 0; j < 8; ++j)
+#pragma unroll
+                    for (int c2 = 0; c2 < 4; ++c2) acc[j][c2] = __builtin_elementwise_fma(w2[c2], (f32x2){pv[j], pv[j]}, acc[j][c2]);
+            }
+        }
+    }
+    if (!active) return;
+#pragma unroll
+    for (int j = 0; j < 8; ++j) {
+        const int p = p0 + pg * 8 + j;
+        if (p >= HW) continue;
+        const int y = p / W, x = p - y * W;
+        half8_t v;
+#pragma unroll
+        for (int c2 = 0; c2 < 4; ++c2) { v[2 * c2] = (half_t)acc[j][c2].x; v[2 * c2 + 1] = (half_t)acc[j][c2].y; }
+        if (add) {
+            const half8_t a = *reinterpret_cast<const half8_t*>(add + ((long)((zb % add_rows) * (H + 2) + y + 1) * (W + 2) + x + 1) * Cout + cg * 8);
+#pragma unroll
+            for (int k = 0; k < 8; ++k) v[k] = (half_t)((float)v[k] + (float)a[k]);
+        }
+        for (int r = zb; r < R; r += zB)
+            *reinterpret_cast<half8_t*>(out + ((long)(r * (H + 2) + y + 1) * (W + 2) + x + 1) * Cout + cg * 8) = v;
+    }
+}
+
 template <int CO, typename TOUT>
 __global__ void __launch_bounds__(256)
 conv_out_kernel(const half_t* __restrict__ x, TOUT* __restrict__ out, const half_t* __restrict__ w,
@@ -170,6 +273,114 @@
     }
 }
 
+template <int TH, typename TOUT>
+__global__ void __launch_bounds__(256)
+gn_conv_out_kernel(const half_t* __restrict__ x, TOUT* __restrict__ out, const half_t* __restrict__ w,
+                   const float* __restrict__ bias, const float* __restrict__ stats, const float* __restrict__ gamma,
+                   const float* __restrict__ beta, int G, int silu, int R, int H, int W, int C, int cout_real,
+                   float post_scale, float post_shift, int clamp01) {
+    constexpr int TW = 32, HH = TH + 2, HW_ = TW + 2, PITCH = 144, NPX = HH * HW_, NIT = (NPX * 8 + 255) / 256, MB = TH / 2;
+    __shared__ __attribute__((aligned(16))) char tile[NPX * PITCH];
+    __shared__ float s_mean[64], s_rstd[64];
+    const int tid = threadIdx.x, lane = tid & 63, wv = tid >> 6;
+    const int tiles_x = (W + TW - 1) / TW, tiles_y = (H + TH - 1) / TH;
+    int b = blockIdx.x;
+    const int txi = b % tiles_x; b /= tiles_x;
+    const int tyi = b % tiles_y; const int r = b / tiles_y;
+    const int y0 = tyi * TH, x0 = txi * TW;
+    if (tid < G) {
+        const float2 mr = *reinterpret_cast<const float2*>(stats + ((long)r * G + tid) * 2);
+        s_mean[tid] = mr.x; s_rstd[tid] = mr.y;
+    }
+    const int cpg = C / G;
+    const int ch = tid & 7;
+    const half_t* xr = x + (long)r * (H + 2) * (W + 2) * C;
+    int poff[NIT];
+#pragma unroll
+    for (int j = 0; j < NIT; ++j) {
+        const int px = (tid >> 3) + j * 32;
+        const int hy = px / HW_, hx = px - hy * HW_;
+        const int gy = y0 + hy, gx = x0 + hx;
+        poff[j] = (px < NPX && gy >= 1 && gy <= H && gx >= 1 && gx <= W) ? (gy * (W + 2) + gx) * C + ch * 8 : -1;
+    }
+    half8_t v[NIT];
+    auto issue = [&](int cb) {
+#pragma unroll
+        for (int j = 0; j < NIT; ++j) {
+            half8_t t = {0, 0, 0, 0, 0, 0, 0, 0};
+            if (poff[j] >= 0) t = *reinterpret_cast<const half8_t*>(xr + poff[j] + cb);
+            v[j] = t;
+        }
+    };
+    issue(0);
+    const int wo = lane & 15, kb = lane >> 4;
+    f32x4 acc[MB];
+#pragma unroll
+    for (int m = 0; m < MB; ++m) acc[m] = (f32x4){0.f, 0.f, 0.f, 0.f};
+    for (int cb = 0; cb < C; cb += 64) {
+        half8_t bw[9][2];
+#pragma unroll
+        for (int tap = 0; tap < 9; ++tap)
+#pragma unroll
+            for (int k32 = 0; k32 < 2; ++k32) {
+                half8_t t = {0, 0, 0, 0, 0, 0, 0, 0};
+                if (wo < cout_real) t = *reinterpret_cast<const half8_t*>(w + ((long)wo * 9 + tap) * C + cb + k32 * 32 + kb * 8);
+                bw[tap][k32] = t;
+            }
+        __syncthreads();
+        {
+            float sc[8], sh[8];
+#pragma unroll
+            for (int k = 0; k < 8; ++k) {
+                const int c = cb + ch * 8 + k;
+                const int g = c / cpg;
+                gn_scale_shift(gamma[c], beta[c], s_mean[g], s_rstd[g], sc[k], sh[k]);
+            }
+#pragma unroll
+            for (int j = 0; j < NIT; ++j) {
+                const int px = (tid >> 3) + j * 32;
+                half8_t o = {0, 0, 0, 0, 0, 0, 0, 0};
+                if (poff[j] >= 0) {
+#pragma unroll
+                    for (int k = 0; k < 8; ++k) o[k] = gn_value(v[j][k], sc[k], sh[k], silu);
+                }
+                if (px < NPX) *reinterpret_cast<half8_t*>(tile + px * PITCH + ch * 16) = o;
+            }
+        }
+        __syncthreads();
+        if (cb + 64 < C) issue(cb + 64);
+#pragma unroll
+        for (int tap = 0; tap < 9; ++tap) {
+            const int dy = tap / 3, dx = tap - 3 * (tap / 3);
+#pragma unroll
+            for (int k32 = 0; k32 < 2; ++k32)
+#pragma unroll
+                for (int m = 0; m < MB; ++m) {
+                    const int ty = wv * (TH / 4) + (m >> 1), xh = m & 1;
+                    const half8_t a = *reinterpret_cast<const half8_t*>(tile + ((ty + dy) * HW_ + xh * 16 + wo + dx) * PITCH + (k32 * 32 + kb * 8) * 2);
+                    acc[m] = __builtin_amdgcn_mfma_f32_16x16x32_f16(a, bw[tap][k32], acc[m], 0, 0, 0);
+                }
+        }
+    }
+    if (wo < cout_real) {
+        const float bo = bias ? bias[wo] : 0.f;
+#pragma unroll
+        for (int m = 0; m < MB; ++m) {
+            const int y = y0 + wv * (TH / 4) + (m >> 1);
+#pragma unroll
+            for (int q = 0; q < 4; ++q) {
+                const int xq = x0 + (m & 1) * 16 + kb * 4 + q;
+                if (y < H && xq < W) {
+                    float f = acc[m][q] + bo;
+                    f = f * post_scale + post_shift;
+                    if (clamp01) f = fminf(fmaxf(f, 0.f), 1.f);
+                    out[((long)(r * cout_real + wo) * H + y) * W + xq] = (TOUT)f;
+                }
+            }
+        }
+    }
+}
+
 __global__ void sinusoid_kernel(const float* __restrict__ vals, float scalar, float* __restrict__ out,
                                 int count, int dim, int out_ld, int out_off) {
     const int i = blockIdx.x;
@@ -336,6 +547,38 @@
     return cfgpp_op_conv_in_add(z, z_is_half, cond, cond_rows, Cc, nullptr, 1, out, w, bias, R, zB, Cz, H, W, Cout, stream);
 }
 
+static int g_conv_in_tiled = 1;
+void cfgpp_conv_in_set_tiled(int on) { g_conv_in_tiled = on ? 1 : 0; }
+
+static int conv_in_launch(const void* z, int z_is_half, const half_t* cond, int cond_rows, int Cc, const half_t* add, int add_rows,
+                          half_t* out, const float* w, const float* bias, int R, int zB, int Cz, int H, int W, int Cout,
+                          const float* pre_w, const float* pre_b, float in_scale, hipStream_t s) {
+    const int K = 9 * (Cz + Cc);
+    const int CG = Cout / 8;
+    const int TP = CG > 0 && CG <= 256 ? 8 * std::min(8, 256 / CG) : 0;
+    const int KC = TP ? std::min(K, (16384 - K * TP) / Cout) : 0;
+    if (g_conv_in_tiled && Cout % 8 == 0 && TP > 0 && KC >= 1 && (((uintptr_t)w | (uintptr_t)out | (uintptr_t)add) & 15) == 0) {
+        dim3 grid(cdiv((long)H * W, TP), std::min(R, zB));
+        const size_t lds = (size_t)(K * TP + KC * Cout) * sizeof(float);
+        if (z_is_half)
+            hipLaunchKernelGGL(conv_in_tile_kernel<half_t>, grid, dim3(256), lds, s, (const half_t*)z, cond, Cc, cond_rows, out, w, bias,
+                               R, zB, Cz, H, W, Cout, pre_w, pre_b, in_scale, add, add_rows, TP, KC);
+        else
+            hipLaunchKernelGGL(conv_in_tile_kernel<float>, grid, dim3(256), lds, s, (const float*)z, cond, Cc, cond_rows, out, w, bias,
+                               R, zB, Cz, H, W, Cout, pre_w, pre_b, in_scale, add, add_rows, TP, KC);
+    } else {
+        dim3 grid(cdiv((long)H * W, 16), R);
+        if (z_is_half)
+            hipLaunchKernelGGL(conv_in_kernel<half_t>, grid, dim3(256), 0, s, (const half_t*)z, cond, Cc, cond_rows, out, w, bias,
+                               R, zB, Cz, H, W, Cout, pre_w, pre_b, in_scale, add, add_rows);
+        else
+            hipLaunchKernelGGL(conv_in_kernel<float>, grid, dim3(256), 0, s, (const float*)z, cond, Cc, cond_rows, out, w, bias,
+                               R, zB, Cz, H, W, Cout, pre_w, pre_b, in_scale, add, add_rows);
+    }
+    CFGPP_HIP_CHECK(hipGetLastError());
+    return 0;
+}
+
 int cfgpp_op_conv_in_add(const void* z, int z_is_half, const void* cond, int cond_rows, int Cc, const void* addend, int add_rows,
                          void* out, const float* w, const float* bias, int R, int zB, int Cz, int H, int W, int Cout, void* stream) {
     CFGPP_REQUIRE(Cz >= 1 && Cz <= 8, "conv_in: Cin=%d (<= 8)", Cz);
@@ -346,16 +589,8 @@
                   Cc, cond_rows, Cz);
     CFGPP_REQUIRE(z && out && w && R > 0 && zB > 0, "conv_in: bad args");
     if (!cond) { Cc = 0; cond_rows = 1; }
-    dim3 grid(cdiv((long)H * W, 16), R);
-    hipStream_t s = (hipStream_t)stream;
-    if (z_is_half)
-        hipLaunchKernelGGL(conv_in_kernel<half_t>, grid, dim3(256), 0, s, (const half_t*)z, (const half_t*)cond, Cc, cond_rows, (half_t*)out, w, bias,
-                           R, zB, Cz, H, W, Cout, (const float*)nullptr, (const float*)nullptr, 1.0f, add, add_rows);
-    else
-        hipLaunchKernelGGL(conv_in_kernel<float>, grid, dim3(256), 0, s, (const float*)z, (const half_t*)cond, Cc, cond_rows, (half_t*)out, w, bias,
-                           R, zB, Cz, H, W, Cout, (const float*)nullptr, (const float*)nullptr, 1.0f, add, add_rows);
-    CFGPP_HIP_CHECK(hipGetLastError());
-    return 0;
+    return conv_in_launch(z, z_is_half, (const half_t*)cond, cond_rows, Cc, add, add_rows, (half_t*)out, w, bias, R, zB, Cz, H, W, Cout,
+                          nullptr, nullptr, 1.0f, (hipStream_t)stream);
 }
 
 int cfgpp_op_conv_in_ex(const void* z, int z_is_half, void* out, const float* w, const float* bias,
@@ -363,16 +598,8 @@
                         float in_scale, void* stream) {
     CFGPP_REQUIRE(Cin >= 1 && Cin <= 8, "conv_in: Cin=%d (<= 8)", Cin);
     CFGPP_REQUIRE(z && out && w && R > 0 && zB > 0, "conv_in: bad args");
-    dim3 grid(cdiv((long)H * W, 16), R);
-    hipStream_t s = (hipStream_t)stream;
-    if (z_is_half)
-        hipLaunchKernelGGL(conv_in_kernel<half_t>, grid, dim3(256), 0, s, (const half_t*)z, (const half_t*)nullptr, 0, 1, (half_t*)out, w, bias,
-                           R, zB, Cin, H, W, Cout, pre_w, pre_b, in_scale, (const half_t*)nullptr, 1);
-    else
-        hipLaunchKernelGGL(conv_in_kernel<float>, grid, dim3(256), 0, s, (const float*)z, (const half_t*)nullptr, 0, 1, (half_t*)out, w, bias,
-                           R, zB, Cin, H, W, Cout, pre_w, pre_b, in_scale, (const half_t*)nullptr, 1);
-    CFGPP_HIP_CHECK(hipGetLastError());
-    return 0;
+    return conv_in_launch(z, z_is_half, nullptr, 1, 0, nullptr, 1, (half_t*)out, w, bias, R, zB, Cin, H, W, Cout, pre_w, pre_b, in_scale,
+                          (hipStream_t)stream);
 }
 
 int cfgpp_op_conv_in(const void* z, int z_is_half, void* out, const float* w, const float* bias,
@@ -397,7 +624,7 @@
     const long total = (long)R * H * W;
     dim3 grid(cdiv(total, 4));
     hipStream_t s = (hipStream_t)stream;
-    if (Cout <= 4 && C % 64 == 0 && (long)H * W >= 128 * 128 && g_conv_out_tiled) {
+    if (Cout <= 4 && C % 64 == 0 && g_conv_out_tiled) {
         dim3 tg((unsigned)((long)R * cdiv(H, 8) * cdiv(W, 32)));
         if (out_is_half)
             hipLaunchKernelGGL((conv_out_tile_kernel<4, half_t>), tg, dim3(256), 0, s, (const half_t*)x, (half_t*)out, (const half_t*)w, bias, R, H, W, C, Cout, post_scale, post_shift, clamp01);
@@ -417,6 +644,52 @@
         hipLaunchKernelGGL((conv_out_kernel<4, float>), grid, dim3(256), 0, s, (const half_t*)x, (float*)out, (const half_t*)w, bias, R, H, W, C, Cout, post_scale, post_shift, clamp01);
     CFGPP_HIP_CHECK(hipGetLastError());
     return 0;
+}
+
+static int g_tail_fused = 1;
+void cfgpp_tail_set_fused(int on) { g_tail_fused = on ? 1 : 0; }
+static int g_tail_last = 0;
+int cfgpp_tail_last_fused(void) { return g_tail_last; }
+
+int cfgpp_op_gn_conv_out_stats(const void* x, const float* stats, void* out, int out_is_half, const float* gamma, const float* beta,
+                               int G, int silu, const void* w, const float* bias, int R, int H, int W, int C, int Cout,
+                               float post_scale, float post_shift, int clamp01, void* stream) {
+    CFGPP_REQUIRE(x && stats && out && w && gamma && beta && R > 0 && H > 0 && W > 0, "gn_conv_out: bad args");
+    CFGPP_REQUIRE(C > 0 && C % 64 == 0 && Cout >= 1 && Cout <= 4 && G > 0 && G <= 64 && C % G == 0, "gn_conv_out: C=%d Cout=%d G=%d", C, Cout, G);
+    CFGPP_REQUIRE((long)(H + 2) * (W + 2) * C < (1L << 31), "gn_conv_out: sample of %d x %d x %d elements", H, W, C);
+    hipStream_t s = (hipStream_t)stream;
+    const bool small = (long)R * cdiv(H, 8) * cdiv(W, 32) < 1024;
+    dim3 tg((unsigned)((long)R * cdiv(H, small ? 4 : 8) * cdiv(W, 32)));
+#define GN_CO(TH_, T_) hipLaunchKernelGGL((gn_conv_out_kernel<TH_, T_>), tg, dim3(256), 0, s, (const half_t*)x, (T_*)out, (const half_t*)w, bias, \
+                                          stats, gamma, beta, G, silu, R, H, W, C, Cout, post_scale, post_shift, clamp01)
+    if (out_is_half) { if (small) GN_CO(4, half_t); else GN_CO(8, half_t); }
+    else { if (small) GN_CO(4, float); else GN_CO(8, float); }
+#undef GN_CO
+    CFGPP_HIP_CHECK(hipGetLastError());
+    return 0;
+}
+
+int cfgpp_op_gn_conv_out(const void* x, const float* gst, int gst_valid, void* scratch, void* out, int out_is_half,
+                         const float* gamma, const float* beta, float* stats, int G, float eps, int silu, const void* w,
+                         const float* bias, int R, int H, int W, int C, int Cout, float post_scale, float post_shift, int clamp01,
+                         void* stream) {
+    CFGPP_REQUIRE(x && out && w && gamma && beta && stats && R > 0, "gn_conv_out: bad args");
+    const bool have = gst && gst_valid && cfgpp_groupnorm_prestats_enabled();
+    g_tail_last = 0;
+    if (g_tail_fused && g_conv_out_tiled && cfgpp_tail_fused(have, H, W, C, Cout, G)) {
+        int e = cfgpp_op_groupnorm_finalize(gst, stats, R, H, W, C, G, eps, stream);
+        if (e) return e;
+        e = cfgpp_op_gn_conv_out_stats(x, stats, out, out_is_half, gamma, beta, G, silu, w, bias, R, H, W, C, Cout, post_scale, post_shift,
+                                       clamp01, stream);
+        if (e == 0) g_tail_last = 1;
+        return e;
+    }
+    CFGPP_REQUIRE(scratch, "gn_conv_out: the two-op form needs the scratch tensor");
+    int e = have && (H * W) % 32 == 0
+                ? cfgpp_op_groupnorm_pre(x, nullptr, scratch, gamma, beta, gst, nullptr, stats, R, H, W, C, 0, G, eps, silu, 1, stream)
+                : cfgpp_op_groupnorm(x, nullptr, scratch, gamma, beta, stats, R, H, W, C, 0, G, eps, silu, 1, stream);
+    if (e) return e;
+    return cfgpp_op_conv_out_ex(scratch, out, out_is_half, w, bias, R, H, W, C, Cout, post_scale, post_shift, clamp01, stream);
 }
 
 int cfgpp_op_sinusoid(const float* vals, float scalar, float* out, int count, int dim, int out_ld, int out_off,
@@ -442,6 +715,16 @@
     return 0;
 }
 
+int cfgpp_op_skinny_gemm_m1(const float* x, int ldx, const void* w, const float* bias, const float* addend, int add_ld,
+                            float* out, int ldo, int M, int N, int K, int silu_in, int silu_out, void* stream) {
+    CFGPP_REQUIRE(x && w && out && M > 0 && M <= 65535 && N > 0 && K % 8 == 0, "skinny_gemm_m1: bad args (M=%d K=%d)", M, K);
+    dim3 grid(cdiv(N, 4 * 2), M);
+    hipLaunchKernelGGL((skinny_gemm_kernel<1, 2>), grid, dim3(256), 0, (hipStream_t)stream, x, ldx, (const half_t*)w, bias, addend, add_ld, out, ldo,
+                       M, N, K, silu_in, silu_out);
+    CFGPP_HIP_CHECK(hipGetLastError());
+    return 0;
+}
+
 int cfgpp_op_f16_to_f32_rows(const void* in, float* out, int rows, int cols, int out_ld, int out_off, void* stream) {
     hipLaunchKernelGGL(f16_to_f32_rows_kernel, dim3(cdiv((long)rows * cols, 256) > 1024 ? 1024 : cdiv((long)rows * cols, 256)),
                        dim3(256), 0, (hipStream_t)stream, (const half_t*)in, out, rows, cols, out_ld, out_off);
diff --git a/cfgpp_amd/csrc/unet.hip b/cfgpp_amd/csrc/unet.hip
--- a/cfgpp_amd/csrc/unet.hip
+++ b/cfgpp_amd/csrc/unet.hip
@@ -37,6 +37,12 @@
     float* d_sin_t = nullptr; float* d_emb_h = nullptr; float* d_emb_t = nullptr; float* d_emb = nullptr;
     float* d_temb_all = nullptr; int temb_total = 0;
     float* d_add_in = nullptr; float* d_add_h = nullptr; float* d_aug = nullptr;
+    CfgppTimestepTable ttab;
+    int head_ops = 0;
+    float* d_ttab = nullptr; float* d_ttab_ts = nullptr; float* d_ttab_sin = nullptr; float* d_ttab_h = nullptr; float* d_ttab_e = nullptr;
+    int ttab_cap = 0;
+    const half_t* te_w1 = nullptr; const float* te_b1 = nullptr; const half_t* te_w2 = nullptr; const float* te_b2 = nullptr;
+    const half_t* te_wall = nullptr; const float* te_ball = nullptr; int te_c0 = 0, te_dim = 0;
 
     half_t *tok_x = nullptr, *tok_ln = nullptr, *tok_attn = nullptr, *tok_ff = nullptr;
     half_t *hq[4] = {nullptr, nullptr, nullptr, nullptr}, *hk[4] = {nullptr, nullptr, nullptr, nullptr},
@@ -425,6 +431,9 @@
             u->plan.push_back([=](hipStream_t s, int) {
                 return cfgpp_op_skinny_gemm(uu->d_emb_t, temb_dim, w_temb_all, b_temb_all, nullptr, 0, uu->d_temb_all, uu->temb_total, 1, uu->temb_total, temb_dim, 1, 0, s);
             });
+            u->head_ops = (int)u->plan.size();
+            u->te_w1 = w1; u->te_b1 = b1; u->te_w2 = w2; u->te_b2 = b2; u->te_wall = w_temb_all; u->te_ball = b_temb_all;
+            u->te_c0 = c0; u->te_dim = temb_dim;
         }
         if (c.addition_embed) {
             const int tdim = c.addition_time_embed_dim, pooled = c.addition_pooled_dim, in = 6 * tdim + pooled;
@@ -680,7 +689,6 @@
     {
         float* g = B.f32("conv_norm_out.weight"); float* b = B.f32("conv_norm_out.bias");
         Tensor gn = u->acq(H, W, c0);
-        P.groupnorm(x, nullptr, gn.p, true, g, b, 1e-5f, true);
         HostParam* pw = B.get("conv_out.weight"); float* bo = B.f32("conv_out.bias");
         CFGPP_REQUIRE(pw, "finalize: %s", B.err.c_str());
         const int Co = c.out_channels;
@@ -691,7 +699,12 @@
         half_t* dw = B.upload(r);
         cfgpp_unet* uu = u; half_t* gp = gn.p; const int HH = H, WW = W;
         u->macs_per_row += (double)H * W * Co * 9.0 * c0 + (double)c.sample_h * c.sample_w * c0 * 9.0 * c.in_channels;
-        u->plan.push_back([=](hipStream_t s, int rows) { return cfgpp_op_conv_out(gp, uu->out_eps, 1, dw, bo, rows, HH, WW, c0, Co, s); });
+        const half_t* xp = x.p; const float* xgst = x.gst; const int* xok = x.gst_ok; const int G = u->norm_groups;
+        u->plan.push_back([=](hipStream_t s, int rows) {
+            return cfgpp_op_gn_conv_out(xp, xgst, xgst && xok ? *xok : 0, gp, uu->out_eps, 1, g, b, uu->d_gn_stats, G, 1e-5f, 1, dw, bo, rows,
+                                        HH, WW, c0, Co, 1.0f, 0.0f, 0, s);
+        });
+        u->tag(3, 0.0, "groupnorm+conv_out HW=" + std::to_string(H * W) + " C=" + std::to_string(c0));
     }
     CFGPP_REQUIRE(B.ok, "finalize: %s", B.err.c_str());
     CFGPP_REQUIRE(skips.empty(), "finalize: internal error, %d skips left", (int)skips.size());
@@ -975,7 +988,43 @@
         int e = u->tune_plan((hipStream_t)stream, rows, shared); if (e) return e;
         ++u->tuned_serial;
     }
-    for (size_t i = 0; i < u->plan.size(); ++i) { int e = u->plan[i]((hipStream_t)stream, u->rows_for(i, rows, shared)); if (e) return e; }
+    size_t first = 0;
+    const int hit = u->head_ops > 0 ? u->ttab.find(t) : -1;
+    if (hit >= 0) {
+        CFGPP_HIP_CHECK(hipMemcpyAsync(u->d_temb_all, u->d_ttab + (size_t)hit * u->temb_total, (size_t)u->temb_total * sizeof(float),
+                                       hipMemcpyDeviceToDevice, (hipStream_t)stream));
+        first = (size_t)u->head_ops;
+    }
+    for (size_t i = first; i < u->plan.size(); ++i) { int e = u->plan[i]((hipStream_t)stream, u->rows_for(i, rows, shared)); if (e) return e; }
+    return 0;
+}
+
+int cfgpp_unet_set_timesteps(cfgpp_unet* u, const float* ts, int n, void* stream) {
+    CFGPP_REQUIRE(u && u->finalized, "set_timesteps: context not finalized");
+    u->ttab.clear();
+    if (u->ctrl) { int e = cfgpp_unet_set_timesteps(u->ctrl, ts, n, stream); if (e) return e; }
+    if (u->head_ops == 0 || !ts || n <= 0 || n > CfgppTimestepTable::MAX_N) return 0;
+    CFGPP_HIP_CHECK(hipSetDevice(u->device));
+    hipStream_t s = (hipStream_t)stream;
+    if (n > u->ttab_cap) {
+        const int cap = (n + 63) / 64 * 64;
+        u->d_ttab = (float*)u->dmalloc((size_t)cap * u->temb_total * sizeof(float), false);
+        u->d_ttab_ts = (float*)u->dmalloc((size_t)cap * sizeof(float), false);
+        u->d_ttab_sin = (float*)u->dmalloc((size_t)cap * u->te_c0 * sizeof(float), false);
+        u->d_ttab_h = (float*)u->dmalloc((size_t)cap * u->te_dim * sizeof(float), false);
+        u->d_ttab_e = (float*)u->dmalloc((size_t)cap * u->te_dim * sizeof(float), false);
+        u->ttab_cap = (u->d_ttab && u->d_ttab_ts && u->d_ttab_sin && u->d_ttab_h && u->d_ttab_e) ? cap : 0;
+        CFGPP_REQUIRE(u->ttab_cap, "set_timesteps: out of device memory for %d timesteps", n);
+    }
+    const int c0 = u->te_c0, td = u->te_dim, tot = u->temb_total;
+    CFGPP_HIP_CHECK(hipMemcpyAsync(u->d_ttab_ts, ts, (size_t)n * sizeof(float), hipMemcpyHostToDevice, s));
+    CFGPP_HIP_CHECK(hipStreamSynchronize(s));
+    int e = cfgpp_op_sinusoid(u->d_ttab_ts, 0.f, u->d_ttab_sin, n, c0, c0, 0, s);
+    if (!e) e = cfgpp_op_skinny_gemm_m1(u->d_ttab_sin, c0, u->te_w1, u->te_b1, nullptr, 0, u->d_ttab_h, td, n, td, c0, 0, 1, s);
+    if (!e) e = cfgpp_op_skinny_gemm_m1(u->d_ttab_h, td, u->te_w2, u->te_b2, nullptr, 0, u->d_ttab_e, td, n, td, td, 0, 0, s);
+    if (!e) e = cfgpp_op_skinny_gemm_m1(u->d_ttab_e, td, u->te_wall, u->te_ball, nullptr, 0, u->d_ttab, tot, n, tot, td, 1, 0, s);
+    if (e) return e;
+    u->ttab.set(ts, n);
     return 0;
 }
 
@@ -1153,6 +1202,7 @@
 int cfgpp_unet_lora(cfgpp_unet* u, const char* key, const float* up, const float* down, int rank, void* stream) {
     WeightSlot* w = lora_slot(u, key, "lora");
     if (!w) return -2;
+    if (cfgpp_key_feeds_time_embedding(key)) u->ttab.clear();
     CFGPP_REQUIRE(rank >= 0, "lora: %s: rank %d", key, rank);
     CFGPP_REQUIRE(rank == 0 || (up && down), "lora: %s: rank %d with a null up / down matrix", key, rank);
     CFGPP_HIP_CHECK(hipSetDevice(u->device));
diff --git a/cfgpp_amd/csrc/vae.hip b/cfgpp_amd/csrc/vae.hip
--- a/cfgpp_amd/csrc/vae.hip
+++ b/cfgpp_amd/csrc/vae.hip
@@ -259,7 +259,6 @@
     {
         float* g = B.f32("decoder.conv_norm_out.weight"); float* b = B.f32("decoder.conv_norm_out.bias");
         Tensor gn = v->acq(H, W, x.C);
-        PD.groupnorm(x, nullptr, gn.p, true, g, b, 1e-6f, true);
         HostParam* pw = B.get("decoder.conv_out.weight"); float* bo = B.f32("decoder.conv_out.bias");
         CFGPP_REQUIRE(pw, "vae_finalize: %s", B.err.c_str());
         const int Cc = x.C;
@@ -269,10 +268,12 @@
         half_t* dw = B.upload(r);
         cfgpp_vae* vv = v; half_t* gp = gn.p; const int HH = H, WW = W;
         v->macs_per_row += (double)H * W * 3 * 9.0 * Cc;
+        const half_t* xp = x.p; const float* xgst = x.gst; const int* xok = x.gst_ok; const int G = v->norm_groups;
         v->plan.push_back([=](hipStream_t s, int rows) {
-            return cfgpp_op_conv_out_ex(gp, vv->out_img, 0, dw, bo, rows, HH, WW, Cc, 3, vv->post_scale, vv->post_shift, vv->post_clamp, s);
+            return cfgpp_op_gn_conv_out(xp, xgst, xgst && xok ? *xok : 0, gp, vv->out_img, 0, g, b, vv->d_gn_stats, G, 1e-6f, 1, dw, bo, rows,
+                                        HH, WW, Cc, 3, vv->post_scale, vv->post_shift, vv->post_clamp, s);
         });
-        v->tag(3, 0.0, "vae conv_out");
+        v->tag(3, 0.0, "vae groupnorm+conv_out");
         v->rel(gn); v->rel(x);
     }
     v->dec_macs = v->macs_per_row + v->attn_macs_per_row;
diff --git a/cfgpp_amd/engine.py b/cfgpp_amd/engine.py
--- a/cfgpp_amd/engine.py
+++ b/cfgpp_amd/engine.py
@@ -255,6 +255,12 @@
                                           eps_out.data_ptr(), rows, _stream_ptr(z)), "cfgpp_unet_forward")
         return eps_out
 
+    def set_timesteps(self, ts):
+        import ctypes
+        vals = [float(t) for t in ts]
+        arr = (ctypes.c_float * max(len(vals), 1))(*vals)
+        check(self.lib.cfgpp_unet_set_timesteps(self._h, arr, len(vals), torch.cuda.current_stream().cuda_stream), "cfgpp_unet_set_timesteps")
+
     def _matrix_shape(self, key: str):
         from .unet_config import param_shapes
         shapes = getattr(self, "_shapes", None)
diff --git a/cfgpp_amd/hip_engine.py b/cfgpp_amd/hip_engine.py
--- a/cfgpp_amd/hip_engine.py
+++ b/cfgpp_amd/hip_engine.py
@@ -143,6 +143,9 @@
     def lora_adapters(self):
         return list(self._lora.adapters)
 
+    def set_timesteps(self, ts):
+        self.unet.set_timesteps(ts)
+
     def predict(self, z: torch.Tensor, t: float):
         eps = self.unet.forward(z, float(t), self._eps)
         self._pins.save(self.unet.rows)
diff --git a/cfgpp_amd/latent_diffusion.py b/cfgpp_amd/latent_diffusion.py
--- a/cfgpp_amd/latent_diffusion.py
+++ b/cfgpp_amd/latent_diffusion.py
@@ -266,6 +266,11 @@
     def predict_noise(self, zt: torch.Tensor, t, uc: Optional[torch.Tensor], c: Optional[torch.Tensor]):
         return self._predict(zt, t, uc, c)
 
+    def _announce_timesteps(self, ts):
+        announce = getattr(self.engine, "set_timesteps", None)
+        if announce is not None:
+            announce([float(t) for t in ts])
+
     def _predict(self, zt, t, uc, c, added=None):
         self._ensure_context(uc, c, added)
         noise_uc, noise_c = self.engine.predict(zt, float(t))
@@ -386,6 +391,7 @@
         update = update or self._ddim_update
         z0t = torch.empty_like(zt)
         n = len(ts)
+        self._announce_timesteps(ts)
         for step, t in enumerate(_progress(ts, desc)):
             sqrt4, dev_a = self._ddim_step_coeffs(t, inversion, wrap)
             noise_uc, noise_c = self._predict(zt, t, uc, c, added)
@@ -439,7 +445,9 @@
         xc, den, old = torch.empty_like(x), torch.empty_like(x), torch.empty_like(x)
         t_of_sigma = t_of_sigma or self.timestep
         have_old = False
-        for i in _progress(range(len(self.scheduler.timesteps) if n_steps is None else n_steps), desc):
+        n_steps = len(self.scheduler.timesteps) if n_steps is None else n_steps
+        self._announce_timesteps(t_of_sigma(sigmas[i]) for i in range(n_steps))
+        for i in _progress(range(n_steps), desc):
             sigma = sigmas[i]
             new_t = t_of_sigma(sigma)
             if alphas is None:
diff --git a/include/cfgpp_timesteps.h b/include/cfgpp_timesteps.h
--- /dev/null
+++ b/include/cfgpp_timesteps.h
@@ -0,0 +1,13 @@
+#ifndef CFGPP_TIMESTEPS_H
+#define CFGPP_TIMESTEPS_H
+#include "cfgpp.h"
+#ifdef __cplusplus
+extern "C" {
+#endif
+
+int cfgpp_unet_set_timesteps(cfgpp_unet* u, const float* ts, int n, void* stream);
+
+#ifdef __cplusplus
+}
+#endif
+#endif
```

Measured after the change: 9.212 images/sec, median of 6. About the same (+0.7%).
